# DiTEC-project/gnn-pressure-estimation

Measured on AMD Instinct MI355X. Metric: train snapshots/sec, higher is better.
Workload: dtype f32; 1 GPU; gatres_small (15 blocks, nc=32), C-Town-sized WDN (388 nodes, 860 directed edges), batch_size=32 per GPU, fp32, full training step (device mask 0.95 -> fwd -> masked MSE -> bwd -> Adam), fused per-snapshot kernel (8 CUs per snapshot, row-window tables), hipGraph replay (20 steps per graph launch); global_batch=32, parallelism=dp1, plan_relabelled=False, row_window=92, dropped_steps=0, captured_graphs=25

## Files before the change

gnn-pressure-estimation_amd/_native.py:

```python
from __future__ import annotations

import ctypes as C
import os
from typing import Optional

import torch

from . import _build

_LIB: Optional[C.CDLL] = None

DTYPE_F32, DTYPE_BF16 = 0, 1

ERRORS = {-1: "GATRES_E_BADARG (null/misaligned pointer or bad size)",
          -2: "GATRES_E_UNSUPPORTED (width / storage type not supported: nc must be a power of two in [4, 128]; bf16 "
              "needs nc >= 32)",
          -3: "GATRES_E_GRAPH (edge endpoint out of range)"}


class GatresGraph(C.Structure):
    _fields_ = [("num_nodes", C.c_int32), ("num_edges_gat", C.c_int32), ("num_edges_mean", C.c_int32),
                ("num_segments", C.c_int32),
                ("rowptr", C.c_void_p), ("col", C.c_void_p), ("t_rowptr", C.c_void_p), ("t_eid", C.c_void_p),
                ("t_dst", C.c_void_p), ("m_rowptr", C.c_void_p), ("m_col", C.c_void_p), ("mt_rowptr", C.c_void_p),
                ("mt_dst", C.c_void_p), ("seg_ptr", C.c_void_p), ("max_segment_nodes", C.c_int32),
                ("max_segment_edges_gat", C.c_int32), ("max_segment_edges_mean", C.c_int32), ("flags", C.c_int32),
                ("window", C.c_int32 * 21), ("reserved2", C.c_int32), ("perm", C.c_void_p),
                ("halo", C.c_int32 * 7), ("reserved3", C.c_int32),
                ("part_tables", C.c_void_p), ("part_tables_m", C.c_int32), ("part_tables_stride", C.c_int32)]


MODEL_INFERENCE = 1


class GatresAutoClip(C.Structure):
    _fields_ = [("log", C.c_void_p), ("sorted", C.c_void_p * 2), ("ctl", C.c_void_p), ("partials", C.c_void_p),
                ("norm_out", C.c_void_p), ("clip_out", C.c_void_p), ("coef_out", C.c_void_p), ("capacity", C.c_int64),
                ("partials_cap", C.c_int32), ("reserved", C.c_int32), ("percentile", C.c_double)]


class GatresEpochConfig(C.Structure):
    _fields_ = [("min_delta", C.c_double), ("factor", C.c_double), ("threshold", C.c_double), ("min_lr", C.c_double),
                ("eps", C.c_double), ("patience", C.c_int32), ("scheduler_patience", C.c_int32), ("use_scheduler", C.c_int32),
                ("reserved", C.c_int32)]


class GatresModel(C.Structure):
    _fields_ = [("num_blocks", C.c_int32), ("nc", C.c_int32), ("act_dtype", C.c_int32), ("flags", C.c_int32)]


_P = C.c_void_p
_I32, _I64, _U64, _F32, _F64 = C.c_int32, C.c_int64, C.c_uint64, C.c_float, C.c_double
_GP, _MP = C.POINTER(GatresGraph), C.POINTER(GatresModel)

SIGNATURES = {
    "gatres_graph_count_host": (C.c_int, [_P, _I64, _I64, C.POINTER(_I64)]),
    "gatres_graph_build_host": (C.c_int, [_P, _I64, _I64] + [_P] * 9),
    "gatres_graph_flags_host": (C.c_int, [_P, _I64, _I64, C.POINTER(_I32)]),
    "gatres_graph_part_tables_host": (C.c_int, [_P] * 10 + [_I32, _I32, _P, _I64, C.POINTER(_I64)]),
    "gatres_graph_segments_host": (C.c_int, [_P, _I64, _I64, _I32, _P] + [C.POINTER(_I32)] * 4),
    "gatres_graph_windows_host": (C.c_int, [_P, _I64, _I64, _P, _I32, _P]),
    "gatres_graph_reorder_host": (C.c_int, [_P, _I64, _I64, _P, _I32, _P]),
    "gatres_lz4_decompress_host": (_I64, [_P, _I64, _P, _I64]),
    "gatres_edge_index_hash": (C.c_int, [_P, _I64, _P, _P]),
    "gatres_permute_f32": (C.c_int, [_P, _P, _P, _I32, _I32, _P]),
    "gatres_gather_u8": (C.c_int, [_P, _P, _P, _I32, _P]),
    "gatres_fused_serialize": (C.c_int, [_P]),
    "gatres_probe_xcd_dispatch": (C.c_int, [_P]),
    "gatres_knobs_reload": (C.c_int, []),
    "gatres_fused_status_offset": (_I64, [_MP, _GP]),
    "gatres_lin0_fwd": (C.c_int, [_P, _P, _P, _P, _P, _I32, _I32, _P]),
    "gatres_proj_attn_fwd": (C.c_int, [_P] * 7 + [_I32] * 4 + [_P]),
    "gatres_gat_aggregate_fwd": (C.c_int, [_GP] + [_P] * 6 + [_I32] * 3 + [_P]),
    "gatres_mean_residual_relu_fwd": (C.c_int, [_GP, _P, _P, _P, _I32, _P]),
    "gatres_lin1_fwd": (C.c_int, [_P, _P, _P, _P, _I32, _I32, _P]),
    "gatres_reduce_slabs": (C.c_int, [_P, _I32, _I64, _I64, _P, _P]),
    "gatres_lin1_bwd": (C.c_int, [_P] * 6 + [_I32, _I64, _I32, _I32, _I32, _P]),
    "gatres_mean_bwd": (C.c_int, [_GP, _P, _P, _I32, _P]),
    "gatres_gat_aggregate_bwd_dst": (C.c_int, [_GP] + [_P] * 7 + [_I32, _I32, _P]),
    "gatres_gat_aggregate_bwd_src": (C.c_int, [_GP] + [_P] * 8 + [_I32, _I32, _P]),
    "gatres_proj_bwd_dx": (C.c_int, [_P] * 5 + [_I32] * 3 + [_P]),
    "gatres_proj_bwd_dw": (C.c_int, [_P] * 3 + [_I32, _I64, _I32, _I32, _I32, _P]),
    "gatres_conv_param_grads": (C.c_int, [_P] * 7 + [_I32, _I64, _I32, _I32, _I32, _P]),
    "gatres_lin0_bwd": (C.c_int, [_P] * 5 + [_I32, _I64, _I32, _I32, _P]),
    "gatres_transpose_conv_weights": (C.c_int, [_P, _P, _I32, _I32, _P]),
    "gatres_mask_generate": (C.c_int, [_P, _I32, _F64, _U64, _P, _P, _P]),
    "gatres_stage_batch_mask": (C.c_int, [_P, _P, _P, _P, _I64, _P, _I32, _F64, _U64, _P, _P, _P]),
    "gatres_stage_rows_mask": (C.c_int, [_P, _P, _I32, _P, _P, _P, _I32, _F64, _U64, _P, _P, _P]),
    "gatres_stage_rows_mask_required": (C.c_int, [_P, _P, _I32, _P, _P, _P, _I32, _F64, _U64, _P, _P, _I32, _P, _P]),
    "gatres_stage_multi_rows_mask_required": (C.c_int, [_P, _I32, _P, _P, _P, _I32, _P, _P, _F64, _U64, _P, _P, _P, _P, _P]),
    "gatres_gather_multi_rows": (C.c_int, [_P, _I32, _P, _P, _P, _I32, _I32, _P, _I64, _P]),
    "gatres_masked_metrics": (C.c_int, [_P, _P, _P, _I32, _F64, _F64, _P, _I32, _I32, _P, _P]),
    "gatres_masked_mse": (C.c_int, [_P] * 5 + [_I32, _P]),
    "gatres_masked_loss": (C.c_int, [_P] * 3 + [_I32] + [_P] * 2 + [_I32, _P]),
    "gatres_adam_step": (C.c_int, [_P] * 5 + [_I64] + [_F64] * 5 + [_F32, _P]),
    "gatres_t_gat_aggregate_fwd": (C.c_int, [_GP] + [_P] * 6 + [C.c_int] * 4 + [_P]),
    "gatres_t_gat_aggregate_bwd_dst": (C.c_int, [_GP] + [_P] * 7 + [C.c_int] * 3 + [_P]),
    "gatres_t_gat_aggregate_bwd_src": (C.c_int, [_GP] + [_P] * 8 + [C.c_int] * 3 + [_P]),
    "gatres_t_mean_residual_relu_fwd": (C.c_int, [_GP, _P, _P, _P, C.c_int, C.c_int, _P]),
    "gatres_t_mean_bwd": (C.c_int, [_GP, _P, _P, C.c_int, C.c_int, _P]),
    "gatres_t_lin0_fwd": (C.c_int, [_P] * 5 + [C.c_int] * 3 + [_P]),
    "gatres_t_lin0_bwd": (C.c_int, [_P] * 5 + [C.c_int, _I64, C.c_int, C.c_int, C.c_int, _P]),
    "gatres_t_lin1_fwd": (C.c_int, [_P] * 4 + [C.c_int] * 3 + [_P]),
    "gatres_t_lin1_bwd": (C.c_int, [_P] * 6 + [C.c_int, _I64, C.c_int, C.c_int, C.c_int, C.c_int, _P]),
    "gatres_t_conv_param_grads": (C.c_int, [_P] * 7 + [C.c_int, _I64, C.c_int, C.c_int, C.c_int, C.c_int, _P]),
    "gatres_t_conv_partials": (C.c_int, [_P] * 3 + [C.c_int, _I64, C.c_int, C.c_int, C.c_int] + [_P] * 7 + [C.c_int] * 4 + [_P]),
    "gatres_convert_conv_weights_bf16": (C.c_int, [_P, _P, C.c_int, C.c_int, _P]),
    "gatres_t_proj_attn_fwd": (C.c_int, [_P] * 7 + [C.c_int] * 5 + [_P]),
    "gatres_t_proj_bwd_dx": (C.c_int, [_P] * 5 + [C.c_int] * 4 + [_P]),
    "gatres_t_proj_bwd_dw": (C.c_int, [_P] * 3 + [C.c_int, _I64, C.c_int, C.c_int, C.c_int, C.c_int, _P]),
    "gatres_blocked_supported": (C.c_int, [_MP, _GP]),
    "gatres_bf16_agg_proj_fwd": (C.c_int, [_GP] + [_P] * 12 + [_I32, _P]),
    "gatres_bf16_mean_proj_fwd": (C.c_int, [_GP] + [_P] * 9 + [_I32, _P]),
    "gatres_bf16_src_dx_bwd": (C.c_int, [_GP] + [_P] * 12 + [_I32, _I32, _P]),
    "gatres_param_count": (_I64, [_I32, _I32]),
    "gatres_saved_floats": (_I64, [_MP, _GP]),
    "gatres_scratch_floats": (_I64, [_MP, _GP]),
    "gatres_num_slabs": (_I32, [_MP, _I32]),
    "gatres_model_forward": (C.c_int, [_MP, _GP] + [_P] * 6 + [_P]),
    "gatres_model_backward": (C.c_int, [_MP, _GP] + [_P] * 8 + [_P]),
    "gatres_model_forward_per_op": (C.c_int, [_MP, _GP] + [_P] * 6 + [_P]),
    "gatres_model_backward_per_op": (C.c_int, [_MP, _GP] + [_P] * 8 + [_P]),
    "gatres_model_backward_per_op_part": (C.c_int, [_MP, _GP] + [_P] * 8 + [_I32, _I32, _I32, _P]),
    "gatres_model_reduce_grads": (C.c_int, [_MP, _GP, _P, _P, _P]),
    "gatres_fused_supported": (C.c_int, [_MP, _GP]),
    "gatres_fused_cus_per_segment": (C.c_int, [_MP, _GP]),
    "gatres_fused_window_kernel": (C.c_int, [_MP, _GP]),
    "gatres_fused_reset_sync": (C.c_int, [_MP, _GP, _P, _P]),
    "gatres_fused_set_stamps": (C.c_int, [_P, _I32]),
    "gatres_fused_prepare_backward": (C.c_int, [_MP, _GP, _P, _P, _P]),
    "gatres_fused_run": (C.c_int, [_MP, _GP] + [_P] * 10 + [_I32, _P]),
    "gatres_fused_param_grads": (C.c_int, [_MP, _GP, _P, _P, _P]),
    "gatres_fused_finish": (C.c_int, [_MP, _GP] + [_P] * 4 + [_I32] + [_P] * 4 + [_F64] * 5 + [_F32, _P]),
    "gatres_fused_finish_hp": (C.c_int, [_MP, _GP] + [_P] * 4 + [_I32] + [_P] * 4 + [_F64] * 5 + [_P, _F32, _P, _I32, _F64, _U64, _P, _P]),
    "gatres_fused_finish_folds": (C.c_int, [_MP, _GP]),
    "gatres_fused_param_grads_finish": (C.c_int, [_MP, _GP] + [_P] * 5 + [_I32] + [_P] * 4 + [_F64] * 5 +
                                        [_P, _F32, _I32, _I32, _P]),
    "gatres_autoclip_partials": (_I32, [_I64]),
    "gatres_autoclip_adam_step": (C.c_int, [_P] * 5 + [_I64] + [_F64] * 5 + [_F32, _P, _P]),
    "gatres_train_step": (C.c_int, [_P, _P]),
    "gatres_epoch_control": (C.c_int, [_P, _P, _P, _P, _I32, _P, C.POINTER(GatresEpochConfig), _P, _P, _P, _I32, _P]),
    "gatres_epoch_val_sums": (C.c_int, [_P, _P, _P, _I32, _P, _P]),
    "gatres_snapshot_if": (C.c_int, [_P] * 9 + [_I64, _P]),
    "gatres_grad_flow": (C.c_int, [_MP, _P, _F64, _P, _P, _P]),
    "gatres_grad_flow_count": (_I32, [_I32, _I32]),
    "gatres_mean_abs_diff": (C.c_int, [_P, _P, _I64, _P, _P]),
    "gatres_version": (C.c_char_p, []),
}


ABI_VERSION = 9
LOSS_MSE, LOSS_MAE, LOSS_SCE = 0, 1, 2
EPOCH_STATE, EPOCH_RECORD = 10, 16
# ... 121 lines not shown
```

gnn-pressure-estimation_amd/csrc/gatres_layout.h:

```cpp
#pragma once
#include "gatres_common.h"

static inline __host__ __device__ int64_t r4(int64_t v) { return (v + 3) & ~(int64_t)3; }
#define GATRES_UREC_WORDS 128

struct Layout {
  int nb, nc;
  int64_t N, Eg;
  int64_t p_lin0_w, p_lin0_b, p_block0, p_block_stride, p_lin1_w, p_lin1_b, P;
  int64_t c1_as, c1_ad, c1_b, c1_W, c2_as, c2_ad, c2_b, c2_W;
  int64_t s_xin, s_h1, s_as1, s_ad1, s_al1, s_o1, s_h2, s_as2, s_ad2, s_al2, s_stride, saved_total;
  int64_t sc_y2, sc_ev, sc_xa, sc_xb, sc_gpa, sc_gpb, sc_gy2, sc_ge, sc_gad, sc_gas, sc_gh, sc_go1, sc_wt,
      sc_ge2, sc_gad2, sc_gas2, sc_gh2, sc_slabs, sc_loss_part, scratch_total;
  int64_t sc_px, sc_pmask, sc_pout, sc_pgout, sc_pgx;
  int64_t sc_wb;
  int64_t sc_xch, xch_stride;
  int64_t sc_urec;
  int64_t sc_keep, keep_stride, k_gh1, k_gh2, k_gas1, k_gad1, k_gas2, k_gad2;
  int split_max;
  int64_t sc_flags, flag_words, col_words, sc_part_slabs;
  int num_slabs;
  int slab_rows;
  int64_t slab_stride;
};
// ... 98 lines not shown
  L->sc_slabs = o; o += (int64_t)L->slab_rows * L->slab_stride;
  L->split_max = fused_nodes > 0 ? split_max_for(num_segments) : 1;
  {
    const int64_t lp = (int64_t)num_segments * L->split_max;
    L->sc_loss_part = o; o += r4((lp > L->slab_rows ? lp : L->slab_rows) + 1);
  }
  L->sc_keep = o;
  int64_t k = 0;
  L->k_gh1 = k;  k += r4(N * 2 * nc);
  L->k_gh2 = k;  k += r4(N * nc);
  L->k_gas1 = k; k += r4(N * 2);
  L->k_gad1 = k; k += r4(N * 2);
  L->k_gas2 = k; k += r4(N);
  L->k_gad2 = k; k += r4(N);
  L->keep_stride = k;
  if (fused_nodes > 0) o += (int64_t)nb * k;
  L->sc_flags = o;
  L->flag_words = r4((int64_t)((num_segments + 7) / 8) * 8 * 8 * 32 + 32);
  L->col_words = r4(2LL * nb + 8);
  L->sc_part_slabs = o + L->flag_words + L->col_words;
  if (fused_nodes > 0) o += L->flag_words + L->col_words;
  if (L->split_max > 1) o += (int64_t)num_segments * L->split_max * L->slab_stride;
  L->sc_xch = o;
  L->xch_stride = 0;
  if (L->split_max > 1 && nc <= 32) {
    const XchLayout X = make_xch_layout(nc, fused_nodes, fused_edges);
    L->xch_stride = 2 * X.total;
    o += (int64_t)num_segments * L->xch_stride;
  }
  L->sc_urec = o;
  if (L->xch_stride > 0) o += (int64_t)((num_segments + 7) / 8) * 8 * 8 * GATRES_UREC_WORDS;
  L->sc_wb = o;    o += r4((int64_t)nb * 4 * nc * nc);
  L->sc_px = o;    o += r4(N);
  L->sc_pmask = o; o += r4((N + 3) / 4);
  L->sc_pout = o;  o += r4(N);
  L->sc_pgout = o; o += r4(N);
  L->sc_pgx = o;   o += r4(N);
  L->scratch_total = o;
  return true;
}

static inline int fused_nodes_of(const gatres_graph_t* g) {
  return (g && g->num_segments > 0 && g->seg_ptr && g->max_segment_nodes > 0 && g->max_segment_nodes <= 4096)
             ? g->max_segment_nodes : 0;
}
static inline bool make_layout_g(const gatres_model_t* m, const gatres_graph_t* g, Layout* L) {
  return g && make_layout(m, g->num_nodes, g->num_edges_gat, g->num_segments, fused_nodes_of(g),
                          g->max_segment_edges_gat, L);
}

constexpr int FUSED_STATUS_FAULT = 0, FUSED_STATUS_FAULT_COUNT = 1, FUSED_STATUS_FAULT_TICKETS = 2,
              FUSED_STATUS_DROPPED_STEPS = 3, FUSED_STATUS_SNAPSHOT = 8;
static inline int64_t fused_status_offset(const Layout& L) { return L.sc_flags + L.flag_words - 32; }
static inline unsigned* fused_status(float* scratch, const Layout& L) {
  return reinterpret_cast<unsigned*>(scratch + fused_status_offset(L));
}
static inline unsigned long long* fused_status_snapshot(unsigned* status) {
  return reinterpret_cast<unsigned long long*>(status + FUSED_STATUS_SNAPSHOT);
}


struct SegLayout {
  int64_t xin, h1, as1, ad1, al1, o1, h2, as2, ad2, al2, bstride, total;
};

static inline __host__ __device__ SegLayout make_seg_layout(int nb, int nc, int64_t mn, int64_t me) {
  SegLayout S;
  int64_t o = 0;
  S.xin = o; o += r4(mn * nc);
  S.h1 = o;  o += r4(mn * 2 * nc);
  S.as1 = o; o += r4(mn * 2);
  S.ad1 = o; o += r4(mn * 2);
  S.al1 = o; o += r4(me * 2);
  S.o1 = o;  o += r4(mn * 2 * nc);
  S.h2 = o;  o += r4(mn * nc);
  S.as2 = o; o += r4(mn);
  S.ad2 = o; o += r4(mn);
  S.al2 = o; o += r4(me);
  S.bstride = o;
  S.total = (int64_t)nb * o + r4(mn * nc);
  S.total = (S.total + 63) & ~(int64_t)63;
  return S;
}
```

gnn-pressure-estimation_amd/csrc/graph_plan.hip:

```cpp
#include <algorithm>
#include <vector>

#include "gatres_common.h"

namespace {

static void counting_sort(const std::vector<int32_t>& key, int64_t N, int32_t* ptr, std::vector<int32_t>& perm) {
  const int64_t n = (int64_t)key.size();
  for (int64_t i = 0; i <= N; ++i) ptr[i] = 0;
  for (int64_t e = 0; e < n; ++e) ptr[key[e] + 1]++;
  for (int64_t i = 0; i < N; ++i) ptr[i + 1] += ptr[i];
  std::vector<int32_t> cur(ptr, ptr + N);
  perm.resize(n);
  for (int64_t e = 0; e < n; ++e) perm[cur[key[e]]++] = (int32_t)e;
}

}

extern "C" int gatres_graph_count_host(const int64_t* ei, int64_t E, int64_t N, int64_t* num_edges_gat_out) {
  if ((!ei && E > 0) || !num_edges_gat_out || E < 0 || N <= 0) return GATRES_E_BADARG;
  int64_t keep = 0;
  for (int64_t e = 0; e < E; ++e) {
    const int64_t s = ei[e], d = ei[E + e];
    if (s < 0 || s >= N || d < 0 || d >= N) return GATRES_E_GRAPH;
    keep += (s != d);
  }
  if (keep + N > INT32_MAX || E > INT32_MAX) return GATRES_E_UNSUPPORTED;
  *num_edges_gat_out = keep + N;
  return 0;
}

extern "C" int gatres_graph_build_host(const int64_t* ei, int64_t E, int64_t N, int32_t* rowptr, int32_t* col,
                                       int32_t* t_rowptr, int32_t* t_eid, int32_t* t_dst, int32_t* m_rowptr,
                                       int32_t* m_col, int32_t* mt_rowptr, int32_t* mt_dst) {
  if ((!ei && E > 0) || !rowptr || !col || !t_rowptr || !t_eid || !t_dst || !m_rowptr || !m_col || !mt_rowptr || !mt_dst)
    return GATRES_E_BADARG;
  int64_t Eg = 0;
  const int rc = gatres_graph_count_host(ei, E, N, &Eg);
  if (rc) return rc;

  std::vector<int32_t> src(Eg), dst(Eg);
  int64_t k = 0;
  for (int64_t e = 0; e < E; ++e)
    if (ei[e] != ei[E + e]) { src[k] = (int32_t)ei[e]; dst[k] = (int32_t)ei[E + e]; ++k; }
  for (int64_t i = 0; i < N; ++i, ++k) { src[k] = (int32_t)i; dst[k] = (int32_t)i; }

  std::vector<int32_t> perm, pos(Eg);
  counting_sort(dst, N, rowptr, perm);
  for (int64_t p = 0; p < Eg; ++p) { col[p] = src[perm[p]]; pos[perm[p]] = (int32_t)p; }
  counting_sort(src, N, t_rowptr, perm);
  for (int64_t p = 0; p < Eg; ++p) { t_eid[p] = pos[perm[p]]; t_dst[p] = dst[perm[p]]; }

  std::vector<int32_t> ms(E), md(E);
  for (int64_t e = 0; e < E; ++e) { ms[e] = (int32_t)ei[e]; md[e] = (int32_t)ei[E + e]; }
  counting_sort(md, N, m_rowptr, perm);
  for (int64_t p = 0; p < E; ++p) m_col[p] = ms[perm[p]];
  counting_sort(ms, N, mt_rowptr, perm);
  for (int64_t p = 0; p < E; ++p) mt_dst[p] = md[perm[p]];
  return 0;
}

extern "C" int gatres_graph_flags_host(const int64_t* ei, int64_t E, int64_t N, int32_t* flags_out) {
  if ((!ei && E > 0) || !flags_out || E < 0 || N <= 0) return GATRES_E_BADARG;
  std::vector<uint64_t> key;
  key.reserve((size_t)E);
  std::vector<int32_t> indeg((size_t)N, 0), outdeg((size_t)N, 0);
  for (int64_t e = 0; e < E; ++e) {
    const int64_t s = ei[e], d = ei[E + e];
    if (s < 0 || s >= N || d < 0 || d >= N) return GATRES_E_GRAPH;
    if (s != d) key.push_back(((uint64_t)s << 32) | (uint64_t)d);
    ++indeg[(size_t)d]; ++outdeg[(size_t)s];
  }
  int32_t most = 0;
  for (int64_t i = 0; i < N; ++i) most = std::max(most, std::max(indeg[(size_t)i], outdeg[(size_t)i]));
  const bool le32 = most + 1 <= 32, le6 = most + 1 <= 6;
  std::sort(key.begin(), key.end());
  bool sym = true;
  for (size_t i = 0; i < key.size() && sym; ++i)
    sym = std::binary_search(key.begin(), key.end(), (key[i] << 32) | (key[i] >> 32));
  *flags_out = (sym ? GATRES_GRAPH_SYMMETRIC : 0) | (le32 ? GATRES_GRAPH_DEG_LE32 : 0) | (le6 ? GATRES_GRAPH_DEG_LE6 : 0);
  return 0;
}

extern "C" int gatres_graph_segments_host(const int64_t* ei, int64_t E, int64_t N, int32_t merge_upto,
                                          int32_t* seg_ptr, int32_t* num_segments_out, int32_t* max_nodes_out,
                                          int32_t* max_edges_gat_out, int32_t* max_edges_mean_out) {
// ... 153 lines not shown
      g.elo = rowptr[g.n0 + g.lo] - g.e0;           g.oeg = rowptr[g.n0 + g.hi] - g.e0 - g.elo;
      g.ewlo = rowptr[g.n0 + g.wlo] - g.e0;         g.weg = rowptr[g.n0 + g.whi] - g.e0 - g.ewlo;
      g.melo = m_rowptr[g.n0 + g.lo] - g.em0;       g.oem = m_rowptr[g.n0 + g.hi] - g.em0 - g.melo;
      g.tlo = t_rowptr[g.n0 + g.lo] - g.t0;         g.otg = t_rowptr[g.n0 + g.hi] - g.t0 - g.tlo;
      g.mtlo = mt_rowptr[g.n0 + g.lo] - g.mt0;      g.otm = mt_rowptr[g.n0 + g.hi] - g.mt0 - g.mtlo;
      std::vector<uint16_t> rpo(ow + 1), colo(g.oeg), mrpo(ow + 1), mcolo(g.oem), trpo(ow + 1), teido(g.otg), tdsto(g.otg),
          mrpw(wr + 1), mtrpo(ow + 1), mtdsto(g.otm);
      for (int r = 0; r <= ow; ++r) {
        rpo[r] = (uint16_t)(rowptr[g.n0 + g.lo + r] - (g.e0 + g.elo));
        mrpo[r] = (uint16_t)(m_rowptr[g.n0 + g.lo + r] - (g.em0 + g.melo));
        trpo[r] = (uint16_t)(t_rowptr[g.n0 + g.lo + r] - (g.t0 + g.tlo));
        mtrpo[r] = (uint16_t)(mt_rowptr[g.n0 + g.lo + r] - (g.mt0 + g.mtlo));
      }
      for (int k = 0; k < g.oeg; ++k) colo[k] = (uint16_t)(col[g.e0 + g.elo + k] - g.n0);
      for (int k = 0; k < g.oem; ++k) mcolo[k] = (uint16_t)(m_col[g.em0 + g.melo + k] - g.n0);
      for (int k = 0; k < g.otg; ++k) {
        teido[k] = (uint16_t)(t_eid[g.t0 + g.tlo + k] - g.e0);
        tdsto[k] = (uint16_t)(t_dst[g.t0 + g.tlo + k] - g.n0);
      }
      for (int r = 0; r <= wr; ++r) mrpw[r] = (uint16_t)(m_rowptr[g.n0 + g.wlo + r] - m_rowptr[g.n0 + g.wlo]);
      for (int k = 0; k < g.otm; ++k) mtdsto[k] = (uint16_t)(mt_dst[g.mt0 + g.mtlo + k] - g.n0);
      std::vector<uint16_t> nbin(8 * ow), mbin(8 * ow), tout(16 * ow, 0), mout(16 * ow, 0);
      for (int r = 0; r < ow; ++r) {
        const int ra = g.lo + r;
        {
          const int beg = rpo[r], deg = (int)rpo[r + 1] - beg, elast = std::max(g.oeg - 1, 0);
          nbin[8 * r] = (uint16_t)beg; nbin[8 * r + 1] = (uint16_t)deg;
          for (int k = 0; k < PT_MAXD; ++k)
            nbin[8 * r + 2 + k] = g.oeg > 0 ? colo[std::min(beg + std::min(k, std::max(deg - 1, 0)), elast)] : (uint16_t)ra;
        }
        {
          const int beg = mrpo[r], deg = (int)mrpo[r + 1] - beg, elast = std::max(g.oem - 1, 0);
          mbin[8 * r] = (uint16_t)beg; mbin[8 * r + 1] = (uint16_t)deg;
          for (int k = 0; k < PT_MAXD; ++k) mbin[8 * r + 2 + k] = k < deg ? mcolo[std::min(beg + k, elast)] : (uint16_t)ra;
        }
        {
          const int beg = trpo[r], deg = (int)trpo[r + 1] - beg, elast = std::max(g.otg - 1, 0);
          tout[16 * r] = (uint16_t)deg;
          for (int k = 0; k < PT_MAXD; ++k) {
            const int kk = std::min(beg + std::min(k, std::max(deg - 1, 0)), elast);
            tout[16 * r + 2 + k] = g.otg > 0 ? tdsto[kk] : (uint16_t)ra;
            tout[16 * r + 8 + k] = g.otg > 0 ? teido[kk] : (uint16_t)0;
          }
        }
        {
          const int beg = mtrpo[r], deg = (int)mtrpo[r + 1] - beg, elast = std::max(g.otm - 1, 0);
          mout[16 * r] = (uint16_t)deg;
          for (int k = 0; k < PT_MAXD; ++k) {
            const int kk = std::min(beg + std::min(k, std::max(deg - 1, 0)), elast);
            const int ii = k < deg ? (int)mtdsto[kk] : ra;
            mout[16 * r + 2 + k] = (uint16_t)ii;
            mout[16 * r + 8 + k] = (uint16_t)std::max((int)mrpw[ii - g.wlo + 1] - (int)mrpw[ii - g.wlo], 1);
          }
        }
      }
      auto remote = [&](int j) { return j < g.lo || j >= g.hi; };
      std::vector<uint16_t> f_hlist, f_elist, b_hrow, b_hedge, b_erow, b_eedge;
      for (int k = 0; k < g.oeg; ++k)
        if (remote(colo[k])) { f_hlist.push_back(colo[k]); b_eedge.push_back((uint16_t)(g.elo + k)); }
      for (int r = 0; r < ow; ++r) {
        bool out_remote = false, in_remote = false;
        for (int t = trpo[r]; t < trpo[r + 1]; ++t) out_remote = out_remote || remote(tdsto[t]);
        for (int e = rpo[r]; e < rpo[r + 1]; ++e) in_remote = in_remote || remote(colo[e]);
        if (out_remote) f_elist.push_back((uint16_t)(g.lo + r));
        if (in_remote) b_erow.push_back((uint16_t)(g.lo + r));
      }
      for (int t = 0; t < g.otg; ++t)
        if (remote(tdsto[t])) { b_hrow.push_back(tdsto[t]); b_hedge.push_back(teido[t]); }
      auto uniq = [](std::vector<uint16_t>& v) { std::sort(v.begin(), v.end()); v.erase(std::unique(v.begin(), v.end()), v.end()); };
      uniq(f_hlist); uniq(b_hrow); uniq(b_hedge);
      img.clear();
      auto put = [&](const std::vector<uint16_t>& v, int padded) {
        img.insert(img.end(), v.begin(), v.end());
        img.resize(img.size() + (size_t)(padded - (int)v.size()), 0);
      };
      auto pad16 = [&](size_t from) { while ((img.size() - from) % 8) img.push_back(0); };
      int32_t hdr[GATRES_PT_HEADER] = {0};
      hdr[GATRES_PT_MAGIC] = GATRES_PT_MAGIC_VALUE; hdr[GATRES_PT_M] = M;
      hdr[GATRES_PT_N0] = g.n0; hdr[GATRES_PT_N] = g.n; hdr[GATRES_PT_E0] = g.e0; hdr[GATRES_PT_EM0] = g.em0;
      hdr[GATRES_PT_T0] = g.t0; hdr[GATRES_PT_MT0] = g.mt0; hdr[GATRES_PT_LO] = g.lo; hdr[GATRES_PT_HI] = g.hi;
      hdr[GATRES_PT_WLO] = g.wlo; hdr[GATRES_PT_WHI] = g.whi; hdr[GATRES_PT_ELO] = g.elo; hdr[GATRES_PT_OEG] = g.oeg;
      hdr[GATRES_PT_EWLO] = g.ewlo; hdr[GATRES_PT_WEG] = g.weg; hdr[GATRES_PT_MELO] = g.melo; hdr[GATRES_PT_OEM] = g.oem;
      hdr[GATRES_PT_TLO] = g.tlo; hdr[GATRES_PT_OTG] = g.otg; hdr[GATRES_PT_MTLO] = g.mtlo; hdr[GATRES_PT_OTM] = g.otm;
      size_t from = img.size();
      hdr[GATRES_PT_F_IMG] = GATRES_PT_HEADER + (int)(img.size() / 2);
      put(rpo, even_i(ow + 1)); put(colo, even_i(g.oeg)); put(mrpo, even_i(ow + 1)); put(mcolo, even_i(g.oem));
      pad16(from); put(nbin, 8 * ow); put(mbin, 8 * ow);
      hdr[GATRES_PT_F_IMG_WORDS] = (int)((img.size() - from) / 2);
      from = img.size();
      hdr[GATRES_PT_B_IMG] = GATRES_PT_HEADER + (int)(img.size() / 2);
      put(rpo, even_i(ow + 1)); put(colo, even_i(g.oeg)); put(trpo, even_i(ow + 1)); put(teido, even_i(g.otg));
      put(tdsto, even_i(g.otg)); put(mrpw, even_i(wr + 1)); put(mtrpo, even_i(ow + 1)); put(mtdsto, even_i(g.otm));
      pad16(from); put(nbin, 8 * ow); put(tout, 16 * ow); put(mout, 16 * ow);
      hdr[GATRES_PT_B_IMG_WORDS] = (int)((img.size() - from) / 2);
      auto put_list = [&](const std::vector<uint16_t>& v, int off_field, int cnt_field) {
        hdr[off_field] = GATRES_PT_HEADER + (int)(img.size() / 2);
        hdr[cnt_field] = (int)v.size();
        put(v, even_i((int)v.size()));
      };
      put_list(f_hlist, GATRES_PT_F_HLIST, GATRES_PT_F_HCNT); put_list(f_elist, GATRES_PT_F_ELIST, GATRES_PT_F_ECNT);
      put_list(b_hrow, GATRES_PT_B_HROW, GATRES_PT_B_HRCNT);   put_list(b_hedge, GATRES_PT_B_HEDGE, GATRES_PT_B_HECNT);
      put_list(b_erow, GATRES_PT_B_EROW, GATRES_PT_B_ERCNT);   put_list(b_eedge, GATRES_PT_B_EEDGE, GATRES_PT_B_EECNT);
      const int64_t total_words = GATRES_PT_HEADER + (int64_t)img.size() / 2;
      need = std::max(need, total_words);
      if (out) {
        if (total_words > stride_words) return GATRES_E_BADARG;
        int32_t* dst = out + ((int64_t)s * M + p) * stride_words;
        for (int i = 0; i < GATRES_PT_HEADER; ++i) dst[i] = hdr[i];
        for (size_t i = 0; i + 1 < img.size() + 1 && i < img.size(); i += 2)
          dst[GATRES_PT_HEADER + i / 2] = (int32_t)((uint32_t)img[i] | ((uint32_t)img[i + 1] << 16));
      }
    }
  }
  *stride_words_out = (need + 3) & ~(int64_t)3;
  return 0;
}

extern "C" int gatres_graph_reorder_host(const int64_t* ei, int64_t E, int64_t N, const int32_t* seg_ptr,
                                         int32_t num_segments, int32_t* perm) {
  if ((!ei && E > 0) || !seg_ptr || !perm || num_segments <= 0 || N <= 0 || E < 0) return GATRES_E_BADARG;
  if (N > INT32_MAX || 2 * E > INT32_MAX) return GATRES_E_UNSUPPORTED;
  std::vector<int32_t> key(2 * E), val(2 * E);
  int64_t k = 0;
  for (int64_t e = 0; e < E; ++e) {
    const int64_t s = ei[e], d = ei[E + e];
    if (s < 0 || s >= N || d < 0 || d >= N) return GATRES_E_GRAPH;
    if (s == d) continue;
    key[k] = (int32_t)s; val[k] = (int32_t)d; ++k;
    key[k] = (int32_t)d; val[k] = (int32_t)s; ++k;
  }
  key.resize(k); val.resize(k);
  std::vector<int32_t> ptr(N + 1), order;
  counting_sort(key, N, ptr.data(), order);
  std::vector<int32_t> adj(k);
  for (int64_t p = 0; p < k; ++p) adj[p] = val[order[p]];
  auto deg = [&](int32_t v) { return ptr[v + 1] - ptr[v]; };

  std::vector<int32_t> level(N, -1), queue;
  std::vector<char> done(N, 0);
  queue.reserve(1024);
  std::vector<int32_t> nb;
  auto bfs = [&](int32_t root, std::vector<int32_t>& out) {
    out.clear();
    out.push_back(root);
    level[root] = 0;
    int32_t ecc = 0;
    for (size_t head = 0; head < out.size(); ++head) {
      const int32_t v = out[head];
      nb.clear();
      for (int32_t p = ptr[v]; p < ptr[v + 1]; ++p) {
        const int32_t u = adj[p];
        if (!done[u] && level[u] < 0) { level[u] = level[v] + 1; nb.push_back(u); }
      }
      std::sort(nb.begin(), nb.end(), [&](int32_t a, int32_t b) { return deg(a) != deg(b) ? deg(a) < deg(b) : a < b; });
      for (int32_t u : nb) { out.push_back(u); if (level[u] > ecc) ecc = level[u]; }
    }
    return ecc;
  };
  auto clear_levels = [&](const std::vector<int32_t>& out) { for (int32_t v : out) level[v] = -1; };

  std::vector<int32_t> comp, trial;
  for (int32_t s = 0; s < num_segments; ++s) {
    const int32_t a = seg_ptr[s], b = seg_ptr[s + 1];
    if (a < 0 || b > N || a > b) return GATRES_E_BADARG;
    int32_t next = a;
    std::vector<int32_t> seg_order;
    seg_order.reserve(b - a);
    for (int32_t v0 = a; v0 < b; ++v0) {
      if (done[v0]) continue;
      bfs(v0, comp);
      clear_levels(comp);
      int32_t root = comp[0];
      for (int32_t v : comp) {
        if (v < a || v >= b) return GATRES_E_GRAPH;
        if (deg(v) < deg(root) || (deg(v) == deg(root) && v < root)) root = v;
      }
      int32_t ecc = bfs(root, trial);
      for (int it = 0; it < 8; ++it) {
        int32_t cand = trial.back();
        for (size_t i = trial.size(); i-- > 0 && level[trial[i]] == ecc;)
          if (deg(trial[i]) < deg(cand) || (deg(trial[i]) == deg(cand) && trial[i] < cand)) cand = trial[i];
        clear_levels(trial);
        std::vector<int32_t> t2;
        const int32_t ecc2 = bfs(cand, t2);
        if (ecc2 > ecc) { ecc = ecc2; root = cand; trial.swap(t2); }
        else { clear_levels(t2); bfs(root, trial); break; }
      }
      for (int32_t v : trial) { done[v] = 1; seg_order.push_back(v); }
      clear_levels(trial);
    }
    if ((int32_t)seg_order.size() != b - a) return GATRES_E_GRAPH;
    for (size_t i = seg_order.size(); i-- > 0;) perm[next++] = seg_order[i];
  }
  return 0;
}

extern "C" int64_t gatres_lz4_decompress_host(const uint8_t* src, int64_t src_len, uint8_t* dst, int64_t dst_cap) {
// ... 37 lines not shown
```

gnn-pressure-estimation_amd/csrc/k_fused_dev.h:

```cpp
#pragma once
#include <cstdlib>
#include <mutex>
#include <type_traits>

#include "gatres_common.h"
#include "gatres_layout.h"

namespace {

typedef float f32x4 __attribute__((ext_vector_type(4)));
typedef unsigned short u16;

constexpr int LDS_BYTES = 163840;
constexpr int MAXD = 6;

struct FusedArgs {
  const int* seg_ptr;
  const int *rowptr, *col, *t_rowptr, *t_eid, *t_dst, *m_rowptr, *m_col, *mt_rowptr, *mt_dst;
  int N;
  const float* params;
  const float* wt;
  const int* perm;
  const float* x;
  const uint8_t* mask;
  const float* y;
  float* out;
  float* g_out;
  float* loss_part;
  float* g_x;
  float* saved;
  float* scratch;
  float* slabs;
  float* part_slabs;
  unsigned* flags;
  int* err;
  int num_segments;
  int seg0, seg_cnt;
  int M;
  int safe_sync;
  int keep_lds;
  int no_halo;
  int sym;
  int facts;
  const int* ptab;
  int ptab_m, ptab_stride;
  unsigned long long* xch;
  int* urec;
  XchLayout XL;
  Layout L;
  SegLayout SL;
  int phases;
  unsigned long long* stamps;
  int stamp_cap;
  int criterion;
};

enum { PH_LOSS = 16 };

#if GATRES_DIAG
#define STAMPS_PTR (a.stamps)
#define STAMP()                                                                                  \
  do {                                                                                           \
    if (a.stamps && blockIdx.x == 0 && threadIdx.x == 0 && stamp_i < a.stamp_cap)                \
      a.stamps[stamp_i++] = wall_clock64();                                                      \
  } while (0)
#else
#define STAMPS_PTR (static_cast<unsigned long long*>(nullptr))
#define STAMP() do {} while (0)
#endif

#if GATRES_DIAG
#define XSTAMP()                                                                                 \
  do {                                                                                           \
    if (xs_on && (threadIdx.x == 0 || threadIdx.x == THREADS - 64) && xs_i < 64)                 \
      a.stamps[2048 + (part * 2 + (threadIdx.x ? 1 : 0)) * 64 + xs_i] = wall_clock64();         \
    ++xs_i;                                                                                      \
  } while (0)
#else
#define XSTAMP() do {} while (0)
#endif

__host__ __device__ inline int even(int v) { return (v + 1) & ~1; }
__host__ __device__ inline int topo_fwd_bytes(int n, int eg, int em) {
  return 2 * (2 * even(n + 1) + even(eg) + even(em));
}
__host__ __device__ inline int topo_bwd_bytes(int n, int eg, int em) {
  return 2 * (4 * even(n + 1) + 3 * even(eg) + 2 * even(em));
}
static long long wl_bytes(int nc) {
  const long long f = 4LL * (2LL * nc * (2 * nc + 4) + 4 * nc);
  return f <= 40960 ? f + 16 : 0;
}
static bool cache_fits(int nc, int threads, int n, int eg, int em) {
  const long long fwd = 4LL * n * (3 * nc + 4) + topo_fwd_bytes(n, eg, em);
  const long long bwd = 12LL * threads + 4LL * n * 2 * nc + 8LL * even(eg) + 16LL * n + topo_bwd_bytes(n, eg, em) +
                        wl_bytes(nc);
// ... 1449 lines not shown
    for (int u = 0; u < U; ++u)
      if (valid[u]) dst[o[u]] = __uint_as_float((unsigned)v[u]);
  }
}

template <int THREADS>
__device__ __forceinline__ void xch_heartbeat(Xch& x, int ) {
  u64* hb = x.base_hb;
  if (threadIdx.x == 0) gran_store(hb + x.part, 0.f, x.ep, x.local);
  const int lane = (int)threadIdx.x - (THREADS - 64);
  if (lane >= 0) {
    const bool mine = lane < x.M && lane != x.part;
    int spin = 0;
    for (;;) {
      const bool ok = !mine || x.dead || (int)((unsigned)(gran_load(hb + lane) >> 32) - (x.ep - 1u)) >= 0;
      if (__all(ok)) break;
      if (++spin > SPIN_LIMIT) { *x.err = 1; x.dead = true; }
    }
  }
  asm volatile("s_waitcnt vmcnt(0)" ::: "memory");
}

template <int THREADS>
__device__ __forceinline__ int build_export_rows(const int* __restrict__ ptr, const int* __restrict__ idx, int n0, Rows rw,
                                                 u16* list, int cap, int* counter) {
  if (threadIdx.x == 0) *counter = 0;
  __syncthreads();
  for (int r = rw.lo + threadIdx.x; r < rw.hi; r += THREADS) {
    bool remote = false;
    for (int t = ptr[n0 + r]; t < ptr[n0 + r + 1]; ++t) {
      const int j = idx[t] - n0;
      remote = remote || j < rw.lo || j >= rw.hi;
    }
    if (remote) {
      const int pos = atomicAdd(counter, 1);
      if (pos < cap) list[pos] = (u16)r;
    }
  }
  __syncthreads();
  const int total = *counter;
  __syncthreads();
  return total;
}

template <int THREADS>
__device__ __forceinline__ void dma_copy16(float* dst, const float* src, int nfloat, int w0) {
  const int lane = threadIdx.x & 63, wave = __builtin_amdgcn_readfirstlane(threadIdx.x >> 6);
  if (wave < w0) return;
  for (int c = (wave - w0) * 256; c < nfloat; c += (THREADS / 64 - w0) * 256)
    if (c + lane * 4 < nfloat) __builtin_amdgcn_global_load_lds(src + c + lane * 4, dst + c, 16, 0, 0);
}
template <int THREADS>
__device__ __forceinline__ void dma_copy4(float* dst, const float* src, int nfloat, int w0) {
  const int lane = threadIdx.x & 63, wave = __builtin_amdgcn_readfirstlane(threadIdx.x >> 6);
  if (wave < w0) return;
  for (int c = (wave - w0) * 64; c < nfloat; c += (THREADS / 64 - w0) * 64)
    if (c + lane < nfloat) __builtin_amdgcn_global_load_lds(src + c + lane, dst + c, 4, 0, 0);
}
template <int K, int M, int EPI, int THREADS>
__device__ __forceinline__ void w_prefetch(float* wl, const float* __restrict__ Wm, const float* __restrict__ att_src,
                                           const float* __restrict__ att_dst, int w0) {
  constexpr int KP = K + 4;
  const int lane = threadIdx.x & 63, wave = __builtin_amdgcn_readfirstlane(threadIdx.x >> 6);
  if (wave < w0) return;
  for (int m = wave - w0; m < M; m += THREADS / 64 - w0)
    if (lane < K / 4) __builtin_amdgcn_global_load_lds(Wm + m * K + lane * 4, wl + m * KP, 16, 0, 0);
  if constexpr (EPI == EPI_ATT) {
    if (wave == THREADS / 64 - 1 && lane < M / 4) __builtin_amdgcn_global_load_lds(att_src + lane * 4, wl + M * KP, 16, 0, 0);
    if (wave == THREADS / 64 - 2 && lane < M / 4) __builtin_amdgcn_global_load_lds(att_dst + lane * 4, wl + M * KP + M, 16, 0, 0);
  }
}

__host__ __device__ inline long long win_fwd_bytes(int nc, int wr, int ow, int ge, int gm, int hl) {
  const long long wlf = 2LL * nc * (2 * nc + 4) + 4 * nc;
  return 4LL * (wr * (3LL * nc + 2) + ow * (3LL * nc + 2 + 8)) + 2 * (4 * wlf + 16) + 2LL * (2 * even(ow + 2) + even(ge) + even(gm)) +
         64 + 4LL * (hl + 4) + 32LL * ow + 16 + ow + 16;
}
__host__ __device__ inline long long win_bwd_bytes(int nc, int threads, int wr, int ow, int ge, int gm, int hl) {
  const long long wlf = 2LL * nc * (2 * nc + 4) + 4 * nc;
  return 12LL * threads + 4LL * (wr * (4LL * nc + 2) + ow * (2LL * nc + 4 + 4) + 4LL * even(ge)) + 2 * (4 * wlf + 16) +
         2LL * (3 * even(ow + 2) + 3 * even(ge) + even(wr + 2) + even(gm)) + 64 + 8LL * (hl + 4) + 80LL * ow + 16 + ow + 16;
}

__host__ __device__ inline long long win_keep_bytes(int nb, int ow) { return (12LL * nb * ow + 15) & ~15LL; }

__device__ __forceinline__ void lds_barrier() { asm volatile("s_waitcnt lgkmcnt(0)\n\ts_barrier" ::: "memory"); }


}
```

gnn-pressure-estimation_amd/csrc/k_fused_host.hip:

```cpp
#include <atomic>
#include <vector>
#include "k_fused_dev.h"
#include "k_mask.h"
#include "k_autoclip.h"
#include "k_update.h"

namespace {

static unsigned long long* g_stamps = nullptr;
static int g_stamp_cap = 0;

struct SlabSumArgs {
  const float* slabs;
  int num_slabs, num_loss;
  long long stride;
  float* grads;
  const float* loss_part;
  float* loss;
  int do_adam, use_snap, reduce_blocks;
  unsigned* status;
  double* ac_partials;
  unsigned long long* ac_ctl;
};

// ... 411 lines not shown
}

extern "C" int gatres_fused_cus_per_segment(const gatres_model_t* m, const gatres_graph_t* g) {
  Layout L;
  if (!gatres_fused_supported(m, g) || !make_layout_g(m, g, &L)) return 0;
  return fused_split(L, g);
}

extern "C" int gatres_fused_reset_sync(const gatres_model_t* m, const gatres_graph_t* g, float* scratch, void* stream) {
  if (!m || !g || !scratch) return GATRES_E_BADARG;
  Layout L;
  if (!make_layout_g(m, g, &L)) return GATRES_E_UNSUPPORTED;
  if (fused_nodes_of(g) == 0) return 0;
  if (L.xch_stride > 0) {
    const hipError_t e = hipMemsetAsync(scratch + L.sc_xch, 0, (size_t)g->num_segments * L.xch_stride * 4, gatres_stream(stream));
    if (e != hipSuccess) return (int)e;
  }
  return (int)hipMemsetAsync(scratch + L.sc_flags, 0, (size_t)(L.flag_words + L.col_words) * 4, gatres_stream(stream));
}

extern "C" int gatres_fused_window_kernel(const gatres_model_t* m, const gatres_graph_t* g) {
  Layout L;
  if (!gatres_fused_supported(m, g) || !make_layout_g(m, g, &L)) return 0;
  return window_kernel_fits(L, g, fused_split(L, g)) ? 1 : 0;
}

extern "C" int gatres_fused_set_stamps(uint64_t* stamps, int32_t capacity) {
  g_stamps = reinterpret_cast<unsigned long long*>(stamps);
  g_stamp_cap = stamps ? capacity : 0;
  return 0;
}

extern "C" int gatres_fused_prepare_backward(const gatres_model_t* m, const gatres_graph_t* g, const float* params,
                                             float* scratch, void* stream) {
  if (!m || !g || !params || !scratch) return GATRES_E_BADARG;
  Layout L;
  if (!make_layout_g(m, g, &L)) return GATRES_E_UNSUPPORTED;
  return gatres_transpose_conv_weights(params, scratch + L.sc_wt, L.nb, L.nc, stream);
}

static std::atomic<int> g_xcd_rr[64];
static int xcd_rr_cached() {
  int dev = 0;
  if (hipGetDevice(&dev) != hipSuccess || dev < 0 || dev >= 64) return 0;
  return g_xcd_rr[dev].load(std::memory_order_acquire) == 2 ? 1 : 0;
}
extern "C" int gatres_fused_run(const gatres_model_t* m, const gatres_graph_t* g, const float* params,
                                const float* x, const uint8_t* mask, const float* y, float* out, float* g_out,
                                float* loss_part, float* g_x, float* saved, float* scratch, int32_t phases,
                                void* stream) {
  if (!m || !g || !params || !x || !scratch) return GATRES_E_BADARG;
  if (!gatres_fused_supported(m, g)) return GATRES_E_UNSUPPORTED;
  FusedArgs a;
  if (!make_layout_g(m, g, &a.L)) return GATRES_E_UNSUPPORTED;
  if ((phases & GATRES_PHASE_FORWARD) && !out) return GATRES_E_BADARG;
  if ((phases & GATRES_PHASE_LOSS) && (!mask || !y || !out || !g_out || !loss_part)) return GATRES_E_BADARG;
  const int32_t crit_bits = phases & (GATRES_PHASE_LOSS_MAE | GATRES_PHASE_LOSS_SCE);
  if (crit_bits && (!(phases & GATRES_PHASE_LOSS) || crit_bits == (GATRES_PHASE_LOSS_MAE | GATRES_PHASE_LOSS_SCE)))
    return GATRES_E_BADARG;
  if ((phases & GATRES_PHASE_BACKWARD) && (!saved || !g_out)) return GATRES_E_BADARG;
  a.seg_ptr = g->seg_ptr;
  a.rowptr = g->rowptr; a.col = g->col; a.t_rowptr = g->t_rowptr; a.t_eid = g->t_eid; a.t_dst = g->t_dst;
  a.m_rowptr = g->m_rowptr; a.m_col = g->m_col; a.mt_rowptr = g->mt_rowptr; a.mt_dst = g->mt_dst;
  a.N = g->num_nodes;
  a.perm = g->perm;
  a.params = params; a.wt = scratch + a.L.sc_wt;
  a.x = x; a.mask = mask; a.y = y; a.out = out; a.g_out = g_out; a.loss_part = loss_part; a.g_x = g_x;
  a.saved = saved; a.scratch = scratch; a.slabs = scratch + a.L.sc_slabs;
  a.num_segments = g->num_segments;
  a.seg0 = 0; a.seg_cnt = g->num_segments;
  a.M = fused_split(a.L, g);
  a.safe_sync = gatres_knobs()->fused_safe_sync;
  a.no_halo = gatres_knobs()->fused_no_halo | (gatres_knobs()->xch_nowait ? 2 : 0) | (gatres_knobs()->diag_nomask ? 4 : 0);
  a.sym = (g->flags & GATRES_GRAPH_SYMMETRIC) && !gatres_knobs()->fused_heartbeat ? 1 : 0;
  a.ptab = g->part_tables; a.ptab_m = g->part_tables_m; a.ptab_stride = g->part_tables_stride;
  {
    const int tiles = (g->max_segment_nodes + 15) / 16, part_rows = a.M > 0 ? 16 * ((tiles + a.M - 1) / a.M) : INT32_MAX;
    a.facts = ((g->flags & GATRES_GRAPH_DEG_LE6) ? 0x400 : 0) | (part_rows <= 64 ? 0x1000 : 0) |
              (((m->flags & GATRES_MODEL_INFERENCE) && phases == GATRES_PHASE_FORWARD) ? 0x2000 : 0) |
              ((xcd_rr_cached() && !gatres_knobs()->window_sync_start) ? 0x4000 : 0);
  }
  a.keep_lds = (phases & GATRES_PHASE_FORWARD) && (phases & GATRES_PHASE_BACKWARD) && !gatres_knobs()->fused_no_keep &&
           window_kernel_fits(a.L, g, a.M, true) ? 1 : 0;
  a.flags = reinterpret_cast<unsigned*>(scratch + a.L.sc_flags);
  a.err = reinterpret_cast<int*>(fused_status(scratch, a.L));
  a.part_slabs = scratch + a.L.sc_part_slabs;
  a.SL = make_seg_layout(a.L.nb, a.L.nc, g->max_segment_nodes, g->max_segment_edges_gat);
  a.xch = reinterpret_cast<unsigned long long*>(scratch + a.L.sc_xch);
  a.urec = reinterpret_cast<int*>(scratch + a.L.sc_urec);
  a.XL = make_xch_layout(a.L.nc, g->max_segment_nodes, g->max_segment_edges_gat);
  a.stamps = g_stamps; a.stamp_cap = g_stamp_cap;
  a.phases = (phases & (GATRES_PHASE_FORWARD | GATRES_PHASE_BACKWARD)) | ((phases & GATRES_PHASE_LOSS) ? PH_LOSS : 0);
  a.criterion = crit_bits == GATRES_PHASE_LOSS_MAE ? GATRES_LOSS_MAE : crit_bits == GATRES_PHASE_LOSS_SCE ? GATRES_LOSS_SCE
                                                                                                        : GATRES_LOSS_MSE;
  hipStream_t st = gatres_stream(stream);
  if (a.M > 1) serialize_split_launch(st);
  int rc = launch_fused(m->nc, threads_for(m->nc), a, g, st);
  if (rc == 0 && a.M > 1 && !(phases & GATRES_PHASE_BACKWARD)) {
    hipLaunchKernelGGL(fused_status_kernel, dim3(1), dim3(64), 0, st, reinterpret_cast<unsigned*>(a.err));
    rc = gatres_launch_status();
  }
  return rc;
}

extern "C" int gatres_fused_serialize(void* stream) { return serialize_split_launch(gatres_stream(stream)); }

extern "C" int gatres_probe_xcd_dispatch(void* stream) {
  int dev = 0;
  if (hipGetDevice(&dev) != hipSuccess || dev < 0 || dev >= 64) return 0;
  const int have = g_xcd_rr[dev].load(std::memory_order_acquire);
  if (have != 0) return have == 2 ? 1 : 0;
  hipStream_t st = gatres_stream(stream);
  hipStreamCaptureStatus cs = hipStreamCaptureStatusNone;
  if (hipStreamIsCapturing(st, &cs) != hipSuccess || cs != hipStreamCaptureStatusNone) return 0;
  const int cus = device_cus();
  if (cus < 16 || cus > 4096) { g_xcd_rr[dev].store(1, std::memory_order_release); return 0; }
  unsigned* d = nullptr;
  if (hipMalloc(&d, sizeof(unsigned) * cus) != hipSuccess) return 0;
  std::vector<unsigned> h((size_t)cus, 0xffu);
  bool ok = hipMemsetAsync(d, 0xff, sizeof(unsigned) * cus, st) == hipSuccess;
  if (ok) {
    hipLaunchKernelGGL(xcd_probe_kernel, dim3((unsigned)cus), dim3(1024), 0, st, d);
    ok = hipGetLastError() == hipSuccess && hipStreamSynchronize(st) == hipSuccess &&
         hipMemcpy(h.data(), d, sizeof(unsigned) * cus, hipMemcpyDeviceToHost) == hipSuccess;
  }
  (void)hipFree(d);
  if (!ok) return 0;
  bool rr = true;
  for (int b = 0; b < cus && rr; ++b) rr = (h[b] & 0xfu) == (h[b & 7] & 0xfu) && h[b] != 0xffffffffu;
  g_xcd_rr[dev].store(rr ? 2 : 1, std::memory_order_release);
  return rr ? 1 : 0;
}

extern "C" int64_t gatres_fused_status_offset(const gatres_model_t* m, const gatres_graph_t* g) {
  Layout L;
  if (!gatres_fused_supported(m, g) || !make_layout_g(m, g, &L)) return -1;
  return fused_status_offset(L);
}

extern "C" int gatres_fused_param_grads(const gatres_model_t* m, const gatres_graph_t* g, const float* saved,
                                        float* scratch, void* stream) {
  return gatres_fused_param_grads_ex(m, g, saved, scratch, nullptr, stream);
}
extern "C" __attribute__((visibility("hidden"))) int gatres_fused_param_grads_ex(
    const gatres_model_t* m, const gatres_graph_t* g, const float* saved, float* scratch, const uint64_t* step_counter, void* stream) {
  if (!m || !g || !saved || !scratch) return GATRES_E_BADARG;
  if (!gatres_fused_supported(m, g)) return GATRES_E_UNSUPPORTED;
  ParamGradArgs a;
  if (!make_layout_g(m, g, &a.L)) return GATRES_E_UNSUPPORTED;
  if (a.L.nb == 0) return 0;
  a.seg_ptr = g->seg_ptr; a.saved = saved; a.keep = scratch + a.L.sc_keep; a.slabs = scratch + a.L.sc_slabs;
  a.M = fused_split(a.L, g); a.part_slabs = scratch + a.L.sc_part_slabs;
  a.SL = make_seg_layout(a.L.nb, a.L.nc, g->max_segment_nodes, g->max_segment_edges_gat);
  a.wt = scratch + a.L.sc_wt;
  const dim3 grid((unsigned)(2 * a.L.nb * g->num_segments));
  hipStream_t st = gatres_stream(stream);
  if (m->nc == 16 || m->nc == 32) {
    if (step_counter) {
      unsigned* status = fused_status(scratch, a.L);
      a.step_counter = reinterpret_cast<const unsigned long long*>(step_counter);
      a.status = fused_nodes_of(g) > 0 ? status : nullptr;
      a.snap = fused_status_snapshot(status);
    }
    if (m->nc == 16) hipLaunchKernelGGL((param_grads_reg_kernel<16>), grid, dim3(PGR_THREADS), 0, st, a);
    else             hipLaunchKernelGGL((param_grads_reg_kernel<32>), grid, dim3(PGR_THREADS), 0, st, a);
    const int rc = gatres_launch_status();
    return rc ? rc : (step_counter ? 1 : 0);
  }
  switch (m->nc) {
    case 4: hipLaunchKernelGGL((param_grads_kernel<4, 256>), grid, dim3(256), 0, st, a); break;
    case 8: hipLaunchKernelGGL((param_grads_kernel<8, 256>), grid, dim3(256), 0, st, a); break;
    case 64: hipLaunchKernelGGL((param_grads_kernel<64, 512>), grid, dim3(512), 0, st, a); break;
    case 128: hipLaunchKernelGGL((param_grads_kernel<128, 512>), grid, dim3(512), 0, st, a); break;
    default: return GATRES_E_UNSUPPORTED;
  }
  return gatres_launch_status();
}

static bool finish_folds(const gatres_model_t* m, const Layout& L) {
  return (m->nc == 16 || m->nc == 32) && L.nb > 0;
}

extern "C" int gatres_fused_finish_folds(const gatres_model_t* m, const gatres_graph_t* g) {
  Layout L;
  if (!gatres_fused_supported(m, g) || !make_layout_g(m, g, &L)) return 0;
  return finish_folds(m, L) ? 1 : 0;
}

extern "C" int gatres_fused_param_grads_finish(const gatres_model_t* m, const gatres_graph_t* g, const float* saved,
                                               float* scratch, float* grads, const float* loss_part, float* loss,
                                               int32_t do_adam, float* params, float* exp_avg, float* exp_avg_sq,
                                               uint64_t* step_counter, double lr, double beta1, double beta2, double eps,
                                               double weight_decay, const double* hparams, float grad_scale,
                                               int32_t block_lo, int32_t block_hi, void* stream) {
  if (!m || !g || !saved || !scratch || !grads) return GATRES_E_BADARG;
  if (do_adam && (!params || !exp_avg || !exp_avg_sq || !step_counter)) return GATRES_E_BADARG;
  if ((loss_part == nullptr) != (loss == nullptr)) return GATRES_E_BADARG;
  if (!gatres_fused_supported(m, g)) return GATRES_E_UNSUPPORTED;
  ParamGradArgs a;
  if (!make_layout_g(m, g, &a.L)) return GATRES_E_UNSUPPORTED;
  if (!finish_folds(m, a.L)) return GATRES_E_UNSUPPORTED;
  if (block_lo < 0 || block_hi > a.L.nb || block_lo >= block_hi) return GATRES_E_BADARG;
  if (do_adam && (block_lo != 0 || block_hi != a.L.nb)) return GATRES_E_BADARG;
  a.seg_ptr = g->seg_ptr; a.saved = saved; a.keep = scratch + a.L.sc_keep; a.slabs = scratch + a.L.sc_slabs;
  a.M = fused_split(a.L, g); a.part_slabs = scratch + a.L.sc_part_slabs;
  a.SL = make_seg_layout(a.L.nb, a.L.nc, g->max_segment_nodes, g->max_segment_edges_gat);
  a.wt = scratch + a.L.sc_wt;
  FinishArgs f;
  f.u = update_args_of(params, nullptr, exp_avg, exp_avg_sq, step_counter, a.L.P, lr, beta1, beta2, eps, weight_decay, hparams,
                       grad_scale);
  f.u.wt = do_adam ? scratch + a.L.sc_wt : nullptr;
  f.grads = grads; f.loss_part = loss_part; f.loss = loss; f.num_loss = g->num_segments * a.M; f.do_adam = do_adam ? 1 : 0;
  f.status = fused_nodes_of(g) > 0 ? fused_status(scratch, a.L) : nullptr;
  f.colcnt = reinterpret_cast<unsigned*>(scratch + a.L.sc_flags + a.L.flag_words);
// ... 79 lines not shown
```

gnn-pressure-estimation_amd/csrc/k_window.hip:

```cpp
#include <climits>
#include "k_window_stages.h"

namespace {

__device__ __forceinline__ void dma_land(int w0) {
  if ((int)__builtin_amdgcn_readfirstlane(threadIdx.x >> 6) >= w0) asm volatile("s_waitcnt vmcnt(0)" ::: "memory");
}
template <int THREADS>
__device__ __forceinline__ void vec_prefetch(float* dst, const float* __restrict__ src, int n) {
  const int lane = threadIdx.x & 63, wave = __builtin_amdgcn_readfirstlane(threadIdx.x >> 6);
  if (wave == THREADS / 64 - 1 && lane * 4 < n) __builtin_amdgcn_global_load_lds(src + lane * 4, dst, 16, 0, 0);
}
__device__ __forceinline__ int launder_s(int v) {
  asm volatile("" : "+s"(v));
  return v;
}

typedef const __attribute__((address_space(4))) FusedArgs* KArgs;
__device__ __forceinline__ KArgs kargs_fresh() {
  KArgs p = (KArgs)__builtin_amdgcn_kernarg_segment_ptr();
  asm volatile("" : "+s"(p));
  return p;
}
#define FRESH_ARGS()                                                                                          \
  const KArgs ka_ = kargs_fresh();                                                                            \
  [[maybe_unused]] const auto& L = ka_->L; [[maybe_unused]] const auto& SL = ka_->SL; [[maybe_unused]] const auto& XL = ka_->XL

struct FwdRec {
  int lo, hi, ow, wr, oeg, elo, hcnt, ecnt;
  int xA, xB, wlA, wlB, hA, hB, hBw, y2T, al2L, sa2, sa1, sd2, sd1, fflag, hlist, elist, nbin, mbin, rp, colo, mrp, mcolo, mo1, mxin;
};
struct BwdRec {
  int lo, hi, ow, wr, wlo, elo, ewlo, weg, n0, hrcnt, hecnt, ercnt, eecnt;
  int RA, gpT, gy2T, ge2, ge1, gad2, gad1, hTw, hT2, hT1, asTw, asT2, asT1, adTo, adT2, adT1, alTw, alT2, alT1, xG2, xG1, gkeep,
      wlA, wlB, rp, colo, trp, teido, tdsto, mrp, mtrp, mtdsto, nbin, tout, mout, hrow, hedge, erow, eedge, bflag, mo1, mxin;
};
static_assert(sizeof(FwdRec) <= 4 * (GATRES_UREC_WORDS / 2) && sizeof(BwdRec) <= 4 * (GATRES_UREC_WORDS / 2), "record halves");
constexpr int NO_TABLE = INT_MIN;
template <class R>
__device__ __forceinline__ const __attribute__((address_space(4))) R* rec_fresh(const int* words) {
  auto p = (const __attribute__((address_space(4))) R*)(unsigned long long)words;
  asm volatile("" : "+s"(p));
  return p;
}
__device__ __forceinline__ void rec_published() { asm volatile("s_dcache_inv\n\ts_waitcnt lgkmcnt(0)" ::: "memory"); }
#define FRESH_FWD() const auto rf_ = rec_fresh<FwdRec>(myrec)
#define FRESH_BWD() const auto rb_ = rec_fresh<BwdRec>(myrec + GATRES_UREC_WORDS / 2)
#define LDS_TABLE(T, base, off) (reinterpret_cast<T*>((base) + (off)))
#define REC_LOAD_T(T, n) const int o_##n = RECP->n;
#define REC_LOAD_I(n) const int o_##n = RECP->n;
#define REC_PIN_T(T, n) , "s"(o_##n)
#define REC_PIN_I(n) , "s"(o_##n)
#define REC_DEF_T(T, n) [[maybe_unused]] T* n = LDS_TABLE(T, lds_raw, o_##n);
#define REC_DEF_N(T, n) [[maybe_unused]] T* n = o_##n == NO_TABLE ? nullptr : LDS_TABLE(T, lds_raw, o_##n);
#define REC_DEF_I(n) [[maybe_unused]] const int n = o_##n;
#define REC_LOADS(LIST) LIST(REC_LOAD_T, REC_LOAD_T, REC_LOAD_I)
#ifdef GATRES_REC_PINS
#define REC_PINS(LIST, ...) asm volatile("" ::"s"(0) LIST(REC_PIN_T, REC_PIN_T, REC_PIN_I) __VA_ARGS__)
#else
#define REC_PINS(LIST, ...) do {} while (0)
#endif
#define REC_DEFS(LIST) LIST(REC_DEF_T, REC_DEF_N, REC_DEF_I) [[maybe_unused]] const Rows rw = {lo, hi}
__device__ __forceinline__ u16* align16(u16* p) {
  return reinterpret_cast<u16*>((reinterpret_cast<uintptr_t>(p) + 15) & ~(uintptr_t)15);
}

template <int NC, int THREADS>
__device__ __forceinline__ void scale_g_pre(float* gpT, const u16* mrp, int lo, int ow) {
  for (int idx = threadIdx.x; idx < ow * NC; idx += THREADS) {
    const int r = lo + idx / NC;
    const float cnt = (float)max((int)mrp[r + 1] - (int)mrp[r], 1);
    float* p = gpT + (size_t)r * NC + idx % NC;
    *p = *p / cnt;
  }
}

template <int NC, int THREADS, int PH = -1>
__global__ __launch_bounds__(THREADS) void gatres_window_kernel(const FusedArgs a) {
  const int ph_ = PH < 0 ? a.phases : (PH & 0xff);
  const bool keep_ = PH < 0 ? a.keep_lds != 0 : (PH & 0x100) != 0;
  constexpr bool SYM = PH >= 0 && (PH & 0x200) != 0;
  constexpr bool NOHUB = PH >= 0 && (PH & 0x400) != 0;
  constexpr bool PTAB = PH >= 0 && (PH & 0x800) != 0;
  constexpr bool OW64 = PH >= 0 && (PH & 0x1000) != 0;
  constexpr bool NOSAVE = PH >= 0 && (PH & 0x2000) != 0 && (PH & 0xff) == GATRES_PHASE_FORWARD;
  constexpr bool XLOCAL = PH >= 0 && (PH & 0x4000) != 0;
  const bool mse_ = PH < 0 ? a.criterion == GATRES_LOSS_MSE : (PH & 0x8000) == 0;
#ifdef GATRES_NO_XPAD
  constexpr int XPF = 0, XPB = 0;
#else
  constexpr int XPF = (NC == 32 && NOHUB) ? 4 : 0;
  constexpr int XPB = (NC == 32 && PH >= 0 && (PH & 0x100) != 0) ? 4 : 0;
#endif
  __shared__ __attribute__((aligned(16))) unsigned char lds_raw[LDS_BYTES];
  float* ldsf = reinterpret_cast<float*>(lds_raw);
  const Layout& L = a.L;
  const int M = a.M;
  const int within = blockIdx.x % (8 * M);
  const int seg = a.seg0 + (blockIdx.x / (8 * M)) * 8 + (within & 7), part = within >> 3;
  if (seg >= a.seg0 + a.seg_cnt) return;
  const int tid = threadIdx.x;
  const int wave_u = __builtin_amdgcn_readfirstlane(threadIdx.x >> 6);
  const int* pt = (PTAB || (a.ptab && a.ptab_m == M)) ? a.ptab + ((size_t)seg * M + part) * (size_t)a.ptab_stride : nullptr;
  int hv = 0;
  if (PTAB || pt) hv = pt[min((int)(threadIdx.x & 63), GATRES_PT_HEADER - 1)];
  auto H = [&](int field) { return __builtin_amdgcn_readlane(hv, field); };
#ifndef GATRES_NO_L2_TOUCH
  if constexpr (PTAB && NC == 32) {
    if (ph_ & GATRES_PHASE_FORWARD) {
      if (tid < 64) { if (tid * 32 < a.ptab_stride) (void)*reinterpret_cast<const volatile int*>(pt + tid * 32); }
      else if (tid < 64 + 2 * NC * NC / 32 && L.nb > 0)
        (void)*reinterpret_cast<const volatile float*>(a.params + L.p_block0 + L.c1_W + (tid - 64) * 32);
    } else {
      for (int k = tid * 32; k < a.ptab_stride; k += THREADS * 32) (void)*reinterpret_cast<const volatile int*>(pt + k);
    }
  }
#endif
  int n0, n, e0, em0, t0, mt0;
  Rows rw;
  if (PTAB || pt) {
    if (H(GATRES_PT_MAGIC) != GATRES_PT_MAGIC_VALUE || H(GATRES_PT_M) != M) {
      if (tid == 0) *a.err = 1;
      if constexpr (PTAB) return;
      pt = nullptr;
    }
  }
  if (PTAB || pt) {
    n0 = H(GATRES_PT_N0); n = H(GATRES_PT_N); e0 = H(GATRES_PT_E0); em0 = H(GATRES_PT_EM0); t0 = H(GATRES_PT_T0);
    mt0 = H(GATRES_PT_MT0); rw.lo = H(GATRES_PT_LO); rw.hi = H(GATRES_PT_HI);
  } else {
    n0 = uni(a.seg_ptr[seg]); n = uni(a.seg_ptr[seg + 1]) - n0;
    e0 = uni(a.rowptr[n0]); em0 = uni(a.m_rowptr[n0]); t0 = uni(a.t_rowptr[n0]); mt0 = uni(a.mt_rowptr[n0]);
    const int tiles = (n + 15) >> 4;
    rw.lo = 16 * (int)((long long)tiles * part / M);
    rw.hi = min(n, 16 * (int)((long long)tiles * (part + 1) / M));
  }
  const int lo = rw.lo, ow = rw.hi - rw.lo;
  const bool ow64 = OW64 || ow <= 64;
  Group grp;
  grp.flags = a.flags + (size_t)seg * 8 * FLAG_STRIDE; grp.M = M; grp.part = part; grp.err = a.err;
  constexpr bool assume_local = XLOCAL;
  group_init<THREADS>(grp, XLOCAL);
  if constexpr (XLOCAL) grp.local = true;
  else if (a.safe_sync) grp.local = false;
  const XchLayout& XL = a.XL;
  Xch xc;
  xc.base = a.xch + (size_t)seg * (size_t)(L.xch_stride / 2);
  xc.base_hb = xc.base + XL.hb;
  xc.M = M; xc.part = part; xc.err = a.err; xc.local = grp.local;
  xc.dead = GATRES_DIAG && (a.no_halo & 2) != 0;
  xc.ep = (unsigned)uni((int)__hip_atomic_load(grp.flags + part * FLAG_STRIDE + 2, __ATOMIC_RELAXED, __HIP_MEMORY_SCOPE_AGENT));
  const XchBuf xbuf = xch_buffer(xc.base, XL.total);
  const bool pace = SYM ? false : !a.sym;
  constexpr int PW = 8;
  const int dw0 = NC == 32 ? PW : min((ow + 15) >> 4, THREADS / 64 - 4);
  constexpr int WL_FLOATS = 2 * NC * (2 * NC + 4) + 4 * NC;
  constexpr int WLB = (WL_FLOATS + 3) & ~3;
  constexpr int B1OFF = 2 * NC * (NC + 4) + 4 * NC;
  constexpr int B2OFF = NC * (2 * NC + 4) + 2 * NC;
  constexpr int A2OFF = 2 * NC * (NC + 4);
  constexpr int A1OFF = NC * (2 * NC + 4);
  static_assert(B1OFF + 2 * NC <= WLB && B2OFF + NC <= WLB && A2OFF + 2 * NC <= WLB && A1OFF + 4 * NC <= WLB, "W slot tails");
  const float* P = a.params;
  float* sc = a.scratch;
  unsigned char* lds_top = lds_raw + LDS_BYTES - (keep_ ? win_keep_bytes(L.nb, ow) : 0);
  unsigned long long* mo1 = keep_ ? reinterpret_cast<unsigned long long*>(lds_top) - lo : nullptr;
  unsigned* mxin = keep_ ? reinterpret_cast<unsigned*>(lds_top + 8LL * L.nb * ow) - lo : nullptr;
  [[maybe_unused]] int stamp_i = 0;
  STAMP();
  if (STAMPS_PTR && blockIdx.x == 0 && threadIdx.x == 0) STAMPS_PTR[a.stamp_cap] = clock64();

  int wlo, whi, elo, oeg, ewlo, weg, melo, oem, tlo, otg, mtlo, otm;
  if (PTAB || pt) {
    wlo = H(GATRES_PT_WLO); whi = H(GATRES_PT_WHI); elo = H(GATRES_PT_ELO); oeg = H(GATRES_PT_OEG); ewlo = H(GATRES_PT_EWLO);
    weg = H(GATRES_PT_WEG); melo = H(GATRES_PT_MELO); oem = H(GATRES_PT_OEM); tlo = H(GATRES_PT_TLO); otg = H(GATRES_PT_OTG);
    mtlo = H(GATRES_PT_MTLO); otm = H(GATRES_PT_OTM);
  } else {
    int* mm = reinterpret_cast<int*>(lds_raw);
    if (tid == 0) { mm[0] = lo; mm[1] = rw.hi; }
    __syncthreads();
    int vmin = lo, vmax = rw.hi;
    for (int e = a.rowptr[n0 + lo] + tid; e < a.rowptr[n0 + rw.hi]; e += THREADS) {
      const int j = a.col[e] - n0; vmin = min(vmin, j); vmax = max(vmax, j + 1);
    }
    for (int t = a.t_rowptr[n0 + lo] + tid; t < a.t_rowptr[n0 + rw.hi]; t += THREADS) {
      const int j = a.t_dst[t] - n0; vmin = min(vmin, j); vmax = max(vmax, j + 1);
    }
    for (int e = a.m_rowptr[n0 + lo] + tid; e < a.m_rowptr[n0 + rw.hi]; e += THREADS) {
      const int j = a.m_col[e] - n0; vmin = min(vmin, j); vmax = max(vmax, j + 1);
    }
    for (int t = a.mt_rowptr[n0 + lo] + tid; t < a.mt_rowptr[n0 + rw.hi]; t += THREADS) {
      const int j = a.mt_dst[t] - n0; vmin = min(vmin, j); vmax = max(vmax, j + 1);
    }
    if (vmin < lo) atomicMin(&mm[0], vmin);
    if (vmax > rw.hi) atomicMax(&mm[1], vmax);
    __syncthreads();
    wlo = uni(mm[0]); whi = uni(mm[1]);
    __syncthreads();
    elo = uni(a.rowptr[n0 + lo]) - e0;        oeg = uni(a.rowptr[n0 + rw.hi]) - e0 - elo;
    ewlo = uni(a.rowptr[n0 + wlo]) - e0;      weg = uni(a.rowptr[n0 + whi]) - e0 - ewlo;
    melo = uni(a.m_rowptr[n0 + lo]) - em0;    oem = uni(a.m_rowptr[n0 + rw.hi]) - em0 - melo;
    tlo = uni(a.t_rowptr[n0 + lo]) - t0;      otg = uni(a.t_rowptr[n0 + rw.hi]) - t0 - tlo;
    mtlo = uni(a.mt_rowptr[n0 + lo]) - mt0;   otm = uni(a.mt_rowptr[n0 + rw.hi]) - mt0 - mtlo;
  }
  const int wr = whi - wlo;

  const SegLayout& SL = a.SL;
  float* segbase = a.saved + (int64_t)seg * SL.total;

  constexpr int LB_R = THREADS / NC;
  const bool fuse_loss = (ph_ & PH_LOSS) && (ph_ & GATRES_PHASE_FORWARD) && (ph_ & GATRES_PHASE_BACKWARD) &&
                         (OW64 || ow <= 2 * LB_R) && ow64 && (OW64 || ow <= THREADS / (NC / 4));
  float* dml = ldsf + 64;
  float xk[2] = {0.f, 0.f};

  int* const myrec = a.urec + (size_t)blockIdx.x * GATRES_UREC_WORDS;
  auto lds_off = [&](const void* p) { return (int)(reinterpret_cast<const unsigned char*>(p) - lds_raw); };

  if (ph_ & GATRES_PHASE_FORWARD) {
    constexpr bool xreg = NC == 32;
    {
    float* hAw = ldsf;
    float* hBw = hAw + (size_t)wr * 2 * NC;
    float* saw = hBw + (size_t)wr * NC;
    float* sdo = saw + (size_t)((wr * 2 + 3) & ~3);
    float* xAo = sdo + (size_t)((ow * 2 + 3) & ~3);
    float* xBo = xAo + (size_t)ow * (NC + XPF);
    float* wlA = reinterpret_cast<float*>(lds_raw + ((reinterpret_cast<unsigned char*>(xBo + (size_t)ow * (2 * NC + XPF)) - lds_raw + 15) & ~15));
    float* wlB = wlA + WLB;
    u16* tp = reinterpret_cast<u16*>(wlB + WLB);
    u16* rpo = tp;             tp += even(ow + 1);
    u16* colo = tp;            tp += even(oeg);
    u16* mrpo = tp;            tp += even(ow + 1);
    u16* mcolo = tp;           tp += even(oem);
    tp = align16(tp);
    u16* nbin = tp;            tp += 8 * ow;
    u16* mbin = tp;            tp += 8 * ow;
    int* hcounter = reinterpret_cast<int*>(tp);
    const u16* f_img_end = tp;
    u16* hlist = tp + 2;
    unsigned char* fflag_o = lds_top - ((ow + 15) & ~15);
    const int hcap = max(0, (int)((fflag_o - reinterpret_cast<unsigned char*>(hlist)) / 4)) & ~1;
    u16* elist = hlist + hcap;
    const unsigned char* fflag = fflag_o - lo;
    float* hA = hAw - wlo * 2 * NC;
    float* hB = hBw - wlo * NC;
    float* sa2 = saw - wlo * 2;  float* sa1 = saw - wlo;
    float* sd2 = sdo - lo * 2;   float* sd1 = sdo - lo;
    float* xA = xAo - lo * (NC + XPF);
    float* xB = xBo - lo * (2 * NC + XPF);
    const u16* rp = rpo - lo;  const u16* mrp = mrpo - lo;
    int hcnt = 0, ecnt = 0;
    if (PTAB || pt) {
      hcnt = H(GATRES_PT_F_HCNT); ecnt = H(GATRES_PT_F_ECNT);
      if (H(GATRES_PT_F_IMG_WORDS) * 2 != (int)(f_img_end - rpo) || hcnt > hcap || ecnt > hcap) {
        if (tid == 0) *a.err = 1;
        hcnt = min(hcnt, hcap); ecnt = min(ecnt, hcap);
      } else {
        dma_copy4<THREADS>(reinterpret_cast<float*>(rpo), reinterpret_cast<const float*>(pt + H(GATRES_PT_F_IMG)),
                           H(GATRES_PT_F_IMG_WORDS), 0);
      }
      dma_copy4<THREADS>(reinterpret_cast<float*>(hlist), reinterpret_cast<const float*>(pt + H(GATRES_PT_F_HLIST)), (hcnt + 1) / 2, 0);
      dma_copy4<THREADS>(reinterpret_cast<float*>(elist), reinterpret_cast<const float*>(pt + H(GATRES_PT_F_ELIST)), (ecnt + 1) / 2, 0);
    } else {
      copy_rowptr16<THREADS>(rpo, a.rowptr, n0 + lo, ow, e0 + elo);
      copy_idx16<THREADS>(colo, a.col, e0 + elo, oeg, n0);
      copy_rowptr16<THREADS>(mrpo, a.m_rowptr, n0 + lo, ow, em0 + melo);
      copy_idx16<THREADS>(mcolo, a.m_col, em0 + melo, oem, n0);
    }
    for (int k = tid; k < ((ow + 15) & ~15) / 4; k += THREADS) reinterpret_cast<unsigned*>(fflag_o)[k] = 0u;
    float* xcur = segbase + SL.xin;
    if (L.nb > 0) {
      const float* pb0 = P + L.p_block0;
      w_prefetch<NC, 2 * NC, EPI_ATT, THREADS>(wlA, pb0 + L.c1_W, pb0 + L.c1_as, pb0 + L.c1_ad, 0);
      vec_prefetch<THREADS>(wlA + B1OFF, pb0 + L.c1_b, 2 * NC);
    }
    {
      const float* w = P + L.p_lin0_w;
      const float* b = P + L.p_lin0_b;
      for (int idx = rw.lo * (NC / 4) + tid; idx < rw.hi * (NC / 4); idx += THREADS) {
        const int r = idx / (NC / 4), c0 = (idx % (NC / 4)) * 4;
        const int node = ext_id(a.perm, n0 + r);
        const float xv = (a.mask && a.mask[node]) ? 0.f : a.x[node];
#ifndef GATRES_NO_XKEEP
        if (mxin && L.nb > 0 && c0 == 0) mxin[r] = __float_as_uint(xv);
#endif
        const float4 wv = ld4(w + c0), bv = ld4(b + c0);
        float4 o;
        o.x = xv * wv.x + bv.x; o.y = xv * wv.y + bv.y; o.z = xv * wv.z + bv.z; o.w = xv * wv.w + bv.w;
        if (!NOSAVE) st4(xcur + (unsigned)(r * NC + c0), o);
        st4(xA + (unsigned)(r * (NC + XPF) + c0), o);
      }
    }
    dma_land(0);
    __syncthreads();
    if (!PTAB && !pt) {
      build_nbr_in<THREADS>(rw, rp, colo, oeg, false, nbin);
      build_nbr_in<THREADS>(rw, mrp, mcolo, oem, true, mbin);
      hcnt = uni(build_halo<THREADS>(rp, colo, nullptr, rw, hlist, nullptr, hcap, hcounter));
      ecnt = uni(build_export_rows<THREADS>(a.t_rowptr, a.t_dst, n0, rw, elist, hcap, hcounter));
      if (hcnt > hcap || ecnt > hcap) {
        if (tid == 0) *a.err = 1;
        hcnt = min(hcnt, hcap); ecnt = min(ecnt, hcap);
      }
    }
    if (xreg)
      for (int k = tid; k < ecnt; k += THREADS) fflag_o[(int)elist[k] - lo] = 1;
    if (tid == 0) {
      FwdRec r;
      r.lo = rw.lo; r.hi = rw.hi; r.ow = ow; r.wr = wr; r.oeg = oeg; r.elo = elo; r.hcnt = hcnt; r.ecnt = ecnt;
      r.xA = lds_off(xA); r.xB = lds_off(xB); r.wlA = lds_off(wlA); r.wlB = lds_off(wlB); r.hA = lds_off(hA); r.hB = lds_off(hB);
      r.hBw = lds_off(hBw); r.y2T = lds_off(hAw - wlo * NC); r.al2L = lds_off(hAw + (size_t)wr * NC);
      r.sa2 = lds_off(sa2); r.sa1 = lds_off(sa1); r.sd2 = lds_off(sd2); r.sd1 = lds_off(sd1); r.fflag = lds_off(fflag);
      r.hlist = lds_off(hlist); r.elist = lds_off(elist); r.nbin = lds_off(nbin); r.mbin = lds_off(mbin);
      r.rp = lds_off(rp); r.colo = lds_off(colo); r.mrp = lds_off(mrp); r.mcolo = lds_off(mcolo);
      r.mo1 = mo1 ? lds_off(mo1) : NO_TABLE; r.mxin = mxin ? lds_off(mxin) : NO_TABLE;
      const int* src = reinterpret_cast<const int*>(&r);
#pragma unroll
      for (int k = 0; k < (int)(sizeof(FwdRec) / 4); ++k)
        __hip_atomic_store(myrec + k, src[k], __ATOMIC_RELAXED, __HIP_MEMORY_SCOPE_AGENT);
      asm volatile("s_waitcnt vmcnt(0)" ::: "memory");
    }
    }
    __syncthreads();
    rec_published();
    auto xout = [&](bool on, const unsigned char* flag, long long t_rows, long long t_small) {
      XOut x;
      x.xb = xbuf; x.ep = xc.ep + 1u; x.local = xc.local; x.on = on; x.flag = flag;
      x.t_rows = (unsigned)t_rows; x.t_small = (unsigned)t_small;
      return x;
    };
    STAMP();
#define RECP rf_
    const int nb = L.nb;
    for (int b = 0; b < nb; ++b) {
      {
        FRESH_ARGS(); FRESH_FWD();
#define LIST_(T_, N_, I_) I_(lo) I_(hi) T_(float, xA) T_(float, wlA) T_(float, wlB) T_(float, hA) T_(float, sa2) T_(float, sd2) T_(const unsigned char, fflag)
        REC_LOADS(LIST_);
        [[maybe_unused]] const float* pb = P + L.p_block0 + (int64_t)launder_s(b) * L.p_block_stride;
        [[maybe_unused]] float* base = segbase + (int64_t)launder_s(b) * SL.bstride;
        REC_PINS(LIST_, , "s"(pb), "s"(base));
        REC_DEFS(LIST_);
#undef LIST_
        if (NC != 32 || wave_u >= dw0) {
          w_prefetch<2 * NC, NC, EPI_ATT, THREADS>(wlB, pb + L.c2_W, pb + L.c2_as, pb + L.c2_ad, dw0);
          vec_prefetch<THREADS>(wlB + B2OFF, pb + L.c2_b, NC);
        }
        if constexpr (NC == 32) {
          if (wave_u < PW) {
            win_proj<NC, 2 * NC, 2, EPI_ATT, 2, PW, THREADS, NC + XPF>(rw, xA, wlA, NOSAVE ? nullptr : base + SL.h1, 0, hA,
                                                         NOSAVE ? nullptr : base + SL.as1, NOSAVE ? nullptr : base + SL.ad1, sa2,
                                                         sd2, nullptr, nullptr, nullptr, nullptr, xout(xreg, fflag, XL.f1h, XL.f1a));
          }
        } else
          seg_proj<NC, 2 * NC, 2, EPI_ATT, THREADS, true, true>(rw, xA, 0, pb + L.c1_W, base + SL.h1, 0, hA, 0, pb + L.c1_as,
                                                                 pb + L.c1_ad, base + SL.as1, base + SL.ad1, 0, sa2, sd2,
                                                                 nullptr, 0, nullptr, 0, wlA);
#ifndef GATRES_PROBE_NO_FWD_LAND
        dma_land(dw0);
#endif
        lds_barrier();
      }
      {
        FRESH_ARGS(); FRESH_FWD();
#define LIST_(T_, N_, I_) I_(lo) I_(hi) T_(float, hA) T_(float, sa2) T_(const u16, hlist) T_(const u16, elist) I_(hcnt) I_(ecnt)
        REC_LOADS(LIST_);
        REC_PINS(LIST_);
        REC_DEFS(LIST_);
#undef LIST_
        ++xc.ep;
        if (!xreg) xch_export2<2 * NC, 2, THREADS>(xc, xbuf, elist, ecnt, hA, (unsigned)XL.f1h, elist, ecnt, sa2, (unsigned)XL.f1a);
        xch_import2<2 * NC, 2, THREADS>(xc, xbuf, hlist, hcnt, (unsigned)XL.f1h, hA, hlist, hcnt, (unsigned)XL.f1a, sa2);
        xch_after<THREADS>(xc, pace);
        lds_barrier();
        STAMP();
      }
      {
        FRESH_ARGS(); FRESH_FWD();
#define LIST_(T_, N_, I_) I_(lo) I_(hi) T_(const u16, nbin) T_(const u16, rp) T_(const u16, colo) T_(float, hA) T_(float, sa2) T_(float, sd2) T_(float, hBw) T_(float, wlA) T_(float, xB) T_(const unsigned char, fflag) N_(unsigned long long, mo1) I_(ow) I_(oeg) I_(wr) I_(elo)
        REC_LOADS(LIST_);
        [[maybe_unused]] const float* pb = P + L.p_block0 + (int64_t)launder_s(b) * L.p_block_stride;
        [[maybe_unused]] float* base = segbase + (int64_t)launder_s(b) * SL.bstride;
        REC_PINS(LIST_, , "s"(pb), "s"(base));
        REC_DEFS(LIST_);
#undef LIST_
        if (NOHUB || __builtin_expect(2 * oeg <= wr * NC, 1)) {
          if constexpr (NC == 32) {
            win_fwd_agg<true, 2, NC, THREADS, NOHUB, 2 * NC + XPF>(rw, nbin, rp, colo, hA, sa2, sd2, NOSAVE ? nullptr : base + SL.al1, elo, hBw, wlA + B1OFF,
                                              NOSAVE ? nullptr : base + SL.o1, 0, xB, mo1 ? mo1 + b * ow : nullptr, xout(false, fflag, 0, 0));
          } else {
            win_softmax<2, THREADS>(rw, nbin, rp, colo, sa2, sd2, base + SL.al1, elo, hBw);
            lds_barrier();
            win_gather<true, 2, NC, THREADS>(rw, nbin, rp, colo, hA, hBw, wlA + B1OFF, base + SL.o1, 0, xB,
                                             mo1 ? mo1 + b * ow : nullptr);
          }
        } else {
          dma_land(dw0);
          seg_softmax<2, false, THREADS>(rw, rp, colo, sa2, sd2, 0, base + SL.al1, elo, nullptr);
          __syncthreads();
          seg_gather<true, 2, NC, THREADS, 1>(rw, rp, colo, hA, 0, base + SL.al1, elo, pb + L.c1_b, base + SL.o1, 0, xB, 0,
                                               mo1 ? mo1 + b * ow : nullptr);
        }
        lds_barrier();
        STAMP();
      }
      {
        FRESH_ARGS(); FRESH_FWD();
// ... 170 lines not shown
          }
          const float scale = Mn > 0.f ? 2.f / Mn : 0.f;
          if (tid < ow) {
            const float g = dv * scale;
            a.g_out[ext_id(a.perm, n0 + rw.lo + tid)] = g;
            dml[tid] = g;
          }
        } else {
          int node = 0;
          float s = 0.f, term = 0.f;
          if (tid < ow) {
            node = ext_id(a.perm, n0 + rw.lo + tid);
            if (a.mask[node]) term = gatres_loss_term(a.criterion, dml[tid], a.y[node], &s);
          }
          const float part_sum = block_sum<THREADS>(term, ldsf);
          if (tid == 0) {
            a.loss_part[seg * M + part] = part_sum;
            if (seg == 0 && part == 0) a.loss_part[a.num_segments * M] = Mn;
          }
          const float inv = Mn > 0.f ? 1.f / Mn : 0.f;
          if (tid < ow) {
            const float g = s * inv;
            a.g_out[node] = g;
            dml[tid] = g;
          }
        }
      }
    }
    __syncthreads();
    STAMP();
    if (fuse_loss) STAMP();
  }

  if ((ph_ & PH_LOSS) && !fuse_loss) {
    float cnt = 0.f;
    for (int i = tid; i < a.N; i += THREADS) cnt += a.mask[i] ? 1.f : 0.f;
    const float Mn = block_sum<THREADS>(cnt, ldsf);
    float part_sum = 0.f;
    for (int r = rw.lo + tid; r < rw.hi; r += THREADS) {
      const int node = ext_id(a.perm, n0 + r);
      if (a.mask[node]) {
        if (mse_) {
          const float d = a.out[node] - a.y[node];
          part_sum = fmaf(d, d, part_sum);
        } else {
          float s;
          part_sum += gatres_loss_term(a.criterion, a.out[node], a.y[node], &s);
        }
      }
    }
    part_sum = block_sum<THREADS>(part_sum, ldsf);
    if (tid == 0) {
      a.loss_part[seg * M + part] = part_sum;
      if (seg == 0 && part == 0) a.loss_part[a.num_segments * M] = Mn;
    }
    if (mse_) {
      const float scale = Mn > 0.f ? 2.f / Mn : 0.f;
      for (int r = rw.lo + tid; r < rw.hi; r += THREADS) {
        const int node = ext_id(a.perm, n0 + r);
        a.g_out[node] = a.mask[node] ? (a.out[node] - a.y[node]) * scale : 0.f;
      }
    } else {
      const float inv = Mn > 0.f ? 1.f / Mn : 0.f;
      for (int r = rw.lo + tid; r < rw.hi; r += THREADS) {
        const int node = ext_id(a.perm, n0 + r);
        float s = 0.f;
        if (a.mask[node]) (void)gatres_loss_term(a.criterion, a.out[node], a.y[node], &s);
        a.g_out[node] = s * inv;
      }
    }
    __syncthreads();
    STAMP();
  }

  if (ph_ & GATRES_PHASE_BACKWARD) {
    float* const red = ldsf;
    constexpr bool xedge = NC == 32;
    const bool xrows = xedge && keep_;
    constexpr int64_t w = 2LL * NC * NC;
    float* gp_cur = sc + L.sc_gpa;
    float* gp_nxt = sc + L.sc_gpb;
    float* const slab = a.part_slabs + ((int64_t)seg * M + part) * L.slab_stride;
    {
    float* RAw = red + 3 * THREADS;
    float* gew = RAw + (size_t)wr * 2 * NC;
    float* gado = gew + 2 * (size_t)even(weg);
    float* hTw = gado + (size_t)((ow * 2 + 3) & ~3);
    float* asTw = hTw + (size_t)wr * 2 * NC;
    float* adTo = asTw + (size_t)((wr * 2 + 3) & ~3);
    float* alTw = adTo + (size_t)((ow * 2 + 3) & ~3);
    float* xGo = alTw + 2 * (size_t)even(weg);
    float* gko = xGo + (size_t)ow * (2 * NC + XPB);
    float* wlA = reinterpret_cast<float*>(lds_raw + ((reinterpret_cast<unsigned char*>(gko + (keep_ ? (size_t)ow * NC : 0)) - lds_raw + 15) & ~15));
    float* wlB = wlA + WLB;
    u16* tp = reinterpret_cast<u16*>(wlB + WLB);
    u16* rpo = tp;             tp += even(ow + 1);
    u16* colo = tp;            tp += even(oeg);
    u16* trpo = tp;            tp += even(ow + 1);
    u16* teido = tp;           tp += even(otg);
    u16* tdsto = tp;           tp += even(otg);
    u16* mrpw = tp;            tp += even(wr + 1);
    u16* mtrpo = tp;           tp += even(ow + 1);
    u16* mtdsto = tp;          tp += even(otm);
    tp = align16(tp);
    u16* nbin = tp;            tp += 8 * ow;
    u16* tout = tp;            tp += 16 * ow;
    u16* mout = tp;            tp += 16 * ow;
    int* hcounter = reinterpret_cast<int*>(tp);
    const u16* b_img_end = tp;
    u16* hrow = tp + 2;
    unsigned char* bflag_o = lds_top - ((ow + 15) & ~15);
    const int hcap = max(0, (int)((bflag_o - reinterpret_cast<unsigned char*>(hrow)) / 8)) & ~1;
    u16* hedge = hrow + hcap;
    u16* erow = hedge + hcap;
    u16* eedge = erow + hcap;
    __syncthreads();
    const unsigned char* bflag = bflag_o - lo;
    for (int k = tid; k < ((ow + 15) & ~15) / 4; k += THREADS) reinterpret_cast<unsigned*>(bflag_o)[k] = 0u;
    int hrcnt = 0, hecnt = 0, ercnt = 0, eecnt = 0;
    if (PTAB || pt) {
      hrcnt = H(GATRES_PT_B_HRCNT); hecnt = H(GATRES_PT_B_HECNT); ercnt = H(GATRES_PT_B_ERCNT); eecnt = H(GATRES_PT_B_EECNT);
      if (H(GATRES_PT_B_IMG_WORDS) * 2 != (int)(b_img_end - rpo) || hrcnt > hcap || hecnt > hcap || ercnt > hcap || eecnt > hcap) {
        if (tid == 0) *a.err = 1;
        hrcnt = min(hrcnt, hcap); hecnt = min(hecnt, hcap); ercnt = min(ercnt, hcap); eecnt = min(eecnt, hcap);
      } else {
        dma_copy4<THREADS>(reinterpret_cast<float*>(rpo), reinterpret_cast<const float*>(pt + H(GATRES_PT_B_IMG)),
                           H(GATRES_PT_B_IMG_WORDS), 0);
      }
      dma_copy4<THREADS>(reinterpret_cast<float*>(hrow), reinterpret_cast<const float*>(pt + H(GATRES_PT_B_HROW)), (hrcnt + 1) / 2, 0);
      dma_copy4<THREADS>(reinterpret_cast<float*>(hedge), reinterpret_cast<const float*>(pt + H(GATRES_PT_B_HEDGE)), (hecnt + 1) / 2, 0);
      dma_copy4<THREADS>(reinterpret_cast<float*>(erow), reinterpret_cast<const float*>(pt + H(GATRES_PT_B_EROW)), (ercnt + 1) / 2, 0);
      dma_copy4<THREADS>(reinterpret_cast<float*>(eedge), reinterpret_cast<const float*>(pt + H(GATRES_PT_B_EEDGE)), (eecnt + 1) / 2, 0);
    } else {
      copy_rowptr16<THREADS>(rpo, a.rowptr, n0 + lo, ow, e0 + elo);
      copy_idx16<THREADS>(colo, a.col, e0 + elo, oeg, n0);
      copy_rowptr16<THREADS>(trpo, a.t_rowptr, n0 + lo, ow, t0 + tlo);
      copy_idx16<THREADS>(teido, a.t_eid, t0 + tlo, otg, e0);
      copy_idx16<THREADS>(tdsto, a.t_dst, t0 + tlo, otg, n0);
      copy_rowptr16<THREADS>(mrpw, a.m_rowptr, n0 + wlo, wr, a.m_rowptr[n0 + wlo]);
      copy_rowptr16<THREADS>(mtrpo, a.mt_rowptr, n0 + lo, ow, mt0 + mtlo);
      copy_idx16<THREADS>(mtdsto, a.mt_dst, mt0 + mtlo, otm, n0);
    }
    const u16* rp = rpo - lo;  const u16* trp = trpo - lo;  const u16* mrp = mrpw - wlo;  const u16* mtrp = mtrpo - lo;
    float* RA = RAw - wlo * 2 * NC;
    float* gpT = RAw - wlo * NC;
    float* gy2T = RAw + (size_t)wr * NC - wlo * NC;
    float* ge2 = gew - ewlo;      float* ge1 = gew - ewlo * 2;
    float* gad2 = gado - lo;      float* gad1 = gado - lo * 2;
    float* hT2 = hTw - wlo * NC;  float* hT1 = hTw - wlo * 2 * NC;
    float* asT2 = asTw - wlo;     float* asT1 = asTw - wlo * 2;
    float* adT2 = adTo - lo;      float* adT1 = adTo - lo * 2;
    float* alT2 = alTw - ewlo;    float* alT1 = alTw - ewlo * 2;
    float* xG2 = xGo - lo * (NC + XPB);   float* xG1 = xGo - lo * (2 * NC + XPB);
    float* gkeep = keep_ ? gko - lo * NC : nullptr;

    const float* xfinal = segbase + (int64_t)L.nb * SL.bstride + SL.xin;
    auto dma_conv2_early = [&](int blk, int w0) {
      if (wave_u < w0) return;
      FRESH_ARGS();
      blk = launder_s(blk);
      const float* bs = segbase + (int64_t)blk * SL.bstride;
      dma_copy16<THREADS>(hTw, bs + SL.h2 + (size_t)wlo * NC, wr * NC, w0);
      dma_copy4<THREADS>(asTw, bs + SL.as2 + wlo, wr, w0);
      dma_copy4<THREADS>(adTo, bs + SL.ad2 + lo, ow, w0);
      w_prefetch<NC, 2 * NC, EPI_RESID_MASK, THREADS>(wlA, a.wt + (int64_t)blk * 2 * w + w, nullptr, nullptr, w0);
      vec_prefetch<THREADS>(wlA + A2OFF, P + L.p_block0 + (int64_t)blk * L.p_block_stride + L.c2_as, 2 * NC);
    };
    auto dma_conv2_late = [&](int blk, int w0) {
      if (wave_u < w0) return;
      FRESH_ARGS();
      blk = launder_s(blk);
      const float* bs = segbase + (int64_t)blk * SL.bstride;
      dma_copy4<THREADS>(alTw, bs + SL.al2 + ewlo, weg, w0);
    };
    if (L.nb > 0) { dma_conv2_early(L.nb - 1, 0); dma_conv2_late(L.nb - 1, 0); }
    if (fuse_loss) {
      const int c = tid % NC, rg = tid / NC;
      const float wv = P[L.p_lin1_w + c];
      float aw = 0.f, ab = 0.f;
#pragma unroll
      for (int k = 0; k < 2; ++k) {
        const int r = rw.lo + rg + k * LB_R;
        if (r < rw.hi) {
          const float go = dml[r - rw.lo], xv = xk[k];
          aw = fmaf(go, xv, aw);
          ab += go;
          const float gv = (L.nb > 0 && !(xv > 0.f)) ? 0.f : go * wv;
          gp_cur[((size_t)n0 + r) * NC + c] = gv;
          gpT[(size_t)r * NC + c] = gv;
          if (gkeep) gkeep[(size_t)r * NC + c] = gv;
        }
      }
      __syncthreads();
      red[tid] = aw; red[THREADS + tid] = ab;
      __syncthreads();
      if (rg == 0) {
        float s0 = 0.f, s1 = 0.f;
        for (int k = 0; k < LB_R; ++k) { s0 += red[k * NC + c]; s1 += red[THREADS + k * NC + c]; }
        slab[L.p_lin1_w + c] = s0;
        if (c == 0) slab[L.p_lin1_b] = s1;
      }
    } else {
      seg_lin1_bwd<NC, THREADS>(rw, n0, a.perm, a.g_out, xfinal, P + L.p_lin1_w, gp_cur, gpT, slab + L.p_lin1_w,
                                slab + L.p_lin1_b, L.nb > 0 ? 1 : 0, red, gkeep);
    }
    dma_land(0);
    if (PTAB || pt) {
      __syncthreads();
    } else {
      build_nbr_in<THREADS>(rw, rp, colo, oeg, false, nbin);
      build_nbr_out<THREADS>(rw, trp, tdsto, teido, 0, nullptr, otg, tout);
      build_nbr_out<THREADS>(rw, mtrp, mtdsto, nullptr, 0, mrp, otm, mout);
      hrcnt = hecnt = uni(build_halo<THREADS>(trp, tdsto, teido, rw, hrow, hedge, hcap, hcounter));
      ercnt = uni(build_export_rows<THREADS>(a.rowptr, a.col, n0, rw, erow, hcap, hcounter));
      if (tid == 0) *hcounter = 0;
      __syncthreads();
      for (int k = tid; k < oeg; k += THREADS) {
        const int j = colo[k];
        if (j < lo || j >= rw.hi) {
          const int pos = atomicAdd(hcounter, 1);
          if (pos < hcap) eedge[pos] = (u16)(elo + k);
        }
      }
      __syncthreads();
      eecnt = uni(*hcounter);
      if (hrcnt > hcap || ercnt > hcap || eecnt > hcap) {
        if (tid == 0) *a.err = 1;
        hrcnt = hecnt = min(hrcnt, hcap); ercnt = min(ercnt, hcap); eecnt = min(eecnt, hcap);
      }
    }
    for (int k = tid; k < ercnt; k += THREADS) bflag_o[(int)erow[k] - lo] = 1;
    if constexpr (NC == 32) scale_g_pre<NC, THREADS>(gpT, mrp, lo, ow);
    if (tid == 0) {
      BwdRec r;
      r.lo = rw.lo; r.hi = rw.hi; r.ow = ow; r.wr = wr; r.wlo = wlo; r.elo = elo; r.ewlo = ewlo; r.weg = weg; r.n0 = n0;
      r.hrcnt = hrcnt; r.hecnt = hecnt; r.ercnt = ercnt; r.eecnt = eecnt;
      r.RA = lds_off(RA); r.gpT = lds_off(gpT); r.gy2T = lds_off(gy2T); r.ge2 = lds_off(ge2); r.ge1 = lds_off(ge1);
      r.gad2 = lds_off(gad2); r.gad1 = lds_off(gad1); r.hTw = lds_off(hTw); r.hT2 = lds_off(hT2); r.hT1 = lds_off(hT1);
      r.asTw = lds_off(asTw); r.asT2 = lds_off(asT2); r.asT1 = lds_off(asT1); r.adTo = lds_off(adTo); r.adT2 = lds_off(adT2);
      r.adT1 = lds_off(adT1); r.alTw = lds_off(alTw); r.alT2 = lds_off(alT2); r.alT1 = lds_off(alT1); r.xG2 = lds_off(xG2);
      r.xG1 = lds_off(xG1); r.gkeep = gkeep ? lds_off(gkeep) : NO_TABLE; r.wlA = lds_off(wlA); r.wlB = lds_off(wlB);
      r.rp = lds_off(rp); r.colo = lds_off(colo); r.trp = lds_off(trp); r.teido = lds_off(teido); r.tdsto = lds_off(tdsto);
      r.mrp = lds_off(mrp); r.mtrp = lds_off(mtrp); r.mtdsto = lds_off(mtdsto); r.nbin = lds_off(nbin); r.tout = lds_off(tout);
      r.mout = lds_off(mout); r.hrow = lds_off(hrow); r.hedge = lds_off(hedge); r.erow = lds_off(erow); r.eedge = lds_off(eedge);
      r.bflag = lds_off(bflag); r.mo1 = mo1 ? lds_off(mo1) : NO_TABLE; r.mxin = mxin ? lds_off(mxin) : NO_TABLE;
      const int* src = reinterpret_cast<const int*>(&r);
#pragma unroll
      for (int k = 0; k < (int)(sizeof(BwdRec) / 4); ++k)
        __hip_atomic_store(myrec + GATRES_UREC_WORDS / 2 + k, src[k], __ATOMIC_RELAXED, __HIP_MEMORY_SCOPE_AGENT);
      asm volatile("s_waitcnt vmcnt(0)" ::: "memory");
    }
    }
    __syncthreads();
    rec_published();
#undef RECP
#define RECP rb_
    auto xout = [&](bool on, const unsigned char* bflag, unsigned t_rows, unsigned t_small) {
      XOut o;
      o.xb = xbuf; o.ep = xc.ep + 1u; o.local = xc.local; o.on = on; o.flag = bflag; o.t_rows = t_rows; o.t_small = t_small;
      return o;
    };
    auto dma_conv2_early = [&](int blk, int w0) {
      if (wave_u < w0) return;
      FRESH_ARGS(); FRESH_BWD();
#define LIST_(T_, N_, I_) I_(lo) I_(hi) T_(float, hTw) T_(float, asTw) T_(float, adTo) T_(float, wlA) I_(wlo) I_(wr) I_(ow)
      REC_LOADS(LIST_);
      REC_PINS(LIST_);
      REC_DEFS(LIST_);
#undef LIST_
      blk = launder_s(blk);
      const float* bs = segbase + (int64_t)blk * SL.bstride;
      dma_copy16<THREADS>(hTw, bs + SL.h2 + (size_t)wlo * NC, wr * NC, w0);
      dma_copy4<THREADS>(asTw, bs + SL.as2 + wlo, wr, w0);
      dma_copy4<THREADS>(adTo, bs + SL.ad2 + lo, ow, w0);
      w_prefetch<NC, 2 * NC, EPI_RESID_MASK, THREADS>(wlA, a.wt + (int64_t)blk * 2 * w + w, nullptr, nullptr, w0);
      vec_prefetch<THREADS>(wlA + A2OFF, P + L.p_block0 + (int64_t)blk * L.p_block_stride + L.c2_as, 2 * NC);
    };
    auto dma_conv2_late = [&](int blk, int w0) {
      if (wave_u < w0) return;
      FRESH_ARGS(); FRESH_BWD();
#define LIST_(T_, N_, I_) I_(lo) I_(hi) T_(float, alTw) I_(ewlo) I_(weg)
      REC_LOADS(LIST_);
      REC_PINS(LIST_);
      REC_DEFS(LIST_);
#undef LIST_
      blk = launder_s(blk);
      const float* bs = segbase + (int64_t)blk * SL.bstride;
      dma_copy4<THREADS>(alTw, bs + SL.al2 + ewlo, weg, w0);
    };
    STAMP();
    const int nb = L.nb;
    for (int b = nb - 1; b >= 0; --b) {
      [[maybe_unused]] const bool xs_on = STAMPS_PTR && a.stamp_cap >= 4096 && seg == 0 && b == nb / 2;
      [[maybe_unused]] int xs_i = 0;
      XSTAMP();
      if (NC != 32 || !xrows || b == nb - 1)
      lds_barrier();
      XSTAMP();
      {
        FRESH_ARGS(); FRESH_BWD();
#define LIST_(T_, N_, I_) I_(lo) I_(hi) T_(float, gpT) T_(const u16, erow) T_(const u16, hrow) I_(ercnt) I_(hrcnt)
        REC_LOADS(LIST_);
        REC_PINS(LIST_);
        REC_DEFS(LIST_);
#undef LIST_
        ++xc.ep;
        if (!xrows || b == nb - 1)
          xch_export2<NC, 0, THREADS>(xc, xbuf, erow, ercnt, gpT, (unsigned)XL.b1, erow, 0, gpT, 0u);
        XSTAMP();
        xch_import2<NC, 0, THREADS>(xc, xbuf, hrow, hrcnt, (unsigned)XL.b1, gpT, hrow, 0, 0u, gpT);
        XSTAMP();
        xch_after<THREADS>(xc, pace);
        XSTAMP();
        lds_barrier();
        XSTAMP();
      }
      STAMP();
      {
        FRESH_ARGS(); FRESH_BWD();
#define LIST_(T_, N_, I_) I_(lo) I_(hi) T_(const u16, nbin) T_(const u16, rp) T_(const u16, colo) T_(float, gy2T) T_(float, hT2) T_(float, alT2) T_(float, asT2) T_(float, adT2) T_(float, ge2) T_(float, gad2) T_(const u16, mout) T_(const u16, mrp) T_(const u16, mtrp) T_(const u16, mtdsto) T_(float, gpT) T_(const unsigned char, bflag) I_(elo) I_(ow)
        REC_LOADS(LIST_);
        REC_PINS(LIST_);
        REC_DEFS(LIST_);
#undef LIST_
        if (NC == 32 && ow64 && wave_u >= 8) {
          const auto rb2_ = rec_fresh<BwdRec>(myrec + GATRES_UREC_WORDS / 2);
          xch_import2_by<NC, 1, 512, THREADS - 512>(xc, xc.ep + 1u, xbuf, LDS_TABLE(const u16, lds_raw, rb2_->hrow), rb2_->hrcnt,
                                                     (unsigned)XL.b2y, gy2T, LDS_TABLE(const u16, lds_raw, rb2_->hedge),
                                                     rb2_->hecnt, (unsigned)XL.b2e, ge2);
        } else
        win_bwd_dst<true, 1, NC, THREADS, NC == 32, NOHUB>(rw, nbin, rp, colo, gy2T, hT2, alT2 + elo, asT2, adT2, ge2 + elo, gad2, mout, mrp,
                                               mtrp, mtdsto, gpT, xout(xedge, bflag, (unsigned)XL.b2y, (unsigned)XL.b2e), elo);
        lds_barrier();
        XSTAMP();
      }
      {
        FRESH_ARGS(); FRESH_BWD();
// ... 155 lines not shown
            win_proj<2 * NC, NC, 1, EPI_RESID_MASK, 1, PW, THREADS, 2 * NC + XPB>(rw, xG1, wlB, gp_nxt, n0, gpT, nullptr, nullptr, nullptr,
                                                                nullptr, gkeep, gkeep, nullptr, bl > 0 ? mxin + bl * ow : nullptr,
                                                                xout(xrows && bl > 0, bflag, (unsigned)XL.b1, 0u), mrp);
          }
      } else {
        FRESH_ARGS(); FRESH_BWD();
#define LIST_(T_, N_, I_) I_(lo) I_(hi) I_(ow) I_(n0) T_(float, xG1) T_(float, wlB) T_(float, gpT) N_(float, gkeep) N_(const unsigned, mxin) T_(const u16, mrp)
        REC_LOADS(LIST_);
        REC_PINS(LIST_);
        REC_DEFS(LIST_);
#undef LIST_
        const float* base = segbase + (int64_t)launder_s(b) * SL.bstride;
        const float* wt1 = a.wt + (int64_t)launder_s(b) * 2 * w;
        seg_proj<2 * NC, NC, 1, EPI_RESID_MASK, THREADS, true, true>(
            rw, xG1, 0, wt1, gp_nxt, n0, gpT, 0, nullptr, nullptr, nullptr, nullptr, 0, nullptr, nullptr,
            (GATRES_DIAG && (a.no_halo & 4)) ? nullptr : gp_cur, n0,
            (b > 0 && !(GATRES_DIAG && (a.no_halo & 4))) ? base + SL.xin : nullptr, 0, wlB, gkeep, gkeep, nullptr,
            (mxin && b > 0) ? mxin + b * ow : nullptr);
        if constexpr (NC == 32) {
          __syncthreads();
          scale_g_pre<NC, THREADS>(gpT, mrp, lo, ow);
        }
      }
#ifndef GATRES_PROBE_NO_BWD_LAND
      dma_land(dw0);
#endif
      XSTAMP();
      STAMP();
      float* t = gp_cur; gp_cur = gp_nxt; gp_nxt = t;
    }
    FRESH_ARGS(); FRESH_BWD();
#define LIST_(T_, N_, I_) I_(lo) I_(hi) N_(float, gkeep) T_(float, gpT) I_(n0)
    REC_LOADS(LIST_);
    REC_PINS(LIST_);
    REC_DEFS(LIST_);
#undef LIST_
    if (assume_local) group_verify_local(grp);
    __syncthreads();
    seg_lin0_bwd<NC, THREADS>(rw, n0, a.perm, gp_cur, a.x, a.mask, slab + L.p_lin0_w, slab + L.p_lin0_b, red,
                              NC == 32 ? gkeep : gpT,
#ifndef GATRES_NO_XKEEP
                              (NC == 32 && keep_ && L.nb > 0 && (ph_ & GATRES_PHASE_FORWARD)) ? mxin : nullptr
#else
                              nullptr
#endif
                              );
    if (a.g_x) {
      constexpr int G = NC / 4;
      const float4 wv = ld4(P + L.p_lin0_w + (tid % G) * 4);
      const int rounds = (rw.hi - rw.lo + THREADS / G - 1) / (THREADS / G);
      for (int it = 0; it < rounds; ++it) {
        int r = rw.lo + it * (THREADS / G) + tid / G;
        const bool valid = r < rw.hi;
        if (!valid) r = rw.hi - 1;
        const float4 xv = ld4(gp_cur + ((size_t)n0 + r) * NC + (tid % G) * 4);
        float d = xv.x * wv.x;
        d = fmaf(xv.y, wv.y, d); d = fmaf(xv.z, wv.z, d); d = fmaf(xv.w, wv.w, d);
        for (int off = G >> 1; off > 0; off >>= 1) d += __shfl_xor(d, off);
        if (valid && (tid % G) == 0) a.g_x[ext_id(a.perm, n0 + r)] = d;
      }
    }
  }
  if (tid == 0) __hip_atomic_store(grp.flags + part * FLAG_STRIDE + 2, xc.ep, __ATOMIC_RELAXED, __HIP_MEMORY_SCOPE_AGENT);
  if (M > 1 && tid == 0 && *a.err) {
    if ((ph_ & GATRES_PHASE_FORWARD) && a.out) a.out[n0] = NAN;
    if (ph_ & GATRES_PHASE_BACKWARD) a.slabs[(int64_t)seg * L.slab_stride + L.p_lin1_b] = NAN;
  }
  if (STAMPS_PTR && blockIdx.x == 0 && threadIdx.x == 0) {
    STAMPS_PTR[a.stamp_cap + 1] = clock64();
    STAMPS_PTR[a.stamp_cap + 2] = wall_clock64();
  }
}

}

extern "C" __attribute__((visibility("hidden"))) int gatres_fused_launch_window(const void* args, int nc, unsigned grid, void* stream) {
  const FusedArgs& a = *static_cast<const FusedArgs*>(args);
  hipStream_t st = gatres_stream(stream);
  switch (nc) {
    case 4: hipLaunchKernelGGL((gatres_window_kernel<4, 1024>), dim3(grid), dim3(1024), 0, st, a); break;
    case 8: hipLaunchKernelGGL((gatres_window_kernel<8, 1024>), dim3(grid), dim3(1024), 0, st, a); break;
    case 16: hipLaunchKernelGGL((gatres_window_kernel<16, 1024>), dim3(grid), dim3(1024), 0, st, a); break;
    case 32: {
      int facts = (a.sym ? 0x200 : 0) | (a.facts & 0x1400) | ((a.ptab && a.ptab_m == a.M) ? 0x800 : 0);
      if ((a.facts & 0x2000) && facts == 0x1e00) facts |= 0x2000;
      if ((a.facts & 0x4000) && (facts & 0x1e00) == 0x1e00 && !a.safe_sync) facts |= 0x4000;
      const int key = a.phases | (a.keep_lds ? 0x100 : 0) | (facts & gatres_knobs()->window_ph_mask) |
                      (a.criterion != GATRES_LOSS_MSE ? 0x8000 : 0);
      if (!gatres_knobs()->window_runtime_phases) {
        switch (key) {
          case 0x5f16: hipLaunchKernelGGL((gatres_window_kernel<32, 1024, 0x5f16>), dim3(grid), dim3(1024), 0, st, a); return gatres_launch_status();
          case 0x7e02: hipLaunchKernelGGL((gatres_window_kernel<32, 1024, 0x7e02>), dim3(grid), dim3(1024), 0, st, a); return gatres_launch_status();
          case 0x5e02: hipLaunchKernelGGL((gatres_window_kernel<32, 1024, 0x5e02>), dim3(grid), dim3(1024), 0, st, a); return gatres_launch_status();
          case 0x5e04: hipLaunchKernelGGL((gatres_window_kernel<32, 1024, 0x5e04>), dim3(grid), dim3(1024), 0, st, a); return gatres_launch_status();
          case 0x1f16: hipLaunchKernelGGL((gatres_window_kernel<32, 1024, 0x1f16>), dim3(grid), dim3(1024), 0, st, a); return gatres_launch_status();
          case 0x1b16: hipLaunchKernelGGL((gatres_window_kernel<32, 1024, 0x1b16>), dim3(grid), dim3(1024), 0, st, a); return gatres_launch_status();
          case 0x0f16: hipLaunchKernelGGL((gatres_window_kernel<32, 1024, 0x0f16>), dim3(grid), dim3(1024), 0, st, a); return gatres_launch_status();
          case 0x0716: hipLaunchKernelGGL((gatres_window_kernel<32, 1024, 0x0716>), dim3(grid), dim3(1024), 0, st, a); return gatres_launch_status();
          case 0x0316: hipLaunchKernelGGL((gatres_window_kernel<32, 1024, 0x0316>), dim3(grid), dim3(1024), 0, st, a); return gatres_launch_status();
          case 0x3e02: hipLaunchKernelGGL((gatres_window_kernel<32, 1024, 0x3e02>), dim3(grid), dim3(1024), 0, st, a); return gatres_launch_status();
          case 0x1e02: hipLaunchKernelGGL((gatres_window_kernel<32, 1024, 0x1e02>), dim3(grid), dim3(1024), 0, st, a); return gatres_launch_status();
          case 0x1e04: hipLaunchKernelGGL((gatres_window_kernel<32, 1024, 0x1e04>), dim3(grid), dim3(1024), 0, st, a); return gatres_launch_status();
          case 0xdf16: hipLaunchKernelGGL((gatres_window_kernel<32, 1024, 0xdf16>), dim3(grid), dim3(1024), 0, st, a); return gatres_launch_status();
          case 0x9f16: hipLaunchKernelGGL((gatres_window_kernel<32, 1024, 0x9f16>), dim3(grid), dim3(1024), 0, st, a); return gatres_launch_status();
          case 0x116: hipLaunchKernelGGL((gatres_window_kernel<32, 1024, 0x116>), dim3(grid), dim3(1024), 0, st, a); return gatres_launch_status();
          default: break;
        }
      }
      hipLaunchKernelGGL((gatres_window_kernel<32, 1024>), dim3(grid), dim3(1024), 0, st, a);
      break;
    }
    default: return GATRES_E_UNSUPPORTED;
  }
  return gatres_launch_status();
}
```

gnn-pressure-estimation_amd/graph_plan.py:

```python
from __future__ import annotations

import ctypes as C
import os
from typing import Dict, Optional, Tuple

import torch

from . import _native


class GraphPlan:

    def __init__(self, edge_index: torch.Tensor, num_nodes: int, device=None, segments: bool = True,
                 merge_upto: int = 64, reorder: Optional[bool] = None):
        if edge_index.dim() != 2 or edge_index.shape[0] != 2:
            raise ValueError(f"edge_index must be [2, E], got {tuple(edge_index.shape)}")
        if edge_index.dtype != torch.int64:
            raise ValueError(f"edge_index must be int64 (PyG convention), got {edge_index.dtype}")
        if num_nodes <= 0:
            raise ValueError("num_nodes must be positive")
        device = torch.device(device if device is not None else edge_index.device)
        lib = _native.load()
        ei_host = edge_index.detach().to("cpu").contiguous()
        E = int(ei_host.shape[1])
        N = int(num_nodes)
        e_gat = C.c_int64(0)
        _native.check(lib.gatres_graph_count_host(ei_host.data_ptr(), E, N, C.byref(e_gat)), "gatres_graph_count_host")
        Eg = int(e_gat.value)
        gflags = C.c_int32(0)
        _native.check(lib.gatres_graph_flags_host(ei_host.data_ptr(), E, N, C.byref(gflags)), "gatres_graph_flags_host")
        self.flags = int(gflags.value)
        i32 = dict(dtype=torch.int32)
        self.num_segments, self.max_segment_nodes = 0, 0
        self.max_segment_edges_gat, self.max_segment_edges_mean = 0, 0
        self.perm_host: Optional[torch.Tensor] = None
        seg = None
        if segments:
            seg = torch.empty(N + 1, **i32)
            ns, mx, mg, mm = C.c_int32(0), C.c_int32(0), C.c_int32(0), C.c_int32(0)
            _native.check(lib.gatres_graph_segments_host(ei_host.data_ptr(), E, N, int(merge_upto), seg.data_ptr(),
                                                         C.byref(ns), C.byref(mx), C.byref(mg), C.byref(mm)),
                          "gatres_graph_segments_host")
            self.num_segments, self.max_segment_nodes = int(ns.value), int(mx.value)
            self.max_segment_edges_gat, self.max_segment_edges_mean = int(mg.value), int(mm.value)
            self.segment_ptr_host = seg[: self.num_segments + 1].clone()

            def windows_of(ei_t):
                win = torch.zeros(28, **i32)
                _native.check(lib.gatres_graph_windows_host(ei_t.data_ptr(), E, N, self.segment_ptr_host.data_ptr(),
                                                            self.num_segments, win.data_ptr()),
                              "gatres_graph_windows_host")
                return [int(v) for v in win]

            self.windows = windows_of(ei_host)
            env = os.environ.get("GATRES_REORDER")
            want = reorder if reorder is not None else (None if env is None else env not in ("0", ""))
            if want is not False and E > 0 and self.max_segment_nodes > 32 and (want or self.max_segment_nodes <= 4096):
                perm = torch.empty(N, **i32)
                _native.check(lib.gatres_graph_reorder_host(ei_host.data_ptr(), E, N, self.segment_ptr_host.data_ptr(),
                                                            self.num_segments, perm.data_ptr()),
                              "gatres_graph_reorder_host")
                old2new = torch.empty(N, dtype=torch.int64)
                old2new[perm.long()] = torch.arange(N, dtype=torch.int64)
                ei_new = old2new[ei_host].contiguous()
                win_new = windows_of(ei_new)
                if want is True or win_new[6] < 0.9 * self.windows[6]:
                    self.perm_host, self.windows, ei_host = perm, win_new, ei_new
        else:
            self.windows = [0] * 28
        host = {
            "rowptr": torch.empty(N + 1, **i32), "col": torch.empty(Eg, **i32),
            "t_rowptr": torch.empty(N + 1, **i32), "t_eid": torch.empty(Eg, **i32), "t_dst": torch.empty(Eg, **i32),
            "m_rowptr": torch.empty(N + 1, **i32), "m_col": torch.empty(max(E, 1), **i32),
            "mt_rowptr": torch.empty(N + 1, **i32), "mt_dst": torch.empty(max(E, 1), **i32),
        }
        _native.check(lib.gatres_graph_build_host(ei_host.data_ptr(), E, N, *[t.data_ptr() for t in host.values()]),
                      "gatres_graph_build_host")
        self.num_nodes, self.num_edges_gat, self.num_edges_mean = N, Eg, E
        self.device = device
        self._host = host if segments else None
        self._part_tables: Dict[int, Tuple[torch.Tensor, int]] = {}
        self._bound: Dict[int, "_native.GatresGraph"] = {}
        import threading
        self._bind_lock = threading.Lock()
        self.arrays: Dict[str, torch.Tensor] = {k: v.to(device) for k, v in host.items()}
        seg_dev_ptr = None
        if segments:
            self.arrays["seg_ptr"] = self.segment_ptr_host.to(device)
            seg_dev_ptr = self.arrays["seg_ptr"].data_ptr()
        perm_dev_ptr = None
        if self.perm_host is not None:
            self.arrays["perm"] = self.perm_host.to(device)
            perm_dev_ptr = self.arrays["perm"].data_ptr()
        self.c = _native.GatresGraph(N, Eg, E, self.num_segments, *[self.arrays[k].data_ptr() for k in host.keys()],
                                     seg_dev_ptr, self.max_segment_nodes, self.max_segment_edges_gat,
                                     self.max_segment_edges_mean, self.flags, (C.c_int32 * 21)(*self.windows[:21]), 0,
                                     perm_dev_ptr,
                                     (C.c_int32 * 7)(*self.windows[21:28]), 0, None, 0, 0)

    def bound(self, cmodel_ref) -> "_native.GatresGraph":
        if self._host is None or self.num_segments <= 0 or os.environ.get("GATRES_NO_PART_TABLES"):
            return self.c
        lib = _native.load()
        m = int(lib.gatres_fused_cus_per_segment(cmodel_ref, C.byref(self.c)))
        if m < 2 or m > 8 or self.max_segment_nodes > 65535:
            return self.c
        with self._bind_lock:
            got = self._bound.get(m)
            if got is not None:
                return got
            ptrs = [self._host[k].data_ptr() for k in ("rowptr", "col", "t_rowptr", "t_eid", "t_dst", "m_rowptr", "m_col",
                                                       "mt_rowptr", "mt_dst")]
            stride = C.c_int64(0)
            rc = lib.gatres_graph_part_tables_host(*ptrs, self.segment_ptr_host.data_ptr(), self.num_segments, m, None, 0,
                                                   C.byref(stride))
            if rc != 0:
                self._bound[m] = self.c
                return self.c
            words = torch.zeros(self.num_segments * m * int(stride.value), dtype=torch.int32)
            _native.check(lib.gatres_graph_part_tables_host(*ptrs, self.segment_ptr_host.data_ptr(), self.num_segments, m,
                                                            words.data_ptr(), int(stride.value), C.byref(stride)),
                          "gatres_graph_part_tables_host")
            dev = words.to(self.device)
            self._part_tables[m] = (dev, int(stride.value))
            c = _native.GatresGraph.from_buffer_copy(self.c)
            c.part_tables, c.part_tables_m, c.part_tables_stride = dev.data_ptr(), m, int(stride.value)
            self._bound[m] = c
            return c

    def bind(self, cmodel_ref) -> None:
        self.bound(cmodel_ref)

    def ref(self, cmodel_ref=None):
        return C.byref(self.c if cmodel_ref is None else self.bound(cmodel_ref))

    def window_rows(self, parts: int) -> int:
        return self.windows[3 * (parts - 2)] if 2 <= parts <= 8 else 0

    def halo_edges(self, parts: int) -> int:
        return self.windows[21 + parts - 2] if 2 <= parts <= 8 else 0

    def node_ptr_for(self, nodes_per_graph) -> torch.Tensor:
        off = [0]
        for n in nodes_per_graph:
            off.append(off[-1] + int(n))
        if off[-1] != self.num_nodes:
            raise ValueError("nodes_per_graph does not add up to num_nodes")
        return torch.tensor(off, dtype=torch.int32, device=self.device)


class PlanCache:

    def __init__(self, max_entries: int = 16, segments: bool = True):
        self.max_entries = max_entries
        self.segments = segments
        self._by_hash: Dict[Tuple[int, int, int, str], GraphPlan] = {}
        self._by_identity: Dict[Tuple[int, int, int, int, str], GraphPlan] = {}

    def clear(self) -> None:
        self._by_hash.clear()
        self._by_identity.clear()

    def get(self, edge_index: torch.Tensor, num_nodes: int) -> GraphPlan:
        _native.require_gpu_tensor(edge_index, "edge_index", torch.int64)
        ident = (edge_index.data_ptr(), edge_index._version, int(edge_index.shape[1]), int(num_nodes),
                 str(edge_index.device))
        plan = self._by_identity.get(ident)
        if plan is not None and getattr(plan, "_src_ref", None) is edge_index:
            return plan
        lib = _native.load()
        h = torch.zeros(1, dtype=torch.int64, device=edge_index.device)
        _native.check(lib.gatres_edge_index_hash(edge_index.data_ptr(), int(edge_index.shape[1]), h.data_ptr(),
                                                 _native.current_stream(edge_index.device)), "gatres_edge_index_hash")
        key = (int(h.item()), int(edge_index.shape[1]), int(num_nodes), str(edge_index.device))
        plan = self._by_hash.get(key)
        if plan is None:
            if len(self._by_hash) >= self.max_entries:
                self.clear()
            plan = GraphPlan(edge_index, num_nodes, segments=self.segments)
            self._by_hash[key] = plan
        plan._src_ref = edge_index
        self._by_identity = {ident: plan}
        return plan
```

include/gatres.h:

```cpp
#ifndef GATRES_H
#define GATRES_H

#include <stdint.h>

#ifdef __cplusplus
extern "C" {
#endif

#define GATRES_ABI_VERSION 9

#define GATRES_E_BADARG      (-1)
#define GATRES_E_UNSUPPORTED (-2)
#define GATRES_E_GRAPH       (-3)

#define GATRES_DTYPE_F32  0
#define GATRES_DTYPE_BF16 1

typedef struct gatres_graph {
  int32_t num_nodes;
  int32_t num_edges_gat;
  int32_t num_edges_mean;
  int32_t num_segments;
  const int32_t* rowptr;
  const int32_t* col;
  const int32_t* t_rowptr;
  const int32_t* t_eid;
  const int32_t* t_dst;
  const int32_t* m_rowptr;
  const int32_t* m_col;
  const int32_t* mt_rowptr;
  const int32_t* mt_dst;
  const int32_t* seg_ptr;
  int32_t max_segment_nodes;
  int32_t max_segment_edges_gat;
  int32_t max_segment_edges_mean;
  int32_t flags;
  int32_t window[7][3];
  int32_t reserved2;
  const int32_t* perm;
  int32_t halo[7];
  int32_t reserved3;
  const int32_t* part_tables;
  int32_t part_tables_m;
  int32_t part_tables_stride;
} gatres_graph_t;

enum {
  GATRES_PT_MAGIC = 0, GATRES_PT_M, GATRES_PT_N0, GATRES_PT_N, GATRES_PT_E0, GATRES_PT_EM0, GATRES_PT_T0, GATRES_PT_MT0,
  GATRES_PT_LO, GATRES_PT_HI, GATRES_PT_WLO, GATRES_PT_WHI, GATRES_PT_ELO, GATRES_PT_OEG, GATRES_PT_EWLO, GATRES_PT_WEG,
  GATRES_PT_MELO, GATRES_PT_OEM, GATRES_PT_TLO, GATRES_PT_OTG, GATRES_PT_MTLO, GATRES_PT_OTM,
  GATRES_PT_F_IMG, GATRES_PT_F_IMG_WORDS, GATRES_PT_F_HLIST, GATRES_PT_F_HCNT, GATRES_PT_F_ELIST, GATRES_PT_F_ECNT,
  GATRES_PT_B_IMG, GATRES_PT_B_IMG_WORDS, GATRES_PT_B_HROW, GATRES_PT_B_HRCNT, GATRES_PT_B_HEDGE, GATRES_PT_B_HECNT,
  GATRES_PT_B_EROW, GATRES_PT_B_ERCNT, GATRES_PT_B_EEDGE, GATRES_PT_B_EECNT,
  GATRES_PT_HEADER = 48
};
#define GATRES_PT_MAGIC_VALUE 0x47545031

#define GATRES_GRAPH_SYMMETRIC 1

#define GATRES_GRAPH_DEG_LE32 2

#define GATRES_GRAPH_DEG_LE6 4

int gatres_graph_count_host(const int64_t* edge_index_host, int64_t num_edges, int64_t num_nodes,
                            int64_t* num_edges_gat_out);
int gatres_graph_build_host(const int64_t* edge_index_host, int64_t num_edges, int64_t num_nodes,
                            int32_t* rowptr, int32_t* col, int32_t* t_rowptr, int32_t* t_eid, int32_t* t_dst,
                            int32_t* m_rowptr, int32_t* m_col, int32_t* mt_rowptr, int32_t* mt_dst);

int gatres_graph_flags_host(const int64_t* edge_index_host, int64_t num_edges, int64_t num_nodes, int32_t* flags_out);

int gatres_graph_part_tables_host(const int32_t* rowptr, const int32_t* col, const int32_t* t_rowptr, const int32_t* t_eid,
                                  const int32_t* t_dst, const int32_t* m_rowptr, const int32_t* m_col,
                                  const int32_t* mt_rowptr, const int32_t* mt_dst, const int32_t* seg_ptr,
                                  int32_t num_segments, int32_t m, int32_t* out, int64_t stride_words,
                                  int64_t* stride_words_out);

int gatres_graph_segments_host(const int64_t* edge_index_host, int64_t num_edges, int64_t num_nodes,
                               int32_t merge_upto, int32_t* seg_ptr_host, int32_t* num_segments_out,
                               int32_t* max_segment_nodes_out, int32_t* max_segment_edges_gat_out,
                               int32_t* max_segment_edges_mean_out);

int gatres_graph_windows_host(const int64_t* edge_index, int64_t num_edges, int64_t num_nodes, const int32_t* seg_ptr,
                              int32_t num_segments, int32_t* out28);

int gatres_graph_reorder_host(const int64_t* edge_index_host, int64_t num_edges, int64_t num_nodes,
                              const int32_t* seg_ptr_host, int32_t num_segments, int32_t* perm_new2old_host);

int64_t gatres_lz4_decompress_host(const uint8_t* src, int64_t src_len, uint8_t* dst, int64_t dst_cap);

int gatres_knobs_reload(void);

int gatres_edge_index_hash(const int64_t* edge_index, int64_t num_edges, uint64_t* hash_out, void* stream);


int gatres_lin0_fwd(const float* x, const uint8_t* mask, const float* w, const float* b, float* out,
                    int32_t num_nodes, int32_t nc, void* stream);

int gatres_proj_attn_fwd(const float* x, const float* W, const float* att_src, const float* att_dst,
                         float* h, float* a_src, float* a_dst,
                         int32_t num_nodes, int32_t K, int32_t H, int32_t C, void* stream);

int gatres_gat_aggregate_fwd(const gatres_graph_t* g, const float* h, const float* a_src, const float* a_dst,
                             const float* bias, float* out, float* alpha,
                             int32_t H, int32_t C, int32_t apply_relu, void* stream);

int gatres_mean_residual_relu_fwd(const gatres_graph_t* g, const float* y, const float* x0, float* out,
                                  int32_t C, void* stream);

int gatres_lin1_fwd(const float* x, const float* w, const float* b, float* out,
                    int32_t num_nodes, int32_t nc, void* stream);


int gatres_reduce_slabs(const float* slabs, int32_t num_slabs, int64_t slab_stride, int64_t count,
                        float* out, void* stream);

int gatres_lin1_bwd(const float* g_out, const float* x, const float* w, float* g_x,
                    float* slab_w, float* slab_b, int32_t num_slabs, int64_t slab_stride,
                    int32_t num_nodes, int32_t nc, int32_t relu_mask, void* stream);

int gatres_mean_bwd(const gatres_graph_t* g, const float* g_pre, float* g_y, int32_t C, void* stream);

int gatres_gat_aggregate_bwd_dst(const gatres_graph_t* g, const float* g_out, const float* h,
                                 const float* alpha, const float* a_src, const float* a_dst,
                                 float* g_e, float* g_a_dst, int32_t H, int32_t C, void* stream);

int gatres_gat_aggregate_bwd_src(const gatres_graph_t* g, const float* g_out, const float* alpha,
                                 const float* g_e, const float* g_a_dst, const float* att_src,
                                 const float* att_dst, float* g_h, float* g_a_src,
                                 int32_t H, int32_t C, void* stream);

int gatres_proj_bwd_dx(const float* g_h, const float* Wt, const float* resid, const float* relu_ref,
                       float* g_x, int32_t num_nodes, int32_t K, int32_t HC, void* stream);

int gatres_proj_bwd_dw(const float* g_h, const float* x, float* slab_W, int32_t num_slabs,
                       int64_t slab_stride, int32_t num_nodes, int32_t K, int32_t HC, void* stream);

int gatres_conv_param_grads(const float* h, const float* g_a_src, const float* g_a_dst, const float* g_out,
                            float* slab_att_src, float* slab_att_dst, float* slab_bias, int32_t num_slabs,
                            int64_t slab_stride, int32_t num_nodes, int32_t H, int32_t C, void* stream);

int gatres_lin0_bwd(const float* g, const float* x, const uint8_t* mask, float* slab_w, float* slab_b,
                    int32_t num_slabs, int64_t slab_stride, int32_t num_nodes, int32_t nc, void* stream);

int gatres_permute_f32(const float* src, const int32_t* perm, float* dst, int32_t num_nodes, int32_t scatter,
                       void* stream);
int gatres_gather_u8(const uint8_t* src, const int32_t* perm, uint8_t* dst, int32_t num_nodes, void* stream);

int gatres_transpose_conv_weights(const float* params, float* wt, int32_t num_blocks, int32_t nc, void* stream);


int gatres_mask_generate(const int32_t* node_ptr, int32_t num_graphs, double mask_rate, uint64_t seed,
                         const uint64_t* step_counter, uint8_t* mask, void* stream);

int gatres_stage_batch_mask(const float* x_src, const float* y_src, float* x_dst, float* y_dst, int64_t num_nodes,
                            const int32_t* node_ptr, int32_t num_graphs, double mask_rate, uint64_t seed,
                            const uint64_t* step_counter, uint8_t* mask, void* stream);

int gatres_stage_rows_mask(const float* data, const int64_t* rows, int32_t nodes_per_graph, float* x_dst, float* y_dst,
// ... 50 lines not shown
                      int64_t slab_stride, int num_nodes, int nc, int dtype, void* stream);
int gatres_t_lin1_fwd(const void* x, const float* w, const float* b, float* out, int num_nodes, int nc, int dtype,
                      void* stream);
int gatres_t_lin1_bwd(const float* g_out, const void* x, const float* w, void* g_x, float* slab_w, float* slab_b,
                      int num_slabs, int64_t slab_stride, int num_nodes, int nc, int relu_mask, int dtype, void* stream);
int gatres_t_conv_param_grads(const void* h, const float* g_a_src, const float* g_a_dst, const void* g_out,
                              float* slab_att_src, float* slab_att_dst, float* slab_bias, int num_slabs,
                              int64_t slab_stride, int num_nodes, int H, int C, int dtype, void* stream);
int gatres_t_conv_partials(const void* g_h, const void* x, float* slab_W, int w_slabs, int64_t slab_stride, int num_nodes,
                           int K, int HC, const void* h, const float* g_a_src, const float* g_a_dst, const void* g_out,
                           float* slab_att_src, float* slab_att_dst, float* slab_bias, int num_slabs, int H, int C, int dtype,
                           void* stream);
int gatres_convert_conv_weights_bf16(const float* params, void* wb, int num_blocks, int nc, void* stream);

int gatres_t_proj_attn_fwd(const void* x, const void* W, const float* att_src, const float* att_dst, void* h, float* a_src,
                           float* a_dst, int num_nodes, int K, int H, int C, int dtype, void* stream);
int gatres_t_proj_bwd_dx(const void* g_h, const void* Wt, const void* resid, const void* relu_ref, void* g_x, int num_nodes,
                         int K, int HC, int dtype, void* stream);
int gatres_t_proj_bwd_dw(const void* g_h, const void* x, float* slab_W, int num_slabs, int64_t slab_stride, int num_nodes,
                         int K, int HC, int dtype, void* stream);

typedef struct gatres_model {
  int32_t num_blocks;
  int32_t nc;
  int32_t act_dtype;
  int32_t flags;
} gatres_model_t;

#define GATRES_MODEL_INFERENCE 1

int gatres_blocked_supported(const gatres_model_t* m, const gatres_graph_t* g);
int gatres_bf16_agg_proj_fwd(const gatres_graph_t* g, const void* h, const float* a_src, const float* a_dst,
                             const float* bias, void* o, float* alpha, const void* W_next, const float* att_src_next,
                             const float* att_dst_next, void* h_next, float* a_src_next, float* a_dst_next, int32_t nc,
                             void* stream);
int gatres_bf16_mean_proj_fwd(const gatres_graph_t* g, const void* y, const void* x0, void* x_next, const void* W_next,
                              const float* att_src_next, const float* att_dst_next, void* h_next, float* a_src_next,
                              float* a_dst_next, int32_t nc, void* stream);
int gatres_bf16_src_dx_bwd(const gatres_graph_t* g, const void* g_out, const float* alpha, const float* g_e,
                           const float* g_a_dst, const float* att_src, const float* att_dst, void* g_h, float* g_a_src,
                           const void* Wt, const void* resid, const void* relu_ref, void* g_x, int32_t H, int32_t nc,
                           void* stream);

int64_t gatres_param_count(int32_t num_blocks, int32_t nc);
int64_t gatres_saved_floats(const gatres_model_t* m, const gatres_graph_t* g);
int64_t gatres_scratch_floats(const gatres_model_t* m, const gatres_graph_t* g);
int32_t gatres_num_slabs(const gatres_model_t* m, int32_t num_nodes);

int gatres_model_forward(const gatres_model_t* m, const gatres_graph_t* g, const float* params,
                         const float* x, const uint8_t* mask, float* out, float* saved, float* scratch,
                         void* stream);

int gatres_model_backward(const gatres_model_t* m, const gatres_graph_t* g, const float* params,
                          const float* x, const uint8_t* mask, const float* g_out, const float* saved,
                          float* scratch, float* grads, float* g_x, void* stream);

int gatres_model_forward_per_op(const gatres_model_t* m, const gatres_graph_t* g, const float* params,
                                const float* x, const uint8_t* mask, float* out, float* saved, float* scratch,
                                void* stream);
int gatres_model_backward_per_op(const gatres_model_t* m, const gatres_graph_t* g, const float* params,
                                 const float* x, const uint8_t* mask, const float* g_out, const float* saved,
                                 float* scratch, float* grads, float* g_x, void* stream);

#define GATRES_PART_FIRST  1
#define GATRES_PART_LAST   2
#define GATRES_PART_REDUCE 4
int gatres_model_backward_per_op_part(const gatres_model_t* m, const gatres_graph_t* g, const float* params,
                                      const float* x, const uint8_t* mask, const float* g_out, const float* saved,
                                      float* scratch, float* grads, float* g_x, int32_t b_hi, int32_t b_lo,
                                      int32_t flags, void* stream);

int gatres_model_reduce_grads(const gatres_model_t* m, const gatres_graph_t* g, float* scratch, float* grads, void* stream);

#define GATRES_PHASE_LOSS 16
#define GATRES_PHASE_LOSS_MAE 32
#define GATRES_PHASE_LOSS_SCE 64
int gatres_fused_supported(const gatres_model_t* m, const gatres_graph_t* g);
int gatres_fused_cus_per_segment(const gatres_model_t* m, const gatres_graph_t* g);
int gatres_fused_window_kernel(const gatres_model_t* m, const gatres_graph_t* g);
int gatres_fused_reset_sync(const gatres_model_t* m, const gatres_graph_t* g, float* scratch, void* stream);
int gatres_fused_serialize(void* stream);
int gatres_probe_xcd_dispatch(void* stream);
int64_t gatres_fused_status_offset(const gatres_model_t* m, const gatres_graph_t* g);
int gatres_fused_set_stamps(uint64_t* stamps, int32_t capacity);
int gatres_fused_prepare_backward(const gatres_model_t* m, const gatres_graph_t* g, const float* params,
                                  float* scratch, void* stream);
int gatres_fused_run(const gatres_model_t* m, const gatres_graph_t* g, const float* params, const float* x,
                     const uint8_t* mask, const float* y, float* out, float* g_out, float* loss_part, float* g_x,
                     float* saved, float* scratch, int32_t phases, void* stream);
int gatres_fused_param_grads(const gatres_model_t* m, const gatres_graph_t* g, const float* saved, float* scratch,
                             void* stream);
int gatres_fused_finish(const gatres_model_t* m, const gatres_graph_t* g, float* scratch, float* grads,
                        const float* loss_part, float* loss, int32_t do_adam, float* params, float* exp_avg,
                        float* exp_avg_sq, uint64_t* step_counter, double lr, double beta1, double beta2,
                        double eps, double weight_decay, float grad_scale, void* stream);
int gatres_fused_finish_hp(const gatres_model_t* m, const gatres_graph_t* g, float* scratch, float* grads,
                           const float* loss_part, float* loss, int32_t do_adam, float* params, float* exp_avg,
                           float* exp_avg_sq, uint64_t* step_counter, double lr, double beta1, double beta2,
                           double eps, double weight_decay, const double* hparams, float grad_scale,
                           const int32_t* mask_node_ptr, int32_t mask_graphs, double mask_rate, uint64_t mask_seed,
                           uint8_t* mask_next, void* stream);
int gatres_fused_finish_folds(const gatres_model_t* m, const gatres_graph_t* g);
int gatres_fused_param_grads_finish(const gatres_model_t* m, const gatres_graph_t* g, const float* saved, float* scratch,
                                    float* grads, const float* loss_part, float* loss, int32_t do_adam, float* params,
                                    float* exp_avg, float* exp_avg_sq, uint64_t* step_counter, double lr, double beta1,
                                    double beta2, double eps, double weight_decay, const double* hparams,
                                    float grad_scale, int32_t block_lo, int32_t block_hi, void* stream);

typedef struct gatres_autoclip {
  double* log;
  double* sorted[2];
  uint64_t* ctl;
  double* partials;
  double* norm_out;
  double* clip_out;
  double* coef_out;
  int64_t capacity;
  int32_t partials_cap;
  int32_t reserved;
  double percentile;
} gatres_autoclip_t;

int32_t gatres_autoclip_partials(int64_t count);

int gatres_autoclip_adam_step(float* params, const float* grads, float* exp_avg, float* exp_avg_sq,
                              uint64_t* step_counter, int64_t count, double lr, double beta1, double beta2, double eps,
                              double weight_decay, float grad_scale, const gatres_autoclip_t* ac, void* stream);

#define GATRES_PHASE_MASK     1
#define GATRES_PHASE_FORWARD  2
#define GATRES_PHASE_BACKWARD 4
#define GATRES_PHASE_ADAM     8
#define GATRES_PHASE_ALL      15

typedef struct gatres_train_step {
  gatres_model_t model;
  const gatres_graph_t* graph;
  float* params;
  float* grads;
  float* exp_avg;
  float* exp_avg_sq;
  uint64_t* step_counter;
  const float* x;
  const float* y;
  uint8_t* mask;
  const int32_t* node_ptr;
  int32_t num_graphs;
  int32_t phases;
  double mask_rate;
  uint64_t seed;
  float* out;
  float* g_out;
  float* loss;
  float* saved;
  float* scratch;
  double lr, beta1, beta2, eps, weight_decay;
  float grad_scale;
  int32_t flags;
  const double* hparams;
  int32_t block_lo, block_hi;
  uint8_t* mask_next;
  const gatres_autoclip_t* autoclip;
} gatres_train_step_t;
#define GATRES_FLAG_PER_OP 1
#define GATRES_FLAG_GRADS_DEFERRED 4
#define GATRES_FLAG_GRADS_ONLY 8
// ... 71 lines not shown
```

Before: 104,700 snapshots/s.

## Precompute per-partition window LDS records and flag tables on host

Moves the computation of the forward and backward window LDS layout records, plus the per-row edge flags, out of the fused kernel and into the host-built partition tables. The tables are now keyed per (M, nc, num_blocks) and validated per flavour. The kernel can then load ready-made records instead of having thread 0 compute them, publish them through global memory and synchronise on that publication. This adds host-side table building and a key/flavour check, and falls back to the non-table path when a flavour does not validate.

```diff
diff --git a/gnn-pressure-estimation_amd/_native.py b/gnn-pressure-estimation_amd/_native.py
--- a/gnn-pressure-estimation_amd/_native.py
+++ b/gnn-pressure-estimation_amd/_native.py
@@ -26,7 +26,7 @@
                 ("mt_dst", C.c_void_p), ("seg_ptr", C.c_void_p), ("max_segment_nodes", C.c_int32),
                 ("max_segment_edges_gat", C.c_int32), ("max_segment_edges_mean", C.c_int32), ("flags", C.c_int32),
                 ("window", C.c_int32 * 21), ("reserved2", C.c_int32), ("perm", C.c_void_p),
-                ("halo", C.c_int32 * 7), ("reserved3", C.c_int32),
+                ("halo", C.c_int32 * 7), ("part_tables_key", C.c_int32),
                 ("part_tables", C.c_void_p), ("part_tables_m", C.c_int32), ("part_tables_stride", C.c_int32)]
 
 
@@ -58,6 +58,7 @@
     "gatres_graph_build_host": (C.c_int, [_P, _I64, _I64] + [_P] * 9),
     "gatres_graph_flags_host": (C.c_int, [_P, _I64, _I64, C.POINTER(_I32)]),
     "gatres_graph_part_tables_host": (C.c_int, [_P] * 10 + [_I32, _I32, _P, _I64, C.POINTER(_I64)]),
+    "gatres_graph_part_records_host": (C.c_int, [_P, _I32, _I32, _I64, _I32, _I32, C.POINTER(_I32)]),
     "gatres_graph_segments_host": (C.c_int, [_P, _I64, _I64, _I32, _P] + [C.POINTER(_I32)] * 4),
     "gatres_graph_windows_host": (C.c_int, [_P, _I64, _I64, _P, _I32, _P]),
     "gatres_graph_reorder_host": (C.c_int, [_P, _I64, _I64, _P, _I32, _P]),
@@ -69,6 +70,7 @@
     "gatres_probe_xcd_dispatch": (C.c_int, [_P]),
     "gatres_knobs_reload": (C.c_int, []),
     "gatres_fused_status_offset": (_I64, [_MP, _GP]),
+    "gatres_fused_record_offset": (_I64, [_MP, _GP, C.POINTER(_I64)]),
     "gatres_lin0_fwd": (C.c_int, [_P, _P, _P, _P, _P, _I32, _I32, _P]),
     "gatres_proj_attn_fwd": (C.c_int, [_P] * 7 + [_I32] * 4 + [_P]),
     "gatres_gat_aggregate_fwd": (C.c_int, [_GP] + [_P] * 6 + [_I32] * 3 + [_P]),
diff --git a/gnn-pressure-estimation_amd/csrc/gatres_layout.h b/gnn-pressure-estimation_amd/csrc/gatres_layout.h
--- a/gnn-pressure-estimation_amd/csrc/gatres_layout.h
+++ b/gnn-pressure-estimation_amd/csrc/gatres_layout.h
@@ -204,3 +204,151 @@
   S.total = (S.total + 63) & ~(int64_t)63;
   return S;
 }
+
+constexpr int GATRES_WIN_LDS_BYTES = 163840;
+constexpr int GATRES_WIN_THREADS = 1024;
+constexpr int NO_TABLE = INT32_MIN;
+struct FwdRec {
+  int lo, hi, ow, wr, oeg, elo, hcnt, ecnt;
+  int xA, xB, wlA, wlB, hA, hB, hBw, y2T, al2L, sa2, sa1, sd2, sd1, fflag, hlist, elist, nbin, mbin, rp, colo, mrp, mcolo, mo1, mxin;
+};
+struct BwdRec {
+  int lo, hi, ow, wr, wlo, elo, ewlo, weg, n0, hrcnt, hecnt, ercnt, eecnt;
+  int RA, gpT, gy2T, ge2, ge1, gad2, gad1, hTw, hT2, hT1, asTw, asT2, asT1, adTo, adT2, adT1, alTw, alT2, alT1, xG2, xG1, gkeep,
+      wlA, wlB, rp, colo, trp, teido, tdsto, mrp, mtrp, mtdsto, nbin, tout, mout, hrow, hedge, erow, eedge, bflag, mo1, mxin;
+};
+static_assert(sizeof(FwdRec) <= 4 * (GATRES_UREC_WORDS / 2) && sizeof(BwdRec) <= 4 * (GATRES_UREC_WORDS / 2), "record halves");
+struct WinPart {
+  int n0, lo, hi, wlo, whi, elo, oeg, ewlo, weg, oem, otg, otm;
+};
+struct WinFlavour {
+  int nc, nb;
+  int xpf, xpb;
+  bool keep;
+};
+constexpr int GATRES_WIN_FLAVOURS = 3;
+static constexpr __host__ __device__ int win_xpf(int nc, bool nohub) {
+#ifdef GATRES_NO_XPAD
+  return 0 * nc * nohub;
+#else
+  return (nc == 32 && nohub) ? 4 : 0;
+#endif
+}
+static constexpr __host__ __device__ int win_xpb(int nc, bool keep) {
+#ifdef GATRES_NO_XPAD
+  return 0 * nc * keep;
+#else
+  return (nc == 32 && keep) ? 4 : 0;
+#endif
+}
+static inline __host__ __device__ WinFlavour win_flavour(int nc, int nb, int index) {
+  WinFlavour f;
+  f.nc = nc; f.nb = nb; f.keep = (index & 2) != 0;
+  f.xpf = win_xpf(nc, (index & 1) != 0);
+  f.xpb = win_xpb(nc, f.keep);
+  return f;
+}
+static inline __host__ __device__ int win_even(int v) { return (v + 1) & ~1; }
+static inline __host__ __device__ int win_wlb(int nc) { return (2 * nc * (2 * nc + 4) + 4 * nc + 3) & ~3; }
+static inline __host__ __device__ long long win_keep_bytes(int nb, int ow) { return (12LL * nb * ow + 15) & ~15LL; }
+static inline __host__ __device__ int win_lds_top(int nb, int ow, bool keep) {
+  return GATRES_WIN_LDS_BYTES - (keep ? (int)win_keep_bytes(nb, ow) : 0);
+}
+static inline __host__ __device__ int win_mo1_off(int top, int lo) { return top - 8 * lo; }
+static inline __host__ __device__ int win_mxin_off(int top, int nb, int ow, int lo) { return top + 8 * nb * ow - 4 * lo; }
+static inline __host__ __device__ FwdRec win_fwd_record(const WinFlavour& f, const WinPart& g, int hcnt, int ecnt, int* img_bytes,
+                                                        int* hcap) {
+  const int nc = f.nc, lo = g.lo, ow = g.hi - g.lo, wlo = g.wlo, wr = g.whi - g.wlo;
+  FwdRec r;
+  r.lo = g.lo; r.hi = g.hi; r.ow = ow; r.wr = wr; r.oeg = g.oeg; r.elo = g.elo; r.hcnt = hcnt; r.ecnt = ecnt;
+  const int hAw = 0;
+  const int hBw = hAw + 4 * wr * 2 * nc;
+  const int saw = hBw + 4 * wr * nc;
+  const int sdo = saw + 4 * ((wr * 2 + 3) & ~3);
+  const int xAo = sdo + 4 * ((ow * 2 + 3) & ~3);
+  const int xBo = xAo + 4 * ow * (nc + f.xpf);
+  r.wlA = (xBo + 4 * ow * (2 * nc + f.xpf) + 15) & ~15;
+  r.wlB = r.wlA + 4 * win_wlb(nc);
+  int tp = r.wlB + 4 * win_wlb(nc);
+  const int rpo = tp;   tp += 2 * win_even(ow + 1);
+  r.colo = tp;          tp += 2 * win_even(g.oeg);
+  const int mrpo = tp;  tp += 2 * win_even(ow + 1);
+  r.mcolo = tp;         tp += 2 * win_even(g.oem);
+  tp = (tp + 15) & ~15;
+  r.nbin = tp;          tp += 16 * ow;
+  r.mbin = tp;          tp += 16 * ow;
+  *img_bytes = tp - rpo;
+  r.hlist = tp + 4;
+  const int top = win_lds_top(f.nb, ow, f.keep);
+  const int fflag_o = top - ((ow + 15) & ~15);
+  const int room = (fflag_o - r.hlist) / 4;
+  *hcap = (room > 0 ? room : 0) & ~1;
+  r.elist = r.hlist + 2 * *hcap;
+  r.fflag = fflag_o - lo;
+  r.hA = hAw - 4 * wlo * 2 * nc; r.hB = hBw - 4 * wlo * nc; r.hBw = hBw;
+  r.y2T = hAw - 4 * wlo * nc; r.al2L = hAw + 4 * wr * nc;
+  r.sa2 = saw - 4 * wlo * 2; r.sa1 = saw - 4 * wlo;
+  r.sd2 = sdo - 4 * lo * 2;  r.sd1 = sdo - 4 * lo;
+  r.xA = xAo - 4 * lo * (nc + f.xpf);
+  r.xB = xBo - 4 * lo * (2 * nc + f.xpf);
+  r.rp = rpo - 2 * lo; r.mrp = mrpo - 2 * lo;
+  r.mo1 = f.keep ? win_mo1_off(top, lo) : NO_TABLE;
+  r.mxin = f.keep ? win_mxin_off(top, f.nb, ow, lo) : NO_TABLE;
+  return r;
+}
+static inline __host__ __device__ BwdRec win_bwd_record(const WinFlavour& f, const WinPart& g, int hrcnt, int hecnt, int ercnt,
+                                                        int eecnt, int* img_bytes, int* hcap) {
+  const int nc = f.nc, lo = g.lo, ow = g.hi - g.lo, wlo = g.wlo, wr = g.whi - g.wlo, weg = g.weg, ewlo = g.ewlo;
+  BwdRec r;
+  r.lo = g.lo; r.hi = g.hi; r.ow = ow; r.wr = wr; r.wlo = wlo; r.elo = g.elo; r.ewlo = ewlo; r.weg = weg; r.n0 = g.n0;
+  r.hrcnt = hrcnt; r.hecnt = hecnt; r.ercnt = ercnt; r.eecnt = eecnt;
+  const int RAw = 4 * 3 * GATRES_WIN_THREADS;
+  const int gew = RAw + 4 * wr * 2 * nc;
+  const int gado = gew + 4 * 2 * win_even(weg);
+  r.hTw = gado + 4 * ((ow * 2 + 3) & ~3);
+  r.asTw = r.hTw + 4 * wr * 2 * nc;
+  r.adTo = r.asTw + 4 * ((wr * 2 + 3) & ~3);
+  r.alTw = r.adTo + 4 * ((ow * 2 + 3) & ~3);
+  const int xGo = r.alTw + 4 * 2 * win_even(weg);
+  const int gko = xGo + 4 * ow * (2 * nc + f.xpb);
+  r.wlA = (gko + (f.keep ? 4 * ow * nc : 0) + 15) & ~15;
+  r.wlB = r.wlA + 4 * win_wlb(nc);
+  int tp = r.wlB + 4 * win_wlb(nc);
+  const int rpo = tp;    tp += 2 * win_even(ow + 1);
+  r.colo = tp;           tp += 2 * win_even(g.oeg);
+  const int trpo = tp;   tp += 2 * win_even(ow + 1);
+  r.teido = tp;          tp += 2 * win_even(g.otg);
+  r.tdsto = tp;          tp += 2 * win_even(g.otg);
+  const int mrpw = tp;   tp += 2 * win_even(wr + 1);
+  const int mtrpo = tp;  tp += 2 * win_even(ow + 1);
+  r.mtdsto = tp;         tp += 2 * win_even(g.otm);
+  tp = (tp + 15) & ~15;
+  r.nbin = tp;           tp += 16 * ow;
+  r.tout = tp;           tp += 32 * ow;
+  r.mout = tp;           tp += 32 * ow;
+  *img_bytes = tp - rpo;
+  r.hrow = tp + 4;
+  const int top = win_lds_top(f.nb, ow, f.keep);
+  const int bflag_o = top - ((ow + 15) & ~15);
+  const int room = (bflag_o - r.hrow) / 8;
+  *hcap = (room > 0 ? room : 0) & ~1;
+  r.hedge = r.hrow + 2 * *hcap;
+  r.erow = r.hedge + 2 * *hcap;
+  r.eedge = r.erow + 2 * *hcap;
+  r.bflag = bflag_o - lo;
+  r.rp = rpo - 2 * lo; r.trp = trpo - 2 * lo; r.mrp = mrpw - 2 * wlo; r.mtrp = mtrpo - 2 * lo;
+  r.RA = RAw - 4 * wlo * 2 * nc;
+  r.gpT = RAw - 4 * wlo * nc;
+  r.gy2T = RAw + 4 * wr * nc - 4 * wlo * nc;
+  r.ge2 = gew - 4 * ewlo;       r.ge1 = gew - 4 * ewlo * 2;
+  r.gad2 = gado - 4 * lo;       r.gad1 = gado - 4 * lo * 2;
+  r.hT2 = r.hTw - 4 * wlo * nc; r.hT1 = r.hTw - 4 * wlo * 2 * nc;
+  r.asT2 = r.asTw - 4 * wlo;    r.asT1 = r.asTw - 4 * wlo * 2;
+  r.adT2 = r.adTo - 4 * lo;     r.adT1 = r.adTo - 4 * lo * 2;
+  r.alT2 = r.alTw - 4 * ewlo;   r.alT1 = r.alTw - 4 * ewlo * 2;
+  r.xG2 = xGo - 4 * lo * (nc + f.xpb);  r.xG1 = xGo - 4 * lo * (2 * nc + f.xpb);
+  r.gkeep = f.keep ? gko - 4 * lo * nc : NO_TABLE;
+  r.mo1 = f.keep ? win_mo1_off(top, lo) : NO_TABLE;
+  r.mxin = f.keep ? win_mxin_off(top, f.nb, ow, lo) : NO_TABLE;
+  return r;
+}
diff --git a/gnn-pressure-estimation_amd/csrc/graph_plan.hip b/gnn-pressure-estimation_amd/csrc/graph_plan.hip
--- a/gnn-pressure-estimation_amd/csrc/graph_plan.hip
+++ b/gnn-pressure-estimation_amd/csrc/graph_plan.hip
@@ -1,7 +1,9 @@
 #include <algorithm>
+#include <cstring>
 #include <vector>
 
 #include "gatres_common.h"
+#include "gatres_layout.h"
 
 namespace {
 
@@ -321,6 +323,8 @@
       hdr[GATRES_PT_WLO] = g.wlo; hdr[GATRES_PT_WHI] = g.whi; hdr[GATRES_PT_ELO] = g.elo; hdr[GATRES_PT_OEG] = g.oeg;
       hdr[GATRES_PT_EWLO] = g.ewlo; hdr[GATRES_PT_WEG] = g.weg; hdr[GATRES_PT_MELO] = g.melo; hdr[GATRES_PT_OEM] = g.oem;
       hdr[GATRES_PT_TLO] = g.tlo; hdr[GATRES_PT_OTG] = g.otg; hdr[GATRES_PT_MTLO] = g.mtlo; hdr[GATRES_PT_OTM] = g.otm;
+      hdr[GATRES_PT_F_REC] = GATRES_PT_HEADER; hdr[GATRES_PT_B_REC] = GATRES_PT_HEADER + GATRES_PT_REC_STRIDE / 2;
+      img.resize((size_t)2 * GATRES_PT_REC_FLAVOURS * GATRES_PT_REC_STRIDE, 0);
       size_t from = img.size();
       hdr[GATRES_PT_F_IMG] = GATRES_PT_HEADER + (int)(img.size() / 2);
       put(rpo, even_i(ow + 1)); put(colo, even_i(g.oeg)); put(mrpo, even_i(ow + 1)); put(mcolo, even_i(g.oem));
@@ -340,6 +344,13 @@
       put_list(f_hlist, GATRES_PT_F_HLIST, GATRES_PT_F_HCNT); put_list(f_elist, GATRES_PT_F_ELIST, GATRES_PT_F_ECNT);
       put_list(b_hrow, GATRES_PT_B_HROW, GATRES_PT_B_HRCNT);   put_list(b_hedge, GATRES_PT_B_HEDGE, GATRES_PT_B_HECNT);
       put_list(b_erow, GATRES_PT_B_EROW, GATRES_PT_B_ERCNT);   put_list(b_eedge, GATRES_PT_B_EEDGE, GATRES_PT_B_EECNT);
+      auto put_flags = [&](const std::vector<uint16_t>& rows, int off_field) {
+        std::vector<uint16_t> fl((size_t)((ow + 15) & ~15) / 2, 0);
+        for (uint16_t rr : rows) fl[(rr - g.lo) / 2] |= (uint16_t)(1u << (8 * ((rr - g.lo) & 1)));
+        hdr[off_field] = GATRES_PT_HEADER + (int)(img.size() / 2);
+        put(fl, (int)fl.size());
+      };
+      put_flags(f_elist, GATRES_PT_F_FLAGS); put_flags(b_erow, GATRES_PT_B_FLAGS);
       const int64_t total_words = GATRES_PT_HEADER + (int64_t)img.size() / 2;
       need = std::max(need, total_words);
       if (out) {
@@ -352,6 +363,49 @@
     }
   }
   *stride_words_out = (need + 3) & ~(int64_t)3;
+  return 0;
+}
+
+extern "C" int gatres_graph_part_records_host(int32_t* tables, int32_t num_segments, int32_t M, int64_t stride_words,
+                                              int32_t nc, int32_t num_blocks, int32_t* key_out) {
+  if (!tables || num_segments <= 0 || M < 2 || M > 8 || !key_out ||
+      stride_words < GATRES_PT_HEADER + GATRES_PT_REC_FLAVOURS * GATRES_PT_REC_STRIDE)
+    return GATRES_E_BADARG;
+  *key_out = 0;
+  if (nc != 32 || num_blocks < 0 || num_blocks > 255) return GATRES_E_UNSUPPORTED;
+  static_assert(GATRES_PT_REC_STRIDE == GATRES_UREC_WORDS && GATRES_PT_REC_FLAVOURS == GATRES_WIN_FLAVOURS, "record slots");
+  int ok_mask = ((1 << GATRES_WIN_FLAVOURS) - 1) << 1;
+  for (int64_t sp = 0; sp < (int64_t)num_segments * M; ++sp) {
+    int32_t* rec = tables + sp * stride_words;
+    if (rec[GATRES_PT_MAGIC] != GATRES_PT_MAGIC_VALUE || rec[GATRES_PT_M] != M || rec[GATRES_PT_F_REC] != GATRES_PT_HEADER ||
+        rec[GATRES_PT_B_REC] != GATRES_PT_HEADER + GATRES_PT_REC_STRIDE / 2)
+      return GATRES_E_BADARG;
+    WinPart g;
+    g.n0 = rec[GATRES_PT_N0]; g.lo = rec[GATRES_PT_LO]; g.hi = rec[GATRES_PT_HI]; g.wlo = rec[GATRES_PT_WLO];
+    g.whi = rec[GATRES_PT_WHI]; g.elo = rec[GATRES_PT_ELO]; g.oeg = rec[GATRES_PT_OEG]; g.ewlo = rec[GATRES_PT_EWLO];
+    g.weg = rec[GATRES_PT_WEG]; g.oem = rec[GATRES_PT_OEM]; g.otg = rec[GATRES_PT_OTG]; g.otm = rec[GATRES_PT_OTM];
+    const int ow = g.hi - g.lo, flag_bytes = (ow + 15) & ~15;
+    for (int k = 1; k <= GATRES_WIN_FLAVOURS; ++k) {
+      const WinFlavour f = win_flavour(nc, num_blocks, k);
+      int img_bytes = 0, hcap = 0;
+      const FwdRec rf = win_fwd_record(f, g, rec[GATRES_PT_F_HCNT], rec[GATRES_PT_F_ECNT], &img_bytes, &hcap);
+      bool ok = rec[GATRES_PT_F_IMG_WORDS] * 4 == img_bytes && rf.hcnt <= hcap && rf.ecnt <= hcap &&
+                rf.elist + 2 * hcap <= rf.fflag + g.lo && rf.fflag + g.lo >= rf.hlist;
+      const BwdRec rb = win_bwd_record(f, g, rec[GATRES_PT_B_HRCNT], rec[GATRES_PT_B_HECNT], rec[GATRES_PT_B_ERCNT],
+                                       rec[GATRES_PT_B_EECNT], &img_bytes, &hcap);
+      ok = ok && rec[GATRES_PT_B_IMG_WORDS] * 4 == img_bytes && rb.hrcnt <= hcap && rb.hecnt <= hcap && rb.ercnt <= hcap &&
+           rb.eecnt <= hcap && rb.eedge + 2 * hcap <= rb.bflag + g.lo && rb.bflag + g.lo >= rb.hrow;
+      ok = ok && win_lds_top(num_blocks, ow, f.keep) - flag_bytes >= 0;
+      if (!ok) ok_mask &= ~(1 << k);
+      int32_t* slot = rec + GATRES_PT_HEADER + (k - 1) * GATRES_PT_REC_STRIDE;
+      std::fill(slot, slot + GATRES_PT_REC_STRIDE, 0);
+      std::memcpy(slot, &rf, sizeof rf);
+      std::memcpy(slot + GATRES_PT_REC_STRIDE / 2, &rb, sizeof rb);
+    }
+  }
+  const int32_t key = GATRES_PT_KEY(nc, num_blocks, ok_mask);
+  for (int64_t sp = 0; sp < (int64_t)num_segments * M; ++sp) tables[sp * stride_words + GATRES_PT_REC_KEY] = key;
+  *key_out = key;
   return 0;
 }
 
diff --git a/gnn-pressure-estimation_amd/csrc/k_fused_dev.h b/gnn-pressure-estimation_amd/csrc/k_fused_dev.h
--- a/gnn-pressure-estimation_amd/csrc/k_fused_dev.h
+++ b/gnn-pressure-estimation_amd/csrc/k_fused_dev.h
@@ -11,7 +11,7 @@
 typedef float f32x4 __attribute__((ext_vector_type(4)));
 typedef unsigned short u16;
 
-constexpr int LDS_BYTES = 163840;
+constexpr int LDS_BYTES = GATRES_WIN_LDS_BYTES;
 constexpr int MAXD = 6;
 
 struct FusedArgs {
@@ -1627,7 +1627,6 @@
          2LL * (3 * even(ow + 2) + 3 * even(ge) + even(wr + 2) + even(gm)) + 64 + 8LL * (hl + 4) + 80LL * ow + 16 + ow + 16;
 }
 
-__host__ __device__ inline long long win_keep_bytes(int nb, int ow) { return (12LL * nb * ow + 15) & ~15LL; }
 
 __device__ __forceinline__ void lds_barrier() { asm volatile("s_waitcnt lgkmcnt(0)\n\ts_barrier" ::: "memory"); }
 
diff --git a/gnn-pressure-estimation_amd/csrc/k_fused_host.hip b/gnn-pressure-estimation_amd/csrc/k_fused_host.hip
--- a/gnn-pressure-estimation_amd/csrc/k_fused_host.hip
+++ b/gnn-pressure-estimation_amd/csrc/k_fused_host.hip
@@ -517,6 +517,15 @@
   }
   a.keep_lds = (phases & GATRES_PHASE_FORWARD) && (phases & GATRES_PHASE_BACKWARD) && !gatres_knobs()->fused_no_keep &&
            window_kernel_fits(a.L, g, a.M, true) ? 1 : 0;
+  if (a.ptab && m->nc == 32) {
+    const int flavour = (a.keep_lds ? 2 : 0) | ((a.facts & gatres_knobs()->window_ph_mask & 0x400) ? 1 : 0);
+    const int key = g->part_tables_key;
+    const bool bound = a.L.nb <= 255 && key == GATRES_PT_KEY(m->nc, a.L.nb, (key >> 16) & 0xf);
+    if (flavour != 0 && bound) {
+      if ((key >> 16) & (1 << flavour)) a.facts |= 0x800;
+      else a.ptab = nullptr;
+    }
+  }
   a.flags = reinterpret_cast<unsigned*>(scratch + a.L.sc_flags);
   a.err = reinterpret_cast<int*>(fused_status(scratch, a.L));
   a.part_slabs = scratch + a.L.sc_part_slabs;
@@ -565,6 +574,14 @@
   for (int b = 0; b < cus && rr; ++b) rr = (h[b] & 0xfu) == (h[b & 7] & 0xfu) && h[b] != 0xffffffffu;
   g_xcd_rr[dev].store(rr ? 2 : 1, std::memory_order_release);
   return rr ? 1 : 0;
+}
+
+extern "C" int64_t gatres_fused_record_offset(const gatres_model_t* m, const gatres_graph_t* g, int64_t* words_out) {
+  Layout L;
+  if (words_out) *words_out = 0;
+  if (!gatres_fused_supported(m, g) || !make_layout_g(m, g, &L) || L.xch_stride <= 0) return -1;
+  if (words_out) *words_out = L.sc_wb - L.sc_urec;
+  return L.sc_urec;
 }
 
 extern "C" int64_t gatres_fused_status_offset(const gatres_model_t* m, const gatres_graph_t* g) {
diff --git a/gnn-pressure-estimation_amd/csrc/k_window.hip b/gnn-pressure-estimation_amd/csrc/k_window.hip
--- a/gnn-pressure-estimation_amd/csrc/k_window.hip
+++ b/gnn-pressure-estimation_amd/csrc/k_window.hip
@@ -26,17 +26,6 @@
   const KArgs ka_ = kargs_fresh();                                                                            \
   [[maybe_unused]] const auto& L = ka_->L; [[maybe_unused]] const auto& SL = ka_->SL; [[maybe_unused]] const auto& XL = ka_->XL
 
-struct FwdRec {
-  int lo, hi, ow, wr, oeg, elo, hcnt, ecnt;
-  int xA, xB, wlA, wlB, hA, hB, hBw, y2T, al2L, sa2, sa1, sd2, sd1, fflag, hlist, elist, nbin, mbin, rp, colo, mrp, mcolo, mo1, mxin;
-};
-struct BwdRec {
-  int lo, hi, ow, wr, wlo, elo, ewlo, weg, n0, hrcnt, hecnt, ercnt, eecnt;
-  int RA, gpT, gy2T, ge2, ge1, gad2, gad1, hTw, hT2, hT1, asTw, asT2, asT1, adTo, adT2, adT1, alTw, alT2, alT1, xG2, xG1, gkeep,
-      wlA, wlB, rp, colo, trp, teido, tdsto, mrp, mtrp, mtdsto, nbin, tout, mout, hrow, hedge, erow, eedge, bflag, mo1, mxin;
-};
-static_assert(sizeof(FwdRec) <= 4 * (GATRES_UREC_WORDS / 2) && sizeof(BwdRec) <= 4 * (GATRES_UREC_WORDS / 2), "record halves");
-constexpr int NO_TABLE = INT_MIN;
 template <class R>
 __device__ __forceinline__ const __attribute__((address_space(4))) R* rec_fresh(const int* words) {
   auto p = (const __attribute__((address_space(4))) R*)(unsigned long long)words;
@@ -61,9 +50,6 @@
 #define REC_PINS(LIST, ...) do {} while (0)
 #endif
 #define REC_DEFS(LIST) LIST(REC_DEF_T, REC_DEF_N, REC_DEF_I) [[maybe_unused]] const Rows rw = {lo, hi}
-__device__ __forceinline__ u16* align16(u16* p) {
-  return reinterpret_cast<u16*>((reinterpret_cast<uintptr_t>(p) + 15) & ~(uintptr_t)15);
-}
 
 template <int NC, int THREADS>
 __device__ __forceinline__ void scale_g_pre(float* gpT, const u16* mrp, int lo, int ow) {
@@ -86,12 +72,7 @@
   constexpr bool NOSAVE = PH >= 0 && (PH & 0x2000) != 0 && (PH & 0xff) == GATRES_PHASE_FORWARD;
   constexpr bool XLOCAL = PH >= 0 && (PH & 0x4000) != 0;
   const bool mse_ = PH < 0 ? a.criterion == GATRES_LOSS_MSE : (PH & 0x8000) == 0;
-#ifdef GATRES_NO_XPAD
-  constexpr int XPF = 0, XPB = 0;
-#else
-  constexpr int XPF = (NC == 32 && NOHUB) ? 4 : 0;
-  constexpr int XPB = (NC == 32 && PH >= 0 && (PH & 0x100) != 0) ? 4 : 0;
-#endif
+  constexpr int XPF = win_xpf(NC, NOHUB), XPB = win_xpb(NC, PH >= 0 && (PH & 0x100) != 0);
   __shared__ __attribute__((aligned(16))) unsigned char lds_raw[LDS_BYTES];
   float* ldsf = reinterpret_cast<float*>(lds_raw);
   const Layout& L = a.L;
@@ -163,9 +144,8 @@
   static_assert(B1OFF + 2 * NC <= WLB && B2OFF + NC <= WLB && A2OFF + 2 * NC <= WLB && A1OFF + 4 * NC <= WLB, "W slot tails");
   const float* P = a.params;
   float* sc = a.scratch;
-  unsigned char* lds_top = lds_raw + LDS_BYTES - (keep_ ? win_keep_bytes(L.nb, ow) : 0);
-  unsigned long long* mo1 = keep_ ? reinterpret_cast<unsigned long long*>(lds_top) - lo : nullptr;
-  unsigned* mxin = keep_ ? reinterpret_cast<unsigned*>(lds_top + 8LL * L.nb * ow) - lo : nullptr;
+  const int top_ = win_lds_top(L.nb, ow, keep_);
+  unsigned* mxin = keep_ ? LDS_TABLE(unsigned, lds_raw, win_mxin_off(top_, L.nb, ow, lo)) : nullptr;
   [[maybe_unused]] int stamp_i = 0;
   STAMP();
   if (STAMPS_PTR && blockIdx.x == 0 && threadIdx.x == 0) STAMPS_PTR[a.stamp_cap] = clock64();
@@ -214,61 +194,69 @@
   float* dml = ldsf + 64;
   float xk[2] = {0.f, 0.f};
 
-  int* const myrec = a.urec + (size_t)blockIdx.x * GATRES_UREC_WORDS;
-  auto lds_off = [&](const void* p) { return (int)(reinterpret_cast<const unsigned char*>(p) - lds_raw); };
+  constexpr int FLAVOUR = ((PH >= 0 && (PH & 0x100) != 0) ? 2 : 0) | (NOHUB ? 1 : 0);
+  int* const urec_w = a.urec + (size_t)blockIdx.x * GATRES_UREC_WORDS;
+  static_assert(!PTAB || (FLAVOUR >= 1 && FLAVOUR <= GATRES_WIN_FLAVOURS), "the part tables carry no record of this flavour");
+  static_assert(THREADS == GATRES_WIN_THREADS, "win_bwd_record sizes the backward's `red` region for this workgroup");
+  const int* const myrec = PTAB ? pt + (GATRES_PT_HEADER + (FLAVOUR - 1) * GATRES_UREC_WORDS) : urec_w;
+  auto win_part = [&]() {
+    WinPart g;
+    g.n0 = n0; g.lo = rw.lo; g.hi = rw.hi; g.wlo = wlo; g.whi = whi; g.elo = elo; g.oeg = oeg; g.ewlo = ewlo; g.weg = weg;
+    g.oem = oem; g.otg = otg; g.otm = otm;
+    return g;
+  };
+  auto win_flav = [&]() {
+    WinFlavour f;
+    f.nc = NC; f.nb = L.nb; f.xpf = XPF; f.xpb = XPB; f.keep = keep_;
+    return f;
+  };
 
   if (ph_ & GATRES_PHASE_FORWARD) {
     constexpr bool xreg = NC == 32;
     {
-    float* hAw = ldsf;
-    float* hBw = hAw + (size_t)wr * 2 * NC;
-    float* saw = hBw + (size_t)wr * NC;
-    float* sdo = saw + (size_t)((wr * 2 + 3) & ~3);
-    float* xAo = sdo + (size_t)((ow * 2 + 3) & ~3);
-    float* xBo = xAo + (size_t)ow * (NC + XPF);
-    float* wlA = reinterpret_cast<float*>(lds_raw + ((reinterpret_cast<unsigned char*>(xBo + (size_t)ow * (2 * NC + XPF)) - lds_raw + 15) & ~15));
-    float* wlB = wlA + WLB;
-    u16* tp = reinterpret_cast<u16*>(wlB + WLB);
-    u16* rpo = tp;             tp += even(ow + 1);
-    u16* colo = tp;            tp += even(oeg);
-    u16* mrpo = tp;            tp += even(ow + 1);
-    u16* mcolo = tp;           tp += even(oem);
-    tp = align16(tp);
-    u16* nbin = tp;            tp += 8 * ow;
-    u16* mbin = tp;            tp += 8 * ow;
-    int* hcounter = reinterpret_cast<int*>(tp);
-    const u16* f_img_end = tp;
-    u16* hlist = tp + 2;
-    unsigned char* fflag_o = lds_top - ((ow + 15) & ~15);
-    const int hcap = max(0, (int)((fflag_o - reinterpret_cast<unsigned char*>(hlist)) / 4)) & ~1;
-    u16* elist = hlist + hcap;
-    const unsigned char* fflag = fflag_o - lo;
-    float* hA = hAw - wlo * 2 * NC;
-    float* hB = hBw - wlo * NC;
-    float* sa2 = saw - wlo * 2;  float* sa1 = saw - wlo;
-    float* sd2 = sdo - lo * 2;   float* sd1 = sdo - lo;
-    float* xA = xAo - lo * (NC + XPF);
-    float* xB = xBo - lo * (2 * NC + XPF);
-    const u16* rp = rpo - lo;  const u16* mrp = mrpo - lo;
+    FwdRec r;
+    int hcap = 0, img_bytes = 0;
+    if constexpr (PTAB) {
+      const auto q = rec_fresh<FwdRec>(myrec);
+      r.xA = q->xA; r.wlA = q->wlA; r.rp = q->rp; r.hlist = q->hlist; r.elist = q->elist; r.fflag = q->fflag;
+    } else {
+      r = win_fwd_record(win_flav(), win_part(), 0, 0, &img_bytes, &hcap);
+    }
+    float* xA = LDS_TABLE(float, lds_raw, r.xA);
+    float* wlA = LDS_TABLE(float, lds_raw, r.wlA);
+    u16* rpo = LDS_TABLE(u16, lds_raw, r.rp + 2 * lo);
+    u16* hlist = LDS_TABLE(u16, lds_raw, r.hlist);
+    u16* elist = LDS_TABLE(u16, lds_raw, r.elist);
+    unsigned char* fflag_o = lds_raw + (r.fflag + lo);
     int hcnt = 0, ecnt = 0;
-    if (PTAB || pt) {
+    if constexpr (PTAB) {
       hcnt = H(GATRES_PT_F_HCNT); ecnt = H(GATRES_PT_F_ECNT);
-      if (H(GATRES_PT_F_IMG_WORDS) * 2 != (int)(f_img_end - rpo) || hcnt > hcap || ecnt > hcap) {
-        if (tid == 0) *a.err = 1;
-        hcnt = min(hcnt, hcap); ecnt = min(ecnt, hcap);
-      } else {
-        dma_copy4<THREADS>(reinterpret_cast<float*>(rpo), reinterpret_cast<const float*>(pt + H(GATRES_PT_F_IMG)),
-                           H(GATRES_PT_F_IMG_WORDS), 0);
-      }
+      dma_copy4<THREADS>(reinterpret_cast<float*>(rpo), reinterpret_cast<const float*>(pt + H(GATRES_PT_F_IMG)),
+                         H(GATRES_PT_F_IMG_WORDS), 0);
       dma_copy4<THREADS>(reinterpret_cast<float*>(hlist), reinterpret_cast<const float*>(pt + H(GATRES_PT_F_HLIST)), (hcnt + 1) / 2, 0);
       dma_copy4<THREADS>(reinterpret_cast<float*>(elist), reinterpret_cast<const float*>(pt + H(GATRES_PT_F_ELIST)), (ecnt + 1) / 2, 0);
+      dma_copy4<THREADS>(reinterpret_cast<float*>(fflag_o), reinterpret_cast<const float*>(pt + H(GATRES_PT_F_FLAGS)),
+                         ((ow + 15) & ~15) / 4, 0);
     } else {
-      copy_rowptr16<THREADS>(rpo, a.rowptr, n0 + lo, ow, e0 + elo);
-      copy_idx16<THREADS>(colo, a.col, e0 + elo, oeg, n0);
-      copy_rowptr16<THREADS>(mrpo, a.m_rowptr, n0 + lo, ow, em0 + melo);
-      copy_idx16<THREADS>(mcolo, a.m_col, em0 + melo, oem, n0);
-    }
-    for (int k = tid; k < ((ow + 15) & ~15) / 4; k += THREADS) reinterpret_cast<unsigned*>(fflag_o)[k] = 0u;
+      if (pt) {
+        hcnt = H(GATRES_PT_F_HCNT); ecnt = H(GATRES_PT_F_ECNT);
+        if (H(GATRES_PT_F_IMG_WORDS) * 4 != img_bytes || hcnt > hcap || ecnt > hcap) {
+          if (tid == 0) *a.err = 1;
+          hcnt = min(hcnt, hcap); ecnt = min(ecnt, hcap);
+        } else {
+          dma_copy4<THREADS>(reinterpret_cast<float*>(rpo), reinterpret_cast<const float*>(pt + H(GATRES_PT_F_IMG)),
+                             H(GATRES_PT_F_IMG_WORDS), 0);
+        }
+        dma_copy4<THREADS>(reinterpret_cast<float*>(hlist), reinterpret_cast<const float*>(pt + H(GATRES_PT_F_HLIST)), (hcnt + 1) / 2, 0);
+        dma_copy4<THREADS>(reinterpret_cast<float*>(elist), reinterpret_cast<const float*>(pt + H(GATRES_PT_F_ELIST)), (ecnt + 1) / 2, 0);
+      } else {
+        copy_rowptr16<THREADS>(rpo, a.rowptr, n0 + lo, ow, e0 + elo);
+        copy_idx16<THREADS>(LDS_TABLE(u16, lds_raw, r.colo), a.col, e0 + elo, oeg, n0);
+        copy_rowptr16<THREADS>(LDS_TABLE(u16, lds_raw, r.mrp + 2 * lo), a.m_rowptr, n0 + lo, ow, em0 + melo);
+        copy_idx16<THREADS>(LDS_TABLE(u16, lds_raw, r.mcolo), a.m_col, em0 + melo, oem, n0);
+      }
+      for (int k = tid; k < ((ow + 15) & ~15) / 4; k += THREADS) reinterpret_cast<unsigned*>(fflag_o)[k] = 0u;
+    }
     float* xcur = segbase + SL.xin;
     if (L.nb > 0) {
       const float* pb0 = P + L.p_block0;
@@ -294,36 +282,36 @@
     }
     dma_land(0);
     __syncthreads();
-    if (!PTAB && !pt) {
-      build_nbr_in<THREADS>(rw, rp, colo, oeg, false, nbin);
-      build_nbr_in<THREADS>(rw, mrp, mcolo, oem, true, mbin);
-      hcnt = uni(build_halo<THREADS>(rp, colo, nullptr, rw, hlist, nullptr, hcap, hcounter));
-      ecnt = uni(build_export_rows<THREADS>(a.t_rowptr, a.t_dst, n0, rw, elist, hcap, hcounter));
-      if (hcnt > hcap || ecnt > hcap) {
-        if (tid == 0) *a.err = 1;
-        hcnt = min(hcnt, hcap); ecnt = min(ecnt, hcap);
-      }
-    }
-    if (xreg)
-      for (int k = tid; k < ecnt; k += THREADS) fflag_o[(int)elist[k] - lo] = 1;
-    if (tid == 0) {
-      FwdRec r;
-      r.lo = rw.lo; r.hi = rw.hi; r.ow = ow; r.wr = wr; r.oeg = oeg; r.elo = elo; r.hcnt = hcnt; r.ecnt = ecnt;
-      r.xA = lds_off(xA); r.xB = lds_off(xB); r.wlA = lds_off(wlA); r.wlB = lds_off(wlB); r.hA = lds_off(hA); r.hB = lds_off(hB);
-      r.hBw = lds_off(hBw); r.y2T = lds_off(hAw - wlo * NC); r.al2L = lds_off(hAw + (size_t)wr * NC);
-      r.sa2 = lds_off(sa2); r.sa1 = lds_off(sa1); r.sd2 = lds_off(sd2); r.sd1 = lds_off(sd1); r.fflag = lds_off(fflag);
-      r.hlist = lds_off(hlist); r.elist = lds_off(elist); r.nbin = lds_off(nbin); r.mbin = lds_off(mbin);
-      r.rp = lds_off(rp); r.colo = lds_off(colo); r.mrp = lds_off(mrp); r.mcolo = lds_off(mcolo);
-      r.mo1 = mo1 ? lds_off(mo1) : NO_TABLE; r.mxin = mxin ? lds_off(mxin) : NO_TABLE;
-      const int* src = reinterpret_cast<const int*>(&r);
+    if constexpr (!PTAB) {
+      if (!pt) {
+        const u16* rp = LDS_TABLE(const u16, lds_raw, r.rp);
+        const u16* mrp = LDS_TABLE(const u16, lds_raw, r.mrp);
+        int* hcounter = reinterpret_cast<int*>(hlist - 2);
+        build_nbr_in<THREADS>(rw, rp, LDS_TABLE(u16, lds_raw, r.colo), oeg, false, LDS_TABLE(u16, lds_raw, r.nbin));
+        build_nbr_in<THREADS>(rw, mrp, LDS_TABLE(u16, lds_raw, r.mcolo), oem, true, LDS_TABLE(u16, lds_raw, r.mbin));
+        hcnt = uni(build_halo<THREADS>(rp, LDS_TABLE(u16, lds_raw, r.colo), nullptr, rw, hlist, nullptr, hcap, hcounter));
+        ecnt = uni(build_export_rows<THREADS>(a.t_rowptr, a.t_dst, n0, rw, elist, hcap, hcounter));
+        if (hcnt > hcap || ecnt > hcap) {
+          if (tid == 0) *a.err = 1;
+          hcnt = min(hcnt, hcap); ecnt = min(ecnt, hcap);
+        }
+      }
+      if (xreg)
+        for (int k = tid; k < ecnt; k += THREADS) fflag_o[(int)elist[k] - lo] = 1;
+      if (tid == 0) {
+        r.hcnt = hcnt; r.ecnt = ecnt;
+        const int* src = reinterpret_cast<const int*>(&r);
 #pragma unroll
-      for (int k = 0; k < (int)(sizeof(FwdRec) / 4); ++k)
-        __hip_atomic_store(myrec + k, src[k], __ATOMIC_RELAXED, __HIP_MEMORY_SCOPE_AGENT);
-      asm volatile("s_waitcnt vmcnt(0)" ::: "memory");
-    }
-    }
-    __syncthreads();
-    rec_published();
+        for (int k = 0; k < (int)(sizeof(FwdRec) / 4); ++k)
+          __hip_atomic_store(urec_w + k, src[k], __ATOMIC_RELAXED, __HIP_MEMORY_SCOPE_AGENT);
+        asm volatile("s_waitcnt vmcnt(0)" ::: "memory");
+      }
+    }
+    }
+    if constexpr (!PTAB) {
+      __syncthreads();
+      rec_published();
+    }
     auto xout = [&](bool on, const unsigned char* flag, long long t_rows, long long t_small) {
       XOut x;
       x.xb = xbuf; x.ep = xc.ep + 1u; x.local = xc.local; x.on = on; x.flag = flag;
@@ -660,78 +648,67 @@
     float* gp_nxt = sc + L.sc_gpb;
     float* const slab = a.part_slabs + ((int64_t)seg * M + part) * L.slab_stride;
     {
-    float* RAw = red + 3 * THREADS;
-    float* gew = RAw + (size_t)wr * 2 * NC;
-    float* gado = gew + 2 * (size_t)even(weg);
-    float* hTw = gado + (size_t)((ow * 2 + 3) & ~3);
-    float* asTw = hTw + (size_t)wr * 2 * NC;
-    float* adTo = asTw + (size_t)((wr * 2 + 3) & ~3);
-    float* alTw = adTo + (size_t)((ow * 2 + 3) & ~3);
-    float* xGo = alTw + 2 * (size_t)even(weg);
-    float* gko = xGo + (size_t)ow * (2 * NC + XPB);
-    float* wlA = reinterpret_cast<float*>(lds_raw + ((reinterpret_cast<unsigned char*>(gko + (keep_ ? (size_t)ow * NC : 0)) - lds_raw + 15) & ~15));
-    float* wlB = wlA + WLB;
-    u16* tp = reinterpret_cast<u16*>(wlB + WLB);
-    u16* rpo = tp;             tp += even(ow + 1);
-    u16* colo = tp;            tp += even(oeg);
-    u16* trpo = tp;            tp += even(ow + 1);
-    u16* teido = tp;           tp += even(otg);
-    u16* tdsto = tp;           tp += even(otg);
-    u16* mrpw = tp;            tp += even(wr + 1);
-    u16* mtrpo = tp;           tp += even(ow + 1);
-    u16* mtdsto = tp;          tp += even(otm);
-    tp = align16(tp);
-    u16* nbin = tp;            tp += 8 * ow;
-    u16* tout = tp;            tp += 16 * ow;
-    u16* mout = tp;            tp += 16 * ow;
-    int* hcounter = reinterpret_cast<int*>(tp);
-    const u16* b_img_end = tp;
-    u16* hrow = tp + 2;
-    unsigned char* bflag_o = lds_top - ((ow + 15) & ~15);
-    const int hcap = max(0, (int)((bflag_o - reinterpret_cast<unsigned char*>(hrow)) / 8)) & ~1;
-    u16* hedge = hrow + hcap;
-    u16* erow = hedge + hcap;
-    u16* eedge = erow + hcap;
+    BwdRec r;
+    int hcap = 0, img_bytes = 0;
+    if constexpr (PTAB) {
+      const auto q = rec_fresh<BwdRec>(myrec + GATRES_UREC_WORDS / 2);
+      r.hTw = q->hTw; r.asTw = q->asTw; r.adTo = q->adTo; r.alTw = q->alTw; r.wlA = q->wlA; r.gpT = q->gpT; r.gkeep = q->gkeep;
+      r.rp = q->rp; r.mrp = q->mrp; r.hrow = q->hrow; r.hedge = q->hedge; r.erow = q->erow; r.eedge = q->eedge; r.bflag = q->bflag;
+    } else {
+      r = win_bwd_record(win_flav(), win_part(), 0, 0, 0, 0, &img_bytes, &hcap);
+    }
+    float* hTw = LDS_TABLE(float, lds_raw, r.hTw);
+    float* asTw = LDS_TABLE(float, lds_raw, r.asTw);
+    float* adTo = LDS_TABLE(float, lds_raw, r.adTo);
+    float* alTw = LDS_TABLE(float, lds_raw, r.alTw);
+    float* wlA = LDS_TABLE(float, lds_raw, r.wlA);
+    float* gpT = LDS_TABLE(float, lds_raw, r.gpT);
+    float* gkeep = (PTAB ? keep_ : r.gkeep != NO_TABLE) ? LDS_TABLE(float, lds_raw, r.gkeep) : nullptr;
+    u16* rpo = LDS_TABLE(u16, lds_raw, r.rp + 2 * lo);
+    const u16* mrp = LDS_TABLE(const u16, lds_raw, r.mrp);
+    u16* hrow = LDS_TABLE(u16, lds_raw, r.hrow);
+    u16* hedge = LDS_TABLE(u16, lds_raw, r.hedge);
+    u16* erow = LDS_TABLE(u16, lds_raw, r.erow);
+    u16* eedge = LDS_TABLE(u16, lds_raw, r.eedge);
+    unsigned char* bflag_o = lds_raw + (r.bflag + lo);
     __syncthreads();
-    const unsigned char* bflag = bflag_o - lo;
-    for (int k = tid; k < ((ow + 15) & ~15) / 4; k += THREADS) reinterpret_cast<unsigned*>(bflag_o)[k] = 0u;
     int hrcnt = 0, hecnt = 0, ercnt = 0, eecnt = 0;
-    if (PTAB || pt) {
+    if constexpr (PTAB) {
       hrcnt = H(GATRES_PT_B_HRCNT); hecnt = H(GATRES_PT_B_HECNT); ercnt = H(GATRES_PT_B_ERCNT); eecnt = H(GATRES_PT_B_EECNT);
-      if (H(GATRES_PT_B_IMG_WORDS) * 2 != (int)(b_img_end - rpo) || hrcnt > hcap || hecnt > hcap || ercnt > hcap || eecnt > hcap) {
-        if (tid == 0) *a.err = 1;
-        hrcnt = min(hrcnt, hcap); hecnt = min(hecnt, hcap); ercnt = min(ercnt, hcap); eecnt = min(eecnt, hcap);
-      } else {
-        dma_copy4<THREADS>(reinterpret_cast<float*>(rpo), reinterpret_cast<const float*>(pt + H(GATRES_PT_B_IMG)),
-                           H(GATRES_PT_B_IMG_WORDS), 0);
-      }
+      dma_copy4<THREADS>(reinterpret_cast<float*>(rpo), reinterpret_cast<const float*>(pt + H(GATRES_PT_B_IMG)),
+                         H(GATRES_PT_B_IMG_WORDS), 0);
       dma_copy4<THREADS>(reinterpret_cast<float*>(hrow), reinterpret_cast<const float*>(pt + H(GATRES_PT_B_HROW)), (hrcnt + 1) / 2, 0);
       dma_copy4<THREADS>(reinterpret_cast<float*>(hedge), reinterpret_cast<const float*>(pt + H(GATRES_PT_B_HEDGE)), (hecnt + 1) / 2, 0);
       dma_copy4<THREADS>(reinterpret_cast<float*>(erow), reinterpret_cast<const float*>(pt + H(GATRES_PT_B_EROW)), (ercnt + 1) / 2, 0);
       dma_copy4<THREADS>(reinterpret_cast<float*>(eedge), reinterpret_cast<const float*>(pt + H(GATRES_PT_B_EEDGE)), (eecnt + 1) / 2, 0);
+      dma_copy4<THREADS>(reinterpret_cast<float*>(bflag_o), reinterpret_cast<const float*>(pt + H(GATRES_PT_B_FLAGS)),
+                         ((ow + 15) & ~15) / 4, 0);
     } else {
-      copy_rowptr16<THREADS>(rpo, a.rowptr, n0 + lo, ow, e0 + elo);
-      copy_idx16<THREADS>(colo, a.col, e0 + elo, oeg, n0);
-      copy_rowptr16<THREADS>(trpo, a.t_rowptr, n0 + lo, ow, t0 + tlo);
-      copy_idx16<THREADS>(teido, a.t_eid, t0 + tlo, otg, e0);
-      copy_idx16<THREADS>(tdsto, a.t_dst, t0 + tlo, otg, n0);
-      copy_rowptr16<THREADS>(mrpw, a.m_rowptr, n0 + wlo, wr, a.m_rowptr[n0 + wlo]);
-      copy_rowptr16<THREADS>(mtrpo, a.mt_rowptr, n0 + lo, ow, mt0 + mtlo);
-      copy_idx16<THREADS>(mtdsto, a.mt_dst, mt0 + mtlo, otm, n0);
-    }
-    const u16* rp = rpo - lo;  const u16* trp = trpo - lo;  const u16* mrp = mrpw - wlo;  const u16* mtrp = mtrpo - lo;
-    float* RA = RAw - wlo * 2 * NC;
-    float* gpT = RAw - wlo * NC;
-    float* gy2T = RAw + (size_t)wr * NC - wlo * NC;
-    float* ge2 = gew - ewlo;      float* ge1 = gew - ewlo * 2;
-    float* gad2 = gado - lo;      float* gad1 = gado - lo * 2;
-    float* hT2 = hTw - wlo * NC;  float* hT1 = hTw - wlo * 2 * NC;
-    float* asT2 = asTw - wlo;     float* asT1 = asTw - wlo * 2;
-    float* adT2 = adTo - lo;      float* adT1 = adTo - lo * 2;
-    float* alT2 = alTw - ewlo;    float* alT1 = alTw - ewlo * 2;
-    float* xG2 = xGo - lo * (NC + XPB);   float* xG1 = xGo - lo * (2 * NC + XPB);
-    float* gkeep = keep_ ? gko - lo * NC : nullptr;
-
+      for (int k = tid; k < ((ow + 15) & ~15) / 4; k += THREADS) reinterpret_cast<unsigned*>(bflag_o)[k] = 0u;
+      if (pt) {
+        hrcnt = H(GATRES_PT_B_HRCNT); hecnt = H(GATRES_PT_B_HECNT); ercnt = H(GATRES_PT_B_ERCNT); eecnt = H(GATRES_PT_B_EECNT);
+        if (H(GATRES_PT_B_IMG_WORDS) * 4 != img_bytes || hrcnt > hcap || hecnt > hcap || ercnt > hcap || eecnt > hcap) {
+          if (tid == 0) *a.err = 1;
+          hrcnt = min(hrcnt, hcap); hecnt = min(hecnt, hcap); ercnt = min(ercnt, hcap); eecnt = min(eecnt, hcap);
+        } else {
+          dma_copy4<THREADS>(reinterpret_cast<float*>(rpo), reinterpret_cast<const float*>(pt + H(GATRES_PT_B_IMG)),
+                             H(GATRES_PT_B_IMG_WORDS), 0);
+        }
+        dma_copy4<THREADS>(reinterpret_cast<float*>(hrow), reinterpret_cast<const float*>(pt + H(GATRES_PT_B_HROW)), (hrcnt + 1) / 2, 0);
+        dma_copy4<THREADS>(reinterpret_cast<float*>(hedge), reinterpret_cast<const float*>(pt + H(GATRES_PT_B_HEDGE)), (hecnt + 1) / 2, 0);
+        dma_copy4<THREADS>(reinterpret_cast<float*>(erow), reinterpret_cast<const float*>(pt + H(GATRES_PT_B_EROW)), (ercnt + 1) / 2, 0);
+        dma_copy4<THREADS>(reinterpret_cast<float*>(eedge), reinterpret_cast<const float*>(pt + H(GATRES_PT_B_EEDGE)), (eecnt + 1) / 2, 0);
+      } else {
+        copy_rowptr16<THREADS>(rpo, a.rowptr, n0 + lo, ow, e0 + elo);
+        copy_idx16<THREADS>(LDS_TABLE(u16, lds_raw, r.colo), a.col, e0 + elo, oeg, n0);
+        copy_rowptr16<THREADS>(LDS_TABLE(u16, lds_raw, r.trp + 2 * lo), a.t_rowptr, n0 + lo, ow, t0 + tlo);
+        copy_idx16<THREADS>(LDS_TABLE(u16, lds_raw, r.teido), a.t_eid, t0 + tlo, otg, e0);
+        copy_idx16<THREADS>(LDS_TABLE(u16, lds_raw, r.tdsto), a.t_dst, t0 + tlo, otg, n0);
+        copy_rowptr16<THREADS>(LDS_TABLE(u16, lds_raw, r.mrp + 2 * wlo), a.m_rowptr, n0 + wlo, wr, a.m_rowptr[n0 + wlo]);
+        copy_rowptr16<THREADS>(LDS_TABLE(u16, lds_raw, r.mtrp + 2 * lo), a.mt_rowptr, n0 + lo, ow, mt0 + mtlo);
+        copy_idx16<THREADS>(LDS_TABLE(u16, lds_raw, r.mtdsto), a.mt_dst, mt0 + mtlo, otm, n0);
+      }
+    }
     const float* xfinal = segbase + (int64_t)L.nb * SL.bstride + SL.xin;
     auto dma_conv2_early = [&](int blk, int w0) {
       if (wave_u < w0) return;
@@ -783,54 +760,56 @@
                                 slab + L.p_lin1_b, L.nb > 0 ? 1 : 0, red, gkeep);
     }
     dma_land(0);
-    if (PTAB || pt) {
+    if constexpr (PTAB) {
       __syncthreads();
     } else {
-      build_nbr_in<THREADS>(rw, rp, colo, oeg, false, nbin);
-      build_nbr_out<THREADS>(rw, trp, tdsto, teido, 0, nullptr, otg, tout);
-      build_nbr_out<THREADS>(rw, mtrp, mtdsto, nullptr, 0, mrp, otm, mout);
-      hrcnt = hecnt = uni(build_halo<THREADS>(trp, tdsto, teido, rw, hrow, hedge, hcap, hcounter));
-      ercnt = uni(build_export_rows<THREADS>(a.rowptr, a.col, n0, rw, erow, hcap, hcounter));
-      if (tid == 0) *hcounter = 0;
-      __syncthreads();
-      for (int k = tid; k < oeg; k += THREADS) {
-        const int j = colo[k];
-        if (j < lo || j >= rw.hi) {
-          const int pos = atomicAdd(hcounter, 1);
-          if (pos < hcap) eedge[pos] = (u16)(elo + k);
-        }
-      }
-      __syncthreads();
-      eecnt = uni(*hcounter);
-      if (hrcnt > hcap || ercnt > hcap || eecnt > hcap) {
-        if (tid == 0) *a.err = 1;
-        hrcnt = hecnt = min(hrcnt, hcap); ercnt = min(ercnt, hcap); eecnt = min(eecnt, hcap);
-      }
-    }
-    for (int k = tid; k < ercnt; k += THREADS) bflag_o[(int)erow[k] - lo] = 1;
+      if (pt) {
+        __syncthreads();
+      } else {
+        const u16* rp = LDS_TABLE(const u16, lds_raw, r.rp);
+        const u16* trp = LDS_TABLE(const u16, lds_raw, r.trp);
+        const u16* mtrp = LDS_TABLE(const u16, lds_raw, r.mtrp);
+        u16* colo = LDS_TABLE(u16, lds_raw, r.colo);
+        u16* teido = LDS_TABLE(u16, lds_raw, r.teido);
+        u16* tdsto = LDS_TABLE(u16, lds_raw, r.tdsto);
+        int* hcounter = reinterpret_cast<int*>(hrow - 2);
+        build_nbr_in<THREADS>(rw, rp, colo, oeg, false, LDS_TABLE(u16, lds_raw, r.nbin));
+        build_nbr_out<THREADS>(rw, trp, tdsto, teido, 0, nullptr, otg, LDS_TABLE(u16, lds_raw, r.tout));
+        build_nbr_out<THREADS>(rw, mtrp, LDS_TABLE(u16, lds_raw, r.mtdsto), nullptr, 0, mrp, otm, LDS_TABLE(u16, lds_raw, r.mout));
+        hrcnt = hecnt = uni(build_halo<THREADS>(trp, tdsto, teido, rw, hrow, hedge, hcap, hcounter));
+        ercnt = uni(build_export_rows<THREADS>(a.rowptr, a.col, n0, rw, erow, hcap, hcounter));
+        if (tid == 0) *hcounter = 0;
+        __syncthreads();
+        for (int k = tid; k < oeg; k += THREADS) {
+          const int j = colo[k];
+          if (j < lo || j >= rw.hi) {
+            const int pos = atomicAdd(hcounter, 1);
+            if (pos < hcap) eedge[pos] = (u16)(elo + k);
+          }
+        }
+        __syncthreads();
+        eecnt = uni(*hcounter);
+        if (hrcnt > hcap || ercnt > hcap || eecnt > hcap) {
+          if (tid == 0) *a.err = 1;
+          hrcnt = hecnt = min(hrcnt, hcap); ercnt = min(ercnt, hcap); eecnt = min(eecnt, hcap);
+        }
+      }
+      for (int k = tid; k < ercnt; k += THREADS) bflag_o[(int)erow[k] - lo] = 1;
+    }
     if constexpr (NC == 32) scale_g_pre<NC, THREADS>(gpT, mrp, lo, ow);
-    if (tid == 0) {
-      BwdRec r;
-      r.lo = rw.lo; r.hi = rw.hi; r.ow = ow; r.wr = wr; r.wlo = wlo; r.elo = elo; r.ewlo = ewlo; r.weg = weg; r.n0 = n0;
-      r.hrcnt = hrcnt; r.hecnt = hecnt; r.ercnt = ercnt; r.eecnt = eecnt;
-      r.RA = lds_off(RA); r.gpT = lds_off(gpT); r.gy2T = lds_off(gy2T); r.ge2 = lds_off(ge2); r.ge1 = lds_off(ge1);
-      r.gad2 = lds_off(gad2); r.gad1 = lds_off(gad1); r.hTw = lds_off(hTw); r.hT2 = lds_off(hT2); r.hT1 = lds_off(hT1);
-      r.asTw = lds_off(asTw); r.asT2 = lds_off(asT2); r.asT1 = lds_off(asT1); r.adTo = lds_off(adTo); r.adT2 = lds_off(adT2);
-      r.adT1 = lds_off(adT1); r.alTw = lds_off(alTw); r.alT2 = lds_off(alT2); r.alT1 = lds_off(alT1); r.xG2 = lds_off(xG2);
-      r.xG1 = lds_off(xG1); r.gkeep = gkeep ? lds_off(gkeep) : NO_TABLE; r.wlA = lds_off(wlA); r.wlB = lds_off(wlB);
-      r.rp = lds_off(rp); r.colo = lds_off(colo); r.trp = lds_off(trp); r.teido = lds_off(teido); r.tdsto = lds_off(tdsto);
-      r.mrp = lds_off(mrp); r.mtrp = lds_off(mtrp); r.mtdsto = lds_off(mtdsto); r.nbin = lds_off(nbin); r.tout = lds_off(tout);
-      r.mout = lds_off(mout); r.hrow = lds_off(hrow); r.hedge = lds_off(hedge); r.erow = lds_off(erow); r.eedge = lds_off(eedge);
-      r.bflag = lds_off(bflag); r.mo1 = mo1 ? lds_off(mo1) : NO_TABLE; r.mxin = mxin ? lds_off(mxin) : NO_TABLE;
-      const int* src = reinterpret_cast<const int*>(&r);
+    if constexpr (!PTAB) {
+      if (tid == 0) {
+        r.hrcnt = hrcnt; r.hecnt = hecnt; r.ercnt = ercnt; r.eecnt = eecnt;
+        const int* src = reinterpret_cast<const int*>(&r);
 #pragma unroll
-      for (int k = 0; k < (int)(sizeof(BwdRec) / 4); ++k)
-        __hip_atomic_store(myrec + GATRES_UREC_WORDS / 2 + k, src[k], __ATOMIC_RELAXED, __HIP_MEMORY_SCOPE_AGENT);
-      asm volatile("s_waitcnt vmcnt(0)" ::: "memory");
+        for (int k = 0; k < (int)(sizeof(BwdRec) / 4); ++k)
+          __hip_atomic_store(urec_w + GATRES_UREC_WORDS / 2 + k, src[k], __ATOMIC_RELAXED, __HIP_MEMORY_SCOPE_AGENT);
+        asm volatile("s_waitcnt vmcnt(0)" ::: "memory");
+      }
     }
     }
     __syncthreads();
-    rec_published();
+    if constexpr (!PTAB) rec_published();
 #undef RECP
 #define RECP rb_
     auto xout = [&](bool on, const unsigned char* bflag, unsigned t_rows, unsigned t_small) {
@@ -1152,7 +1131,7 @@
     case 8: hipLaunchKernelGGL((gatres_window_kernel<8, 1024>), dim3(grid), dim3(1024), 0, st, a); break;
     case 16: hipLaunchKernelGGL((gatres_window_kernel<16, 1024>), dim3(grid), dim3(1024), 0, st, a); break;
     case 32: {
-      int facts = (a.sym ? 0x200 : 0) | (a.facts & 0x1400) | ((a.ptab && a.ptab_m == a.M) ? 0x800 : 0);
+      int facts = (a.sym ? 0x200 : 0) | (a.facts & 0x1400) | ((a.ptab && a.ptab_m == a.M && (a.facts & 0x800)) ? 0x800 : 0);
       if ((a.facts & 0x2000) && facts == 0x1e00) facts |= 0x2000;
       if ((a.facts & 0x4000) && (facts & 0x1e00) == 0x1e00 && !a.safe_sync) facts |= 0x4000;
       const int key = a.phases | (a.keep_lds ? 0x100 : 0) | (facts & gatres_knobs()->window_ph_mask) |
diff --git a/gnn-pressure-estimation_amd/graph_plan.py b/gnn-pressure-estimation_amd/graph_plan.py
--- a/gnn-pressure-estimation_amd/graph_plan.py
+++ b/gnn-pressure-estimation_amd/graph_plan.py
@@ -79,8 +79,9 @@
         self.num_nodes, self.num_edges_gat, self.num_edges_mean = N, Eg, E
         self.device = device
         self._host = host if segments else None
-        self._part_tables: Dict[int, Tuple[torch.Tensor, int]] = {}
-        self._bound: Dict[int, "_native.GatresGraph"] = {}
+        self._part_tables_host: Dict[int, Tuple[torch.Tensor, int]] = {}
+        self._part_tables: Dict[Tuple[int, int, int], Tuple[torch.Tensor, int]] = {}
+        self._bound: Dict[Tuple[int, int, int], "_native.GatresGraph"] = {}
         import threading
         self._bind_lock = threading.Lock()
         self.arrays: Dict[str, torch.Tensor] = {k: v.to(device) for k, v in host.items()}
@@ -105,27 +106,39 @@
         m = int(lib.gatres_fused_cus_per_segment(cmodel_ref, C.byref(self.c)))
         if m < 2 or m > 8 or self.max_segment_nodes > 65535:
             return self.c
+        cm = cmodel_ref._obj
+        key = (m, int(cm.nc), int(cm.num_blocks))
         with self._bind_lock:
-            got = self._bound.get(m)
+            got = self._bound.get(key)
             if got is not None:
                 return got
-            ptrs = [self._host[k].data_ptr() for k in ("rowptr", "col", "t_rowptr", "t_eid", "t_dst", "m_rowptr", "m_col",
-                                                       "mt_rowptr", "mt_dst")]
-            stride = C.c_int64(0)
-            rc = lib.gatres_graph_part_tables_host(*ptrs, self.segment_ptr_host.data_ptr(), self.num_segments, m, None, 0,
-                                                   C.byref(stride))
+            host = self._part_tables_host.get(m)
+            if host is None:
+                ptrs = [self._host[k].data_ptr() for k in ("rowptr", "col", "t_rowptr", "t_eid", "t_dst", "m_rowptr", "m_col",
+                                                           "mt_rowptr", "mt_dst")]
+                stride = C.c_int64(0)
+                rc = lib.gatres_graph_part_tables_host(*ptrs, self.segment_ptr_host.data_ptr(), self.num_segments, m, None, 0,
+                                                       C.byref(stride))
+                if rc != 0:
+                    self._bound[key] = self.c
+                    return self.c
+                words = torch.zeros(self.num_segments * m * int(stride.value), dtype=torch.int32)
+                _native.check(lib.gatres_graph_part_tables_host(*ptrs, self.segment_ptr_host.data_ptr(), self.num_segments, m,
+                                                                words.data_ptr(), int(stride.value), C.byref(stride)),
+                              "gatres_graph_part_tables_host")
+                host = self._part_tables_host[m] = (words, int(stride.value))
+            words, stride_words = host[0].clone(), host[1]
+            rec_key = C.c_int32(0)
+            rc = lib.gatres_graph_part_records_host(words.data_ptr(), self.num_segments, m, stride_words, key[1], key[2],
+                                                    C.byref(rec_key))
             if rc != 0:
-                self._bound[m] = self.c
-                return self.c
-            words = torch.zeros(self.num_segments * m * int(stride.value), dtype=torch.int32)
-            _native.check(lib.gatres_graph_part_tables_host(*ptrs, self.segment_ptr_host.data_ptr(), self.num_segments, m,
-                                                            words.data_ptr(), int(stride.value), C.byref(stride)),
-                          "gatres_graph_part_tables_host")
+                rec_key = C.c_int32(0)
             dev = words.to(self.device)
-            self._part_tables[m] = (dev, int(stride.value))
+            self._part_tables[key] = (dev, stride_words)
             c = _native.GatresGraph.from_buffer_copy(self.c)
-            c.part_tables, c.part_tables_m, c.part_tables_stride = dev.data_ptr(), m, int(stride.value)
-            self._bound[m] = c
+            c.part_tables, c.part_tables_m, c.part_tables_stride = dev.data_ptr(), m, stride_words
+            c.part_tables_key = int(rec_key.value)
+            self._bound[key] = c
             return c
 
     def bind(self, cmodel_ref) -> None:
diff --git a/include/gatres.h b/include/gatres.h
--- a/include/gatres.h
+++ b/include/gatres.h
@@ -39,7 +39,7 @@
   int32_t reserved2;
   const int32_t* perm;
   int32_t halo[7];
-  int32_t reserved3;
+  int32_t part_tables_key;
   const int32_t* part_tables;
   int32_t part_tables_m;
   int32_t part_tables_stride;
@@ -52,9 +52,14 @@
   GATRES_PT_F_IMG, GATRES_PT_F_IMG_WORDS, GATRES_PT_F_HLIST, GATRES_PT_F_HCNT, GATRES_PT_F_ELIST, GATRES_PT_F_ECNT,
   GATRES_PT_B_IMG, GATRES_PT_B_IMG_WORDS, GATRES_PT_B_HROW, GATRES_PT_B_HRCNT, GATRES_PT_B_HEDGE, GATRES_PT_B_HECNT,
   GATRES_PT_B_EROW, GATRES_PT_B_ERCNT, GATRES_PT_B_EEDGE, GATRES_PT_B_EECNT,
+  GATRES_PT_F_FLAGS, GATRES_PT_B_FLAGS,
+  GATRES_PT_F_REC, GATRES_PT_B_REC, GATRES_PT_REC_KEY,
   GATRES_PT_HEADER = 48
 };
 #define GATRES_PT_MAGIC_VALUE 0x47545031
+#define GATRES_PT_REC_STRIDE   128
+#define GATRES_PT_REC_FLAVOURS 3
+#define GATRES_PT_KEY(nc, nb, ok_mask) (0x40000000 | (((ok_mask) & 0xf) << 16) | (((nb) & 0xff) << 8) | ((nc) & 0xff))
 
 #define GATRES_GRAPH_SYMMETRIC 1
 
@@ -75,6 +80,9 @@
                                   const int32_t* mt_rowptr, const int32_t* mt_dst, const int32_t* seg_ptr,
                                   int32_t num_segments, int32_t m, int32_t* out, int64_t stride_words,
                                   int64_t* stride_words_out);
+
+int gatres_graph_part_records_host(int32_t* part_tables_host, int32_t num_segments, int32_t m, int64_t stride_words,
+                                   int32_t nc, int32_t num_blocks, int32_t* key_out);
 
 int gatres_graph_segments_host(const int64_t* edge_index_host, int64_t num_edges, int64_t num_nodes,
                                int32_t merge_upto, int32_t* seg_ptr_host, int32_t* num_segments_out,
@@ -291,6 +299,7 @@
 int gatres_fused_serialize(void* stream);
 int gatres_probe_xcd_dispatch(void* stream);
 int64_t gatres_fused_status_offset(const gatres_model_t* m, const gatres_graph_t* g);
+int64_t gatres_fused_record_offset(const gatres_model_t* m, const gatres_graph_t* g, int64_t* words_out);
 int gatres_fused_set_stamps(uint64_t* stamps, int32_t capacity);
 int gatres_fused_prepare_backward(const gatres_model_t* m, const gatres_graph_t* g, const float* params,
                                   float* scratch, void* stream);
```

New measurement: 106,500 snapshots/s, median of 6. +1.7%, better.
